# Orange-OpenSource/Cool-Chic

Measured on AMD Instinct MI355X. Metric: decoded Mpixel/s, higher is better.
Workload: dtype int64+f64 entropy / f32 synthesis; 1 GPU; kodak24; frames_on_rank0=24, frame=512x768 RGB 8-bit, HOP decoder

## Files before the change

cool_chic_amd/csrc/ccd_dec_parts4.inc:

```
                ".p2align 6\n\t"
                "440:\n\t"
                "s_lshr_b64 s[40:41], s[52:53], 24\n\t"
                "ds_read2st64_b64 v[58:61], v50 offset0:2 offset1:3\n\t"
                "s_waitcnt lgkmcnt(1)\n\t"
                "v_mad_u64_u32 v[44:45], s[42:43], s40, v40, 0\n\t"
                "v_mad_u32_u24 v45, v40, s41, v45\n\t"
                "v_cmpx_ge_u64 vcc, s[50:51], v[44:45]\n\t"
                "v_mad_u64_u32 v[48:49], s[42:43], s40, v41, 0\n\t"
                "v_mad_u32_u24 v49, v41, s41, v49\n\t"
                "s_ff1_i32_b64 s44, vcc\n\t"
                "v_writelane_b32 %[raw], s44, 0\n\t"
                "v_readfirstlane_b32 s48, v48\n\t"
                "v_readfirstlane_b32 s49, v49\n\t"
                "v_readfirstlane_b32 s46, v44\n\t"
                "v_readfirstlane_b32 s47, v45\n\t"
                "s_mov_b64 exec, -1\n\t"
                "s_sub_u32 s76, s50, s46\n\t"
                "s_subb_u32 s77, s51, s47\n\t"
                "441:\n\t"
                "s_lshr_b64 s[40:41], s[48:49], 24\n\t"
                "v_mad_u64_u32 v[44:45], s[42:43], s40, v42, 0\n\t"
                "v_mad_u32_u24 v45, v42, s41, v45\n\t"
                "v_cmpx_ge_u64 vcc, s[76:77], v[44:45]\n\t"
                "v_mad_u64_u32 v[48:49], s[42:43], s40, v43, 0\n\t"
                "v_mad_u32_u24 v49, v43, s41, v49\n\t"
                "s_ff1_i32_b64 s80, vcc\n\t"
                "v_writelane_b32 %[raw], s80, 1\n\t"
                "v_readfirstlane_b32 s74, v48\n\t"
                "v_readfirstlane_b32 s75, v49\n\t"
                "v_readfirstlane_b32 s78, v44\n\t"
                "v_readfirstlane_b32 s79, v45\n\t"
                "s_mov_b64 exec, -1\n\t"
                "s_min_u32 s58, s49, s75\n\t"
                "s_cmp_eq_u32 s58, 0\n\t"
                "s_cbranch_scc1 1801f\n\t"
                "s_sub_u32 s50, s76, s78\n\t"
                "s_subb_u32 s51, s77, s79\n\t"
                "442:\n\t"
                "ds_read_b32 v54, v51\n\t"
                "s_lshr_b64 s[40:41], s[74:75], 24\n\t"
                "ds_read2st64_b64 v[40:43], v50 offset0:4 offset1:5\n\t"
                "s_waitcnt lgkmcnt(2)\n\t"
                "v_mad_u64_u32 v[44:45], s[42:43], s40, v58, 0\n\t"
                "v_mad_u32_u24 v45, v58, s41, v45\n\t"
                "v_cmpx_ge_u64 vcc, s[50:51], v[44:45]\n\t"
                "v_mad_u64_u32 v[48:49], s[42:43], s40, v59, 0\n\t"
                "v_mad_u32_u24 v49, v59, s41, v49\n\t"
                "s_ff1_i32_b64 s44, vcc\n\t"
                "v_writelane_b32 %[raw], s44, 2\n\t"
                "v_readfirstlane_b32 s52, v48\n\t"
                "v_readfirstlane_b32 s53, v49\n\t"
                "v_readfirstlane_b32 s46, v44\n\t"
                "v_readfirstlane_b32 s47, v45\n\t"
                "s_mov_b64 exec, -1\n\t"
                "s_sub_u32 s76, s50, s46\n\t"
                "s_subb_u32 s77, s51, s47\n\t"
                "443:\n\t"
                "s_lshr_b64 s[40:41], s[52:53], 24\n\t"
                "v_mad_u64_u32 v[44:45], s[42:43], s40, v60, 0\n\t"
                "v_mad_u32_u24 v45, v60, s41, v45\n\t"
                "v_cmpx_ge_u64 vcc, s[76:77], v[44:45]\n\t"
                "v_mad_u64_u32 v[48:49], s[42:43], s40, v61, 0\n\t"
                "v_mad_u32_u24 v49, v61, s41, v49\n\t"
                "s_ff1_i32_b64 s80, vcc\n\t"
                "v_writelane_b32 %[raw], s80, 3\n\t"
                "v_readfirstlane_b32 s48, v48\n\t"
                "v_readfirstlane_b32 s49, v49\n\t"
                "v_readfirstlane_b32 s78, v44\n\t"
                "v_readfirstlane_b32 s79, v45\n\t"
                "s_mov_b64 exec, -1\n\t"
                "s_min_u32 s58, s53, s49\n\t"
                "s_cmp_eq_u32 s58, 0\n\t"
                "s_cbranch_scc1 1802f\n\t"
                "s_sub_u32 s50, s76, s78\n\t"
                "s_subb_u32 s51, s77, s79\n\t"
                "444:\n\t"
                "s_mov_b64 exec, 0xf\n\t"
                "v_sub_u32 v52, %[top], %[raw]\n\t"
                "v_add_u32 v52, 1, v52\n\t"
                "ds_write_b8 %[ring], v52\n\t"
                "global_store_byte %[goff], v52, %[lat]\n\t"
                "s_mov_b64 exec, -1\n\t"
                "s_add_u32 s58, %[pix0], %[i]\n\t"
                "s_add_u32 s58, s58, 4\n\t"
                "v_mov_b32 v56, s58\n\t"
                "ds_write_b32 %[rdy], v56 offset:68\n\t"
                "s_add_u32 s59, %[i], 8\n\t"
                "s_waitcnt lgkmcnt(3)\n\t"
                "v_readfirstlane_b32 s58, v54\n\t"
                "s_cmp_le_u32 s59, s66\n\t"
                "s_cbranch_scc0 445f\n\t"
                "s_bitcmp1_b32 s58, 1\n\t"
                "s_cbranch_scc0 445f\n\t"
                "s_mov_b64 s[52:53], s[48:49]\n\t"
                "v_add_u32 v50, 0x800, v50\n\t"
                "ds_read_b32 %[top], v53\n\t"
                "ds_read_b32 %[ring], v53 offset:520\n\t"
                "ds_read_b32 %[goff], v53 offset:1040\n\t"
                "s_add_u32 %[i], %[i], 4\n\t"
                "s_mov_b32 s67, %[i]\n\t"
                "s_add_u32 s54, %[i], 4\n\t"
                "s_branch 450f\n\t"
                "445:\n\t"
                "s_mov_b64 s[52:53], s[48:49]\n\t"
                "s_add_u32 %[i], %[i], 4\n\t"
                "s_mov_b32 s67, %[i]\n\t"
                "s_branch 126b\n\t"
                "1801:\n\t"
                "s_cmp_eq_u32 s49, 0\n\t"
                "s_cbranch_scc0 1851f\n\t"
                "s_cmp_eq_u32 s48, 0\n\t"
                "s_cbranch_scc1 2001f\n\t"
                "s_sub_u32 s58, %[wpos], %[wbase]\n\t"
                "s_and_b32 s58, s58, 63\n\t"
                "v_readlane_b32 s57, %[wbuf], s58\n\t"
                "s_mov_b32 s77, s76\n\t"
                "s_mov_b32 s76, s57\n\t"
                "s_mov_b32 s49, s48\n\t"
                "s_mov_b32 s48, 0\n\t"
                "s_add_u32 %[wpos], %[wpos], 1\n\t"
                "s_cmp_eq_u32 s58, 63\n\t"
                "s_cbranch_scc0 441b\n\t"
                "s_mov_b64 s[50:51], s[76:77]\n\t"
                "s_mov_b64 s[52:53], s[48:49]\n\t"
                "s_add_u32 %[i], %[i], 1\n\t"
                "s_branch 15f\n\t"
                "2001:\n\t"
                "ds_read_b64 v[42:43], v50 offset:512\n\t"
                "ds_read_b64 v[46:47], v50 offset:1024\n\t"
                "s_branch 40b\n\t"
                "1851:\n\t"
                "s_cmp_eq_u32 s74, 0\n\t"
                "s_cbranch_scc1 2051f\n\t"
                "s_sub_u32 s50, s76, s78\n\t"
                "s_subb_u32 s51, s77, s79\n\t"
                "s_sub_u32 s58, %[wpos], %[wbase]\n\t"
                "s_and_b32 s58, s58, 63\n\t"
                "v_readlane_b32 s57, %[wbuf], s58\n\t"
                "s_mov_b32 s51, s50\n\t"
                "s_mov_b32 s50, s57\n\t"
                "s_mov_b32 s75, s74\n\t"
                "s_mov_b32 s74, 0\n\t"
                "s_add_u32 %[wpos], %[wpos], 1\n\t"
                "s_cmp_eq_u32 s58, 63\n\t"
                "s_cbranch_scc0 442b\n\t"
                "s_mov_b64 s[52:53], s[74:75]\n\t"
                "s_add_u32 %[i], %[i], 2\n\t"
                "s_branch 15f\n\t"
                "2051:\n\t"
                "s_mov_b64 s[50:51], s[76:77]\n\t"
                "s_mov_b32 s46, s78\n\t"
                "s_mov_b32 s47, s79\n\t"
                "s_mov_b32 s44, s80\n\t"
                "s_mov_b64 s[52:53], s[48:49]\n\t"
                "s_mov_b64 s[48:49], s[74:75]\n\t"
                "s_add_u32 %[i], %[i], 1\n\t"
                "ds_read_b64 v[46:47], v50 offset:1024\n\t"
                "ds_read_b64 v[40:41], v50 offset:1536\n\t"
                "s_branch 41b\n\t"
                "1802:\n\t"
                "s_cmp_eq_u32 s53, 0\n\t"
                "s_cbranch_scc0 1852f\n\t"
                "s_cmp_eq_u32 s52, 0\n\t"
                "s_cbranch_scc1 2002f\n\t"
                "s_sub_u32 s58, %[wpos], %[wbase]\n\t"
                "s_and_b32 s58, s58, 63\n\t"
                "v_readlane_b32 s57, %[wbuf], s58\n\t"
                "s_mov_b32 s77, s76\n\t"
                "s_mov_b32 s76, s57\n\t"
                "s_mov_b32 s53, s52\n\t"
                "s_mov_b32 s52, 0\n\t"
                "s_add_u32 %[wpos], %[wpos], 1\n\t"
                "s_cmp_eq_u32 s58, 63\n\t"
                "s_cbranch_scc0 443b\n\t"
                "s_mov_b64 s[50:51], s[76:77]\n\t"
                "s_add_u32 %[i], %[i], 3\n\t"
                "s_branch 15f\n\t"
                "2002:\n\t"
                "s_mov_b64 s[48:49], s[52:53]\n\t"
                "s_mov_b64 s[52:53], s[74:75]\n\t"
                "s_add_u32 %[i], %[i], 2\n\t"
                "ds_read_b64 v[40:41], v50 offset:1536\n\t"
                "ds_read_b64 v[42:43], v50 offset:2048\n\t"
                "s_branch 42b\n\t"
                "1852:\n\t"
                "s_cmp_eq_u32 s48, 0\n\t"
                "s_cbranch_scc1 2052f\n\t"
                "s_sub_u32 s50, s76, s78\n\t"
                "s_subb_u32 s51, s77, s79\n\t"
                "s_sub_u32 s58, %[wpos], %[wbase]\n\t"
                "s_and_b32 s58, s58, 63\n\t"
                "v_readlane_b32 s57, %[wbuf], s58\n\t"
                "s_mov_b32 s51, s50\n\t"
                "s_mov_b32 s50, s57\n\t"
                "s_mov_b32 s49, s48\n\t"
                "s_mov_b32 s48, 0\n\t"
                "s_add_u32 %[wpos], %[wpos], 1\n\t"
                "s_cmp_eq_u32 s58, 63\n\t"
                "s_cbranch_scc0 444b\n\t"
                "s_mov_b64 s[52:53], s[48:49]\n\t"
                "s_add_u32 %[i], %[i], 4\n\t"
                "s_branch 15f\n\t"
                "2052:\n\t"
                "s_mov_b64 s[50:51], s[76:77]\n\t"
                "s_mov_b32 s46, s78\n\t"
                "s_mov_b32 s47, s79\n\t"
                "s_mov_b32 s44, s80\n\t"
                "s_add_u32 %[i], %[i], 3\n\t"
                "v_add_u32 v50, 0x600, v50\n\t"
                "ds_read_b64 v[42:43], v50 offset:512\n\t"
                "ds_read_b64 v[46:47], v50 offset:1024\n\t"
                "s_branch 40b\n\t"
                ".p2align 6\n\t"
                "450:\n\t"
                "s_lshr_b64 s[40:41], s[52:53], 24\n\t"
                "ds_read2st64_b64 v[58:61], v50 offset0:2 offset1:3\n\t"
                "s_waitcnt lgkmcnt(1)\n\t"
                "v_mad_u64_u32 v[44:45], s[42:43], s40, v40, 0\n\t"
                "v_mad_u32_u24 v45, v40, s41, v45\n\t"
                "v_cmpx_ge_u64 vcc, s[50:51], v[44:45]\n\t"
                "v_mad_u64_u32 v[48:49], s[42:43], s40, v41, 0\n\t"
                "v_mad_u32_u24 v49, v41, s41, v49\n\t"
                "s_ff1_i32_b64 s44, vcc\n\t"
                "v_writelane_b32 %[raw], s44, 4\n\t"
                "v_readfirstlane_b32 s48, v48\n\t"
                "v_readfirstlane_b32 s49, v49\n\t"
                "v_readfirstlane_b32 s46, v44\n\t"
                "v_readfirstlane_b32 s47, v45\n\t"
                "s_mov_b64 exec, -1\n\t"
                "s_sub_u32 s76, s50, s46\n\t"
                "s_subb_u32 s77, s51, s47\n\t"
                "451:\n\t"
                "s_lshr_b64 s[40:41], s[48:49], 24\n\t"
                "v_mad_u64_u32 v[44:45], s[42:43], s40, v42, 0\n\t"
                "v_mad_u32_u24 v45, v42, s41, v45\n\t"
                "v_cmpx_ge_u64 vcc, s[76:77], v[44:45]\n\t"
                "v_mad_u64_u32 v[48:49], s[42:43], s40, v43, 0\n\t"
                "v_mad_u32_u24 v49, v43, s41, v49\n\t"
                "s_ff1_i32_b64 s80, vcc\n\t"
                "v_writelane_b32 %[raw], s80, 5\n\t"
                "v_readfirstlane_b32 s74, v48\n\t"
                "v_readfirstlane_b32 s75, v49\n\t"
                "v_readfirstlane_b32 s78, v44\n\t"
                "v_readfirstlane_b32 s79, v45\n\t"
                "s_mov_b64 exec, -1\n\t"
                "s_min_u32 s58, s49, s75\n\t"
                "s_cmp_eq_u32 s58, 0\n\t"
                "s_cbranch_scc1 2201f\n\t"
                "s_sub_u32 s50, s76, s78\n\t"
                "s_subb_u32 s51, s77, s79\n\t"
                "452:\n\t"
                "ds_read_b32 v54, v51\n\t"
                "s_lshr_b64 s[40:41], s[74:75], 24\n\t"
                "ds_read2st64_b64 v[40:43], v50 offset0:4 offset1:5\n\t"
                "s_waitcnt lgkmcnt(2)\n\t"
                "v_mad_u64_u32 v[44:45], s[42:43], s40, v58, 0\n\t"
                "v_mad_u32_u24 v45, v58, s41, v45\n\t"
                "v_cmpx_ge_u64 vcc, s[50:51], v[44:45]\n\t"
                "v_mad_u64_u32 v[48:49], s[42:43], s40, v59, 0\n\t"
                "v_mad_u32_u24 v49, v59, s41, v49\n\t"
                "s_ff1_i32_b64 s44, vcc\n\t"
                "v_writelane_b32 %[raw], s44, 6\n\t"
                "v_readfirstlane_b32 s52, v48\n\t"
                "v_readfirstlane_b32 s53, v49\n\t"
                "v_readfirstlane_b32 s46, v44\n\t"
                "v_readfirstlane_b32 s47, v45\n\t"
                "s_mov_b64 exec, -1\n\t"
                "s_sub_u32 s76, s50, s46\n\t"
                "s_subb_u32 s77, s51, s47\n\t"
                "453:\n\t"
                "s_lshr_b64 s[40:41], s[52:53], 24\n\t"
                "v_mad_u64_u32 v[44:45], s[42:43], s40, v60, 0\n\t"
                "v_mad_u32_u24 v45, v60, s41, v45\n\t"
                "v_cmpx_ge_u64 vcc, s[76:77], v[44:45]\n\t"
                "v_mad_u64_u32 v[48:49], s[42:43], s40, v61, 0\n\t"
                "v_mad_u32_u24 v49, v61, s41, v49\n\t"
                "s_ff1_i32_b64 s80, vcc\n\t"
                "v_writelane_b32 %[raw], s80, 7\n\t"
                "v_readfirstlane_b32 s48, v48\n\t"
                "v_readfirstlane_b32 s49, v49\n\t"
                "v_readfirstlane_b32 s78, v44\n\t"
                "v_readfirstlane_b32 s79, v45\n\t"
                "s_mov_b64 exec, -1\n\t"
                "s_min_u32 s58, s53, s49\n\t"
                "s_cmp_eq_u32 s58, 0\n\t"
                "s_cbranch_scc1 2202f\n\t"
                "s_sub_u32 s50, s76, s78\n\t"
                "s_subb_u32 s51, s77, s79\n\t"
                "454:\n\t"
                "s_mov_b64 exec, 0xf0\n\t"
                "v_sub_u32 v52, %[top], %[raw]\n\t"
                "v_add_u32 v52, 1, v52\n\t"
                "ds_write_b8 %[ring], v52\n\t"
                "global_store_byte %[goff], v52, %[lat]\n\t"
                "s_mov_b64 exec, -1\n\t"
                "s_add_u32 s58, %[pix0], %[i]\n\t"
                "s_add_u32 s58, s58, 4\n\t"
                "v_mov_b32 v56, s58\n\t"
                "ds_write_b32 %[rdy], v56 offset:68\n\t"
                "s_add_u32 s59, %[i], 8\n\t"
                "s_waitcnt lgkmcnt(3)\n\t"
                "v_readfirstlane_b32 s58, v54\n\t"
                "s_cmp_le_u32 s59, s66\n\t"
                "s_cbranch_scc0 455f\n\t"
                "s_bitcmp1_b32 s58, 2\n\t"
                "s_cbranch_scc0 455f\n\t"
                "s_mov_b64 s[52:53], s[48:49]\n\t"
                "v_add_u32 v50, 0x800, v50\n\t"
                "ds_read_b32 %[top], v53\n\t"
                "ds_read_b32 %[ring], v53 offset:520\n\t"
                "ds_read_b32 %[goff], v53 offset:1040\n\t"
                "s_add_u32 %[i], %[i], 4\n\t"
                "s_mov_b32 s67, %[i]\n\t"
                "s_add_u32 s54, %[i], 4\n\t"
                "s_branch 460f\n\t"
                "455:\n\t"
                "s_mov_b64 s[52:53], s[48:49]\n\t"
                "s_add_u32 %[i], %[i], 4\n\t"
                "s_mov_b32 s67, %[i]\n\t"
                "s_branch 126b\n\t"
                "2201:\n\t"
                "s_cmp_eq_u32 s49, 0\n\t"
                "s_cbranch_scc0 2251f\n\t"
                "s_cmp_eq_u32 s48, 0\n\t"
                "s_cbranch_scc1 2401f\n\t"
                "s_sub_u32 s58, %[wpos], %[wbase]\n\t"
                "s_and_b32 s58, s58, 63\n\t"
                "v_readlane_b32 s57, %[wbuf], s58\n\t"
                "s_mov_b32 s77, s76\n\t"
                "s_mov_b32 s76, s57\n\t"
                "s_mov_b32 s49, s48\n\t"
                "s_mov_b32 s48, 0\n\t"
                "s_add_u32 %[wpos], %[wpos], 1\n\t"
                "s_cmp_eq_u32 s58, 63\n\t"
                "s_cbranch_scc0 451b\n\t"
                "s_mov_b64 s[50:51], s[76:77]\n\t"
                "s_mov_b64 s[52:53], s[48:49]\n\t"
                "s_add_u32 %[i], %[i], 1\n\t"
                "s_branch 15f\n\t"
                "2401:\n\t"
                "ds_read_b64 v[42:43], v50 offset:512\n\t"
                "ds_read_b64 v[46:47], v50 offset:1024\n\t"
                "s_branch 40b\n\t"
                "2251:\n\t"
                "s_cmp_eq_u32 s74, 0\n\t"
                "s_cbranch_scc1 2451f\n\t"
                "s_sub_u32 s50, s76, s78\n\t"
                "s_subb_u32 s51, s77, s79\n\t"
                "s_sub_u32 s58, %[wpos], %[wbase]\n\t"
                "s_and_b32 s58, s58, 63\n\t"
                "v_readlane_b32 s57, %[wbuf], s58\n\t"
                "s_mov_b32 s51, s50\n\t"
                "s_mov_b32 s50, s57\n\t"
                "s_mov_b32 s75, s74\n\t"
                "s_mov_b32 s74, 0\n\t"
                "s_add_u32 %[wpos], %[wpos], 1\n\t"
                "s_cmp_eq_u32 s58, 63\n\t"
                "s_cbranch_scc0 452b\n\t"
                "s_mov_b64 s[52:53], s[74:75]\n\t"
                "s_add_u32 %[i], %[i], 2\n\t"
                "s_branch 15f\n\t"
                "2451:\n\t"
                "s_mov_b64 s[50:51], s[76:77]\n\t"
                "s_mov_b32 s46, s78\n\t"
                "s_mov_b32 s47, s79\n\t"
                "s_mov_b32 s44, s80\n\t"
                "s_mov_b64 s[52:53], s[48:49]\n\t"
                "s_mov_b64 s[48:49], s[74:75]\n\t"
                "s_add_u32 %[i], %[i], 1\n\t"
                "ds_read_b64 v[46:47], v50 offset:1024\n\t"
                "ds_read_b64 v[40:41], v50 offset:1536\n\t"
                "s_branch 41b\n\t"
                "2202:\n\t"
                "s_cmp_eq_u32 s53, 0\n\t"
                "s_cbranch_scc0 2252f\n\t"
                "s_cmp_eq_u32 s52, 0\n\t"
                "s_cbranch_scc1 2402f\n\t"
                "s_sub_u32 s58, %[wpos], %[wbase]\n\t"
                "s_and_b32 s58, s58, 63\n\t"
                "v_readlane_b32 s57, %[wbuf], s58\n\t"
                "s_mov_b32 s77, s76\n\t"
                "s_mov_b32 s76, s57\n\t"
                "s_mov_b32 s53, s52\n\t"
                "s_mov_b32 s52, 0\n\t"
                "s_add_u32 %[wpos], %[wpos], 1\n\t"
                "s_cmp_eq_u32 s58, 63\n\t"
                "s_cbranch_scc0 453b\n\t"
                "s_mov_b64 s[50:51], s[76:77]\n\t"
                "s_add_u32 %[i], %[i], 3\n\t"
                "s_branch 15f\n\t"
                "2402:\n\t"
                "s_mov_b64 s[48:49], s[52:53]\n\t"
                "s_mov_b64 s[52:53], s[74:75]\n\t"
                "s_add_u32 %[i], %[i], 2\n\t"
                "ds_read_b64 v[40:41], v50 offset:1536\n\t"
                "ds_read_b64 v[42:43], v50 offset:2048\n\t"
                "s_branch 42b\n\t"
                "2252:\n\t"
                "s_cmp_eq_u32 s48, 0\n\t"
                "s_cbranch_scc1 2452f\n\t"
                "s_sub_u32 s50, s76, s78\n\t"
                "s_subb_u32 s51, s77, s79\n\t"
                "s_sub_u32 s58, %[wpos], %[wbase]\n\t"
                "s_and_b32 s58, s58, 63\n\t"
                "v_readlane_b32 s57, %[wbuf], s58\n\t"
                "s_mov_b32 s51, s50\n\t"
                "s_mov_b32 s50, s57\n\t"
                "s_mov_b32 s49, s48\n\t"
                "s_mov_b32 s48, 0\n\t"
                "s_add_u32 %[wpos], %[wpos], 1\n\t"
                "s_cmp_eq_u32 s58, 63\n\t"
                "s_cbranch_scc0 454b\n\t"
                "s_mov_b64 s[52:53], s[48:49]\n\t"
                "s_add_u32 %[i], %[i], 4\n\t"
                "s_branch 15f\n\t"
                "2452:\n\t"
                "s_mov_b64 s[50:51], s[76:77]\n\t"
                "s_mov_b32 s46, s78\n\t"
                "s_mov_b32 s47, s79\n\t"
                "s_mov_b32 s44, s80\n\t"
                "s_add_u32 %[i], %[i], 3\n\t"
                "v_add_u32 v50, 0x600, v50\n\t"
                "ds_read_b64 v[42:43], v50 offset:512\n\t"
                "ds_read_b64 v[46:47], v50 offset:1024\n\t"
                "s_branch 40b\n\t"
                ".p2align 6\n\t"
                "460:\n\t"
                "s_lshr_b64 s[40:41], s[52:53], 24\n\t"
                "ds_read2st64_b64 v[58:61], v50 offset0:2 offset1:3\n\t"
                "s_waitcnt lgkmcnt(1)\n\t"
                "v_mad_u64_u32 v[44:45], s[42:43], s40, v40, 0\n\t"
                "v_mad_u32_u24 v45, v40, s41, v45\n\t"
                "v_cmpx_ge_u64 vcc, s[50:51], v[44:45]\n\t"
                "v_mad_u64_u32 v[48:49], s[42:43], s40, v41, 0\n\t"
                "v_mad_u32_u24 v49, v41, s41, v49\n\t"
                "s_ff1_i32_b64 s44, vcc\n\t"
                "v_writelane_b32 %[raw], s44, 8\n\t"
                "v_readfirstlane_b32 s48, v48\n\t"
                "v_readfirstlane_b32 s49, v49\n\t"
                "v_readfirstlane_b32 s46, v44\n\t"
                "v_readfirstlane_b32 s47, v45\n\t"
                "s_mov_b64 exec, -1\n\t"
                "s_sub_u32 s76, s50, s46\n\t"
                "s_subb_u32 s77, s51, s47\n\t"
                "461:\n\t"
                "s_lshr_b64 s[40:41], s[48:49], 24\n\t"
                "v_mad_u64_u32 v[44:45], s[42:43], s40, v42, 0\n\t"
                "v_mad_u32_u24 v45, v42, s41, v45\n\t"
                "v_cmpx_ge_u64 vcc, s[76:77], v[44:45]\n\t"
                "v_mad_u64_u32 v[48:49], s[42:43], s40, v43, 0\n\t"
                "v_mad_u32_u24 v49, v43, s41, v49\n\t"
                "s_ff1_i32_b64 s80, vcc\n\t"
                "v_writelane_b32 %[raw], s80, 9\n\t"
                "v_readfirstlane_b32 s74, v48\n\t"
                "v_readfirstlane_b32 s75, v49\n\t"
                "v_readfirstlane_b32 s78, v44\n\t"
                "v_readfirstlane_b32 s79, v45\n\t"
                "s_mov_b64 exec, -1\n\t"
                "s_min_u32 s58, s49, s75\n\t"
                "s_cmp_eq_u32 s58, 0\n\t"
                "s_cbranch_scc1 2601f\n\t"
                "s_sub_u32 s50, s76, s78\n\t"
                "s_subb_u32 s51, s77, s79\n\t"
                "462:\n\t"
                "ds_read_b32 v54, v51\n\t"
                "s_lshr_b64 s[40:41], s[74:75], 24\n\t"
                "ds_read2st64_b64 v[40:43], v50 offset0:4 offset1:5\n\t"
                "s_waitcnt lgkmcnt(2)\n\t"
                "v_mad_u64_u32 v[44:45], s[42:43], s40, v58, 0\n\t"
                "v_mad_u32_u24 v45, v58, s41, v45\n\t"
                "v_cmpx_ge_u64 vcc, s[50:51], v[44:45]\n\t"
                "v_mad_u64_u32 v[48:49], s[42:43], s40, v59, 0\n\t"
                "v_mad_u32_u24 v49, v59, s41, v49\n\t"
                "s_ff1_i32_b64 s44, vcc\n\t"
                "v_writelane_b32 %[raw], s44, 10\n\t"
                "v_readfirstlane_b32 s52, v48\n\t"
                "v_readfirstlane_b32 s53, v49\n\t"
                "v_readfirstlane_b32 s46, v44\n\t"
                "v_readfirstlane_b32 s47, v45\n\t"
                "s_mov_b64 exec, -1\n\t"
                "s_sub_u32 s76, s50, s46\n\t"
                "s_subb_u32 s77, s51, s47\n\t"
                "463:\n\t"
                "s_lshr_b64 s[40:41], s[52:53], 24\n\t"
                "v_mad_u64_u32 v[44:45], s[42:43], s40, v60, 0\n\t"
                "v_mad_u32_u24 v45, v60, s41, v45\n\t"
                "v_cmpx_ge_u64 vcc, s[76:77], v[44:45]\n\t"
                "v_mad_u64_u32 v[48:49], s[42:43], s40, v61, 0\n\t"
                "v_mad_u32_u24 v49, v61, s41, v49\n\t"
                "s_ff1_i32_b64 s80, vcc\n\t"
                "v_writelane_b32 %[raw], s80, 11\n\t"
                "v_readfirstlane_b32 s48, v48\n\t"
                "v_readfirstlane_b32 s49, v49\n\t"
                "v_readfirstlane_b32 s78, v44\n\t"
                "v_readfirstlane_b32 s79, v45\n\t"
                "s_mov_b64 exec, -1\n\t"
                "s_min_u32 s58, s53, s49\n\t"
                "s_cmp_eq_u32 s58, 0\n\t"
                "s_cbranch_scc1 2602f\n\t"
                "s_sub_u32 s50, s76, s78\n\t"
                "s_subb_u32 s51, s77, s79\n\t"
                "464:\n\t"
                "s_mov_b64 exec, 0xf00\n\t"
                "v_sub_u32 v52, %[top], %[raw]\n\t"
                "v_add_u32 v52, 1, v52\n\t"
                "ds_write_b8 %[ring], v52\n\t"
                "global_store_byte %[goff], v52, %[lat]\n\t"
                "s_mov_b64 exec, -1\n\t"
                "s_add_u32 s58, %[pix0], %[i]\n\t"
                "s_add_u32 s58, s58, 4\n\t"
                "v_mov_b32 v56, s58\n\t"
                "ds_write_b32 %[rdy], v56 offset:68\n\t"
                "s_add_u32 s59, %[i], 8\n\t"
                "s_waitcnt lgkmcnt(3)\n\t"
                "v_readfirstlane_b32 s58, v54\n\t"
                "s_cmp_le_u32 s59, s66\n\t"
                "s_cbranch_scc0 465f\n\t"
                "s_bitcmp1_b32 s58, 3\n\t"
                "s_cbranch_scc0 465f\n\t"
                "s_mov_b64 s[52:53], s[48:49]\n\t"
                "v_add_u32 v50, 0x800, v50\n\t"
                "ds_read_b32 %[top], v53\n\t"
                "ds_read_b32 %[ring], v53 offset:520\n\t"
                "ds_read_b32 %[goff], v53 offset:1040\n\t"
                "s_add_u32 %[i], %[i], 4\n\t"
                "s_mov_b32 s67, %[i]\n\t"
                "s_add_u32 s54, %[i], 4\n\t"
                "s_branch 470f\n\t"
                "465:\n\t"
                "s_mov_b64 s[52:53], s[48:49]\n\t"
                "s_add_u32 %[i], %[i], 4\n\t"
                "s_mov_b32 s67, %[i]\n\t"
                "s_branch 126b\n\t"
                "2601:\n\t"
                "s_cmp_eq_u32 s49, 0\n\t"
                "s_cbranch_scc0 2651f\n\t"
                "s_cmp_eq_u32 s48, 0\n\t"
                "s_cbranch_scc1 2801f\n\t"
                "s_sub_u32 s58, %[wpos], %[wbase]\n\t"
                "s_and_b32 s58, s58, 63\n\t"
                "v_readlane_b32 s57, %[wbuf], s58\n\t"
                "s_mov_b32 s77, s76\n\t"
                "s_mov_b32 s76, s57\n\t"
                "s_mov_b32 s49, s48\n\t"
                "s_mov_b32 s48, 0\n\t"
                "s_add_u32 %[wpos], %[wpos], 1\n\t"
                "s_cmp_eq_u32 s58, 63\n\t"
                "s_cbranch_scc0 461b\n\t"
                "s_mov_b64 s[50:51], s[76:77]\n\t"
                "s_mov_b64 s[52:53], s[48:49]\n\t"
                "s_add_u32 %[i], %[i], 1\n\t"
                "s_branch 15f\n\t"
                "2801:\n\t"
                "ds_read_b64 v[42:43], v50 offset:512\n\t"
                "ds_read_b64 v[46:47], v50 offset:1024\n\t"
                "s_branch 40b\n\t"
                "2651:\n\t"
                "s_cmp_eq_u32 s74, 0\n\t"
                "s_cbranch_scc1 2851f\n\t"
                "s_sub_u32 s50, s76, s78\n\t"
                "s_subb_u32 s51, s77, s79\n\t"
                "s_sub_u32 s58, %[wpos], %[wbase]\n\t"
                "s_and_b32 s58, s58, 63\n\t"
                "v_readlane_b32 s57, %[wbuf], s58\n\t"
                "s_mov_b32 s51, s50\n\t"
                "s_mov_b32 s50, s57\n\t"
                "s_mov_b32 s75, s74\n\t"
                "s_mov_b32 s74, 0\n\t"
                "s_add_u32 %[wpos], %[wpos], 1\n\t"
                "s_cmp_eq_u32 s58, 63\n\t"
                "s_cbranch_scc0 462b\n\t"
                "s_mov_b64 s[52:53], s[74:75]\n\t"
                "s_add_u32 %[i], %[i], 2\n\t"
                "s_branch 15f\n\t"
                "2851:\n\t"
                "s_mov_b64 s[50:51], s[76:77]\n\t"
                "s_mov_b32 s46, s78\n\t"
                "s_mov_b32 s47, s79\n\t"
                "s_mov_b32 s44, s80\n\t"
                "s_mov_b64 s[52:53], s[48:49]\n\t"
                "s_mov_b64 s[48:49], s[74:75]\n\t"
                "s_add_u32 %[i], %[i], 1\n\t"
                "ds_read_b64 v[46:47], v50 offset:1024\n\t"
                "ds_read_b64 v[40:41], v50 offset:1536\n\t"
                "s_branch 41b\n\t"
                "2602:\n\t"
                "s_cmp_eq_u32 s53, 0\n\t"
                "s_cbranch_scc0 2652f\n\t"
                "s_cmp_eq_u32 s52, 0\n\t"
                "s_cbranch_scc1 2802f\n\t"
                "s_sub_u32 s58, %[wpos], %[wbase]\n\t"
                "s_and_b32 s58, s58, 63\n\t"
                "v_readlane_b32 s57, %[wbuf], s58\n\t"
                "s_mov_b32 s77, s76\n\t"
                "s_mov_b32 s76, s57\n\t"
                "s_mov_b32 s53, s52\n\t"
                "s_mov_b32 s52, 0\n\t"
                "s_add_u32 %[wpos], %[wpos], 1\n\t"
                "s_cmp_eq_u32 s58, 63\n\t"
                "s_cbranch_scc0 463b\n\t"
                "s_mov_b64 s[50:51], s[76:77]\n\t"
                "s_add_u32 %[i], %[i], 3\n\t"
                "s_branch 15f\n\t"
                "2802:\n\t"
                "s_mov_b64 s[48:49], s[52:53]\n\t"
                "s_mov_b64 s[52:53], s[74:75]\n\t"
                "s_add_u32 %[i], %[i], 2\n\t"
                "ds_read_b64 v[40:41], v50 offset:1536\n\t"
                "ds_read_b64 v[42:43], v50 offset:2048\n\t"
                "s_branch 42b\n\t"
                "2652:\n\t"
                "s_cmp_eq_u32 s48, 0\n\t"
                "s_cbranch_scc1 2852f\n\t"
                "s_sub_u32 s50, s76, s78\n\t"
                "s_subb_u32 s51, s77, s79\n\t"
                "s_sub_u32 s58, %[wpos], %[wbase]\n\t"
                "s_and_b32 s58, s58, 63\n\t"
                "v_readlane_b32 s57, %[wbuf], s58\n\t"
                "s_mov_b32 s51, s50\n\t"
                "s_mov_b32 s50, s57\n\t"
                "s_mov_b32 s49, s48\n\t"
                "s_mov_b32 s48, 0\n\t"
                "s_add_u32 %[wpos], %[wpos], 1\n\t"
                "s_cmp_eq_u32 s58, 63\n\t"
                "s_cbranch_scc0 464b\n\t"
                "s_mov_b64 s[52:53], s[48:49]\n\t"
                "s_add_u32 %[i], %[i], 4\n\t"
                "s_branch 15f\n\t"
                "2852:\n\t"
                "s_mov_b64 s[50:51], s[76:77]\n\t"
                "s_mov_b32 s46, s78\n\t"
                "s_mov_b32 s47, s79\n\t"
                "s_mov_b32 s44, s80\n\t"
                "s_add_u32 %[i], %[i], 3\n\t"
                "v_add_u32 v50, 0x600, v50\n\t"
                "ds_read_b64 v[42:43], v50 offset:512\n\t"
                "ds_read_b64 v[46:47], v50 offset:1024\n\t"
                "s_branch 40b\n\t"
                ".p2align 6\n\t"
                "470:\n\t"
                "s_lshr_b64 s[40:41], s[52:53], 24\n\t"
                "ds_read2st64_b64 v[58:61], v50 offset0:2 offset1:3\n\t"
                "s_waitcnt lgkmcnt(1)\n\t"
                "v_mad_u64_u32 v[44:45], s[42:43], s40, v40, 0\n\t"
                "v_mad_u32_u24 v45, v40, s41, v45\n\t"
                "v_cmpx_ge_u64 vcc, s[50:51], v[44:45]\n\t"
                "v_mad_u64_u32 v[48:49], s[42:43], s40, v41, 0\n\t"
                "v_mad_u32_u24 v49, v41, s41, v49\n\t"
                "s_ff1_i32_b64 s44, vcc\n\t"
                "v_writelane_b32 %[raw], s44, 12\n\t"
                "v_readfirstlane_b32 s48, v48\n\t"
                "v_readfirstlane_b32 s49, v49\n\t"
                "v_readfirstlane_b32 s46, v44\n\t"
                "v_readfirstlane_b32 s47, v45\n\t"
                "s_mov_b64 exec, -1\n\t"
                "s_sub_u32 s76, s50, s46\n\t"
                "s_subb_u32 s77, s51, s47\n\t"
                "471:\n\t"
                "s_lshr_b64 s[40:41], s[48:49], 24\n\t"
                "v_mad_u64_u32 v[44:45], s[42:43], s40, v42, 0\n\t"
                "v_mad_u32_u24 v45, v42, s41, v45\n\t"
                "v_cmpx_ge_u64 vcc, s[76:77], v[44:45]\n\t"
                "v_mad_u64_u32 v[48:49], s[42:43], s40, v43, 0\n\t"
                "v_mad_u32_u24 v49, v43, s41, v49\n\t"
                "s_ff1_i32_b64 s80, vcc\n\t"
                "v_writelane_b32 %[raw], s80, 13\n\t"
                "v_readfirstlane_b32 s74, v48\n\t"
                "v_readfirstlane_b32 s75, v49\n\t"
                "v_readfirstlane_b32 s78, v44\n\t"
                "v_readfirstlane_b32 s79, v45\n\t"
                "s_mov_b64 exec, -1\n\t"
                "s_min_u32 s58, s49, s75\n\t"
                "s_cmp_eq_u32 s58, 0\n\t"
                "s_cbranch_scc1 3001f\n\t"
                "s_sub_u32 s50, s76, s78\n\t"
                "s_subb_u32 s51, s77, s79\n\t"
                "472:\n\t"
                "s_lshr_b64 s[40:41], s[74:75], 24\n\t"
                "s_waitcnt lgkmcnt(0)\n\t"
                "v_mad_u64_u32 v[44:45], s[42:43], s40, v58, 0\n\t"
                "v_mad_u32_u24 v45, v58, s41, v45\n\t"
                "v_cmpx_ge_u64 vcc, s[50:51], v[44:45]\n\t"
                "v_mad_u64_u32 v[48:49], s[42:43], s40, v59, 0\n\t"
                "v_mad_u32_u24 v49, v59, s41, v49\n\t"
                "s_ff1_i32_b64 s44, vcc\n\t"
                "v_writelane_b32 %[raw], s44, 14\n\t"
                "v_readfirstlane_b32 s52, v48\n\t"
                "v_readfirstlane_b32 s53, v49\n\t"
                "v_readfirstlane_b32 s46, v44\n\t"
                "v_readfirstlane_b32 s47, v45\n\t"
                "s_mov_b64 exec, -1\n\t"
                "s_sub_u32 s76, s50, s46\n\t"
                "s_subb_u32 s77, s51, s47\n\t"
                "473:\n\t"
                "s_lshr_b64 s[40:41], s[52:53], 24\n\t"
                "v_mad_u64_u32 v[44:45], s[42:43], s40, v60, 0\n\t"
                "v_mad_u32_u24 v45, v60, s41, v45\n\t"
                "v_cmpx_ge_u64 vcc, s[76:77], v[44:45]\n\t"
                "v_mad_u64_u32 v[48:49], s[42:43], s40, v61, 0\n\t"
                "v_mad_u32_u24 v49, v61, s41, v49\n\t"
                "s_ff1_i32_b64 s80, vcc\n\t"
                "v_writelane_b32 %[raw], s80, 15\n\t"
                "v_readfirstlane_b32 s48, v48\n\t"
                "v_readfirstlane_b32 s49, v49\n\t"
                "v_readfirstlane_b32 s78, v44\n\t"
                "v_readfirstlane_b32 s79, v45\n\t"
                "s_mov_b64 exec, -1\n\t"
                "s_min_u32 s58, s53, s49\n\t"
                "s_cmp_eq_u32 s58, 0\n\t"
                "s_cbranch_scc1 3002f\n\t"
                "s_sub_u32 s50, s76, s78\n\t"
                "s_subb_u32 s51, s77, s79\n\t"
                "474:\n\t"
                "s_mov_b64 s[52:53], s[48:49]\n\t"
                "s_add_u32 %[i], %[i], 4\n\t"
                "s_branch 2b\n\t"
                "3001:\n\t"
                "s_cmp_eq_u32 s49, 0\n\t"
                "s_cbranch_scc0 3051f\n\t"
                "s_cmp_eq_u32 s48, 0\n\t"
                "s_cbranch_scc1 3201f\n\t"
                "s_sub_u32 s58, %[wpos], %[wbase]\n\t"
                "s_and_b32 s58, s58, 63\n\t"
                "v_readlane_b32 s57, %[wbuf], s58\n\t"
                "s_mov_b32 s77, s76\n\t"
                "s_mov_b32 s76, s57\n\t"
                "s_mov_b32 s49, s48\n\t"
                "s_mov_b32 s48, 0\n\t"
                "s_add_u32 %[wpos], %[wpos], 1\n\t"
                "s_cmp_eq_u32 s58, 63\n\t"
                "s_cbranch_scc0 471b\n\t"
                "s_mov_b64 s[50:51], s[76:77]\n\t"
                "s_mov_b64 s[52:53], s[48:49]\n\t"
                "s_add_u32 %[i], %[i], 1\n\t"
                "s_branch 15f\n\t"
                "3201:\n\t"
                "ds_read_b64 v[42:43], v50 offset:512\n\t"
                "ds_read_b64 v[46:47], v50 offset:1024\n\t"
                "s_branch 40b\n\t"
                "3051:\n\t"
                "s_cmp_eq_u32 s74, 0\n\t"
                "s_cbranch_scc1 3251f\n\t"
                "s_sub_u32 s50, s76, s78\n\t"
                "s_subb_u32 s51, s77, s79\n\t"
                "s_sub_u32 s58, %[wpos], %[wbase]\n\t"
                "s_and_b32 s58, s58, 63\n\t"
                "v_readlane_b32 s57, %[wbuf], s58\n\t"
                "s_mov_b32 s51, s50\n\t"
                "s_mov_b32 s50, s57\n\t"
                "s_mov_b32 s75, s74\n\t"
                "s_mov_b32 s74, 0\n\t"
                "s_add_u32 %[wpos], %[wpos], 1\n\t"
                "s_cmp_eq_u32 s58, 63\n\t"
                "s_cbranch_scc0 472b\n\t"
                "s_mov_b64 s[52:53], s[74:75]\n\t"
                "s_add_u32 %[i], %[i], 2\n\t"
                "s_branch 15f\n\t"
                "3251:\n\t"
                "s_mov_b64 s[50:51], s[76:77]\n\t"
                "s_mov_b32 s46, s78\n\t"
                "s_mov_b32 s47, s79\n\t"
                "s_mov_b32 s44, s80\n\t"
                "s_mov_b64 s[52:53], s[48:49]\n\t"
                "s_mov_b64 s[48:49], s[74:75]\n\t"
                "s_add_u32 %[i], %[i], 1\n\t"
                "ds_read_b64 v[46:47], v50 offset:1024\n\t"
                "ds_read_b64 v[40:41], v50 offset:1536\n\t"
                "s_branch 41b\n\t"
                "3002:\n\t"
                "s_cmp_eq_u32 s53, 0\n\t"
                "s_cbranch_scc0 3052f\n\t"
                "s_cmp_eq_u32 s52, 0\n\t"
                "s_cbranch_scc1 3202f\n\t"
                "s_sub_u32 s58, %[wpos], %[wbase]\n\t"
                "s_and_b32 s58, s58, 63\n\t"
                "v_readlane_b32 s57, %[wbuf], s58\n\t"
                "s_mov_b32 s77, s76\n\t"
                "s_mov_b32 s76, s57\n\t"
                "s_mov_b32 s53, s52\n\t"
                "s_mov_b32 s52, 0\n\t"
                "s_add_u32 %[wpos], %[wpos], 1\n\t"
                "s_cmp_eq_u32 s58, 63\n\t"
                "s_cbranch_scc0 473b\n\t"
                "s_mov_b64 s[50:51], s[76:77]\n\t"
                "s_add_u32 %[i], %[i], 3\n\t"
                "s_branch 15f\n\t"
                "3202:\n\t"
                "s_mov_b64 s[48:49], s[52:53]\n\t"
                "s_mov_b64 s[52:53], s[74:75]\n\t"
                "s_add_u32 %[i], %[i], 2\n\t"
                "ds_read_b64 v[40:41], v50 offset:1536\n\t"
                "ds_read_b64 v[42:43], v50 offset:2048\n\t"
                "s_branch 42b\n\t"
                "3052:\n\t"
                "s_cmp_eq_u32 s48, 0\n\t"
                "s_cbranch_scc1 3252f\n\t"
                "s_sub_u32 s50, s76, s78\n\t"
                "s_subb_u32 s51, s77, s79\n\t"
                "s_sub_u32 s58, %[wpos], %[wbase]\n\t"
                "s_and_b32 s58, s58, 63\n\t"
                "v_readlane_b32 s57, %[wbuf], s58\n\t"
                "s_mov_b32 s51, s50\n\t"
                "s_mov_b32 s50, s57\n\t"
                "s_mov_b32 s49, s48\n\t"
                "s_mov_b32 s48, 0\n\t"
                "s_add_u32 %[wpos], %[wpos], 1\n\t"
                "s_cmp_eq_u32 s58, 63\n\t"
                "s_cbranch_scc0 474b\n\t"
                "s_mov_b64 s[52:53], s[48:49]\n\t"
                "s_add_u32 %[i], %[i], 4\n\t"
                "s_branch 15f\n\t"
                "3252:\n\t"
                "s_mov_b64 s[50:51], s[76:77]\n\t"
                "s_mov_b32 s46, s78\n\t"
                "s_mov_b32 s47, s79\n\t"
                "s_mov_b32 s44, s80\n\t"
                "s_add_u32 %[i], %[i], 3\n\t"
                "v_add_u32 v50, 0x600, v50\n\t"
                "ds_read_b64 v[42:43], v50 offset:512\n\t"
                "ds_read_b64 v[46:47], v50 offset:1024\n\t"
                "s_branch 40b\n\t"
```

cool_chic_amd/csrc/ccd_dec_parts8.inc:

```
                ".p2align 6\n\t"
                "400:\n\t"
                "s_lshr_b64 s[40:41], s[52:53], 24\n\t"
                "ds_read2st64_b64 v[58:61], v50 offset0:2 offset1:3\n\t"
                "s_waitcnt lgkmcnt(1)\n\t"
                "v_mad_u64_u32 v[44:45], s[42:43], s40, v40, 0\n\t"
                "v_mad_u32_u24 v45, v40, s41, v45\n\t"
                "v_cmpx_ge_u64 vcc, s[50:51], v[44:45]\n\t"
                "v_mad_u64_u32 v[48:49], s[42:43], s40, v41, 0\n\t"
                "v_mad_u32_u24 v49, v41, s41, v49\n\t"
                "s_ff1_i32_b64 s44, vcc\n\t"
                "v_writelane_b32 %[raw], s44, 0\n\t"
                "v_readfirstlane_b32 s48, v48\n\t"
                "v_readfirstlane_b32 s49, v49\n\t"
                "v_readfirstlane_b32 s46, v44\n\t"
                "v_readfirstlane_b32 s47, v45\n\t"
                "s_mov_b64 exec, -1\n\t"
                "s_sub_u32 s76, s50, s46\n\t"
                "s_subb_u32 s77, s51, s47\n\t"
                "401:\n\t"
                "s_lshr_b64 s[40:41], s[48:49], 24\n\t"
                "v_mad_u64_u32 v[44:45], s[42:43], s40, v42, 0\n\t"
                "v_mad_u32_u24 v45, v42, s41, v45\n\t"
                "v_cmpx_ge_u64 vcc, s[76:77], v[44:45]\n\t"
                "v_mad_u64_u32 v[48:49], s[42:43], s40, v43, 0\n\t"
                "v_mad_u32_u24 v49, v43, s41, v49\n\t"
                "s_ff1_i32_b64 s80, vcc\n\t"
                "v_writelane_b32 %[raw], s80, 1\n\t"
                "v_readfirstlane_b32 s74, v48\n\t"
                "v_readfirstlane_b32 s75, v49\n\t"
                "v_readfirstlane_b32 s78, v44\n\t"
                "v_readfirstlane_b32 s79, v45\n\t"
                "s_mov_b64 exec, -1\n\t"
                "s_min_u32 s58, s49, s75\n\t"
                "s_cmp_eq_u32 s58, 0\n\t"
                "s_cbranch_scc1 1001f\n\t"
                "s_sub_u32 s50, s76, s78\n\t"
                "s_subb_u32 s51, s77, s79\n\t"
                "402:\n\t"
                "s_lshr_b64 s[40:41], s[74:75], 24\n\t"
                "ds_read2st64_b64 v[40:43], v50 offset0:4 offset1:5\n\t"
                "s_waitcnt lgkmcnt(1)\n\t"
                "v_mad_u64_u32 v[44:45], s[42:43], s40, v58, 0\n\t"
                "v_mad_u32_u24 v45, v58, s41, v45\n\t"
                "v_cmpx_ge_u64 vcc, s[50:51], v[44:45]\n\t"
                "v_mad_u64_u32 v[48:49], s[42:43], s40, v59, 0\n\t"
                "v_mad_u32_u24 v49, v59, s41, v49\n\t"
                "s_ff1_i32_b64 s44, vcc\n\t"
                "v_writelane_b32 %[raw], s44, 2\n\t"
                "v_readfirstlane_b32 s52, v48\n\t"
                "v_readfirstlane_b32 s53, v49\n\t"
                "v_readfirstlane_b32 s46, v44\n\t"
                "v_readfirstlane_b32 s47, v45\n\t"
                "s_mov_b64 exec, -1\n\t"
                "s_sub_u32 s76, s50, s46\n\t"
                "s_subb_u32 s77, s51, s47\n\t"
                "403:\n\t"
                "s_lshr_b64 s[40:41], s[52:53], 24\n\t"
                "v_mad_u64_u32 v[44:45], s[42:43], s40, v60, 0\n\t"
                "v_mad_u32_u24 v45, v60, s41, v45\n\t"
                "v_cmpx_ge_u64 vcc, s[76:77], v[44:45]\n\t"
                "v_mad_u64_u32 v[48:49], s[42:43], s40, v61, 0\n\t"
                "v_mad_u32_u24 v49, v61, s41, v49\n\t"
                "s_ff1_i32_b64 s80, vcc\n\t"
                "v_writelane_b32 %[raw], s80, 3\n\t"
                "v_readfirstlane_b32 s48, v48\n\t"
                "v_readfirstlane_b32 s49, v49\n\t"
                "v_readfirstlane_b32 s78, v44\n\t"
                "v_readfirstlane_b32 s79, v45\n\t"
                "s_mov_b64 exec, -1\n\t"
                "s_min_u32 s58, s53, s49\n\t"
                "s_cmp_eq_u32 s58, 0\n\t"
                "s_cbranch_scc1 1002f\n\t"
                "s_sub_u32 s50, s76, s78\n\t"
                "s_subb_u32 s51, s77, s79\n\t"
                "404:\n\t"
                "s_lshr_b64 s[40:41], s[48:49], 24\n\t"
                "ds_read2st64_b64 v[58:61], v50 offset0:6 offset1:7\n\t"
                "s_waitcnt lgkmcnt(1)\n\t"
                "v_mad_u64_u32 v[44:45], s[42:43], s40, v40, 0\n\t"
                "v_mad_u32_u24 v45, v40, s41, v45\n\t"
                "v_cmpx_ge_u64 vcc, s[50:51], v[44:45]\n\t"
                "v_mad_u64_u32 v[48:49], s[42:43], s40, v41, 0\n\t"
                "v_mad_u32_u24 v49, v41, s41, v49\n\t"
                "s_ff1_i32_b64 s44, vcc\n\t"
                "v_writelane_b32 %[raw], s44, 4\n\t"
                "v_readfirstlane_b32 s74, v48\n\t"
                "v_readfirstlane_b32 s75, v49\n\t"
                "v_readfirstlane_b32 s46, v44\n\t"
                "v_readfirstlane_b32 s47, v45\n\t"
                "s_mov_b64 exec, -1\n\t"
                "s_sub_u32 s76, s50, s46\n\t"
                "s_subb_u32 s77, s51, s47\n\t"
                "405:\n\t"
                "s_lshr_b64 s[40:41], s[74:75], 24\n\t"
                "v_mad_u64_u32 v[44:45], s[42:43], s40, v42, 0\n\t"
                "v_mad_u32_u24 v45, v42, s41, v45\n\t"
                "v_cmpx_ge_u64 vcc, s[76:77], v[44:45]\n\t"
                "v_mad_u64_u32 v[48:49], s[42:43], s40, v43, 0\n\t"
                "v_mad_u32_u24 v49, v43, s41, v49\n\t"
                "s_ff1_i32_b64 s80, vcc\n\t"
                "v_writelane_b32 %[raw], s80, 5\n\t"
                "v_readfirstlane_b32 s52, v48\n\t"
                "v_readfirstlane_b32 s53, v49\n\t"
                "v_readfirstlane_b32 s78, v44\n\t"
                "v_readfirstlane_b32 s79, v45\n\t"
                "s_mov_b64 exec, -1\n\t"
                "s_min_u32 s58, s75, s53\n\t"
                "s_cmp_eq_u32 s58, 0\n\t"
                "s_cbranch_scc1 1003f\n\t"
                "s_sub_u32 s50, s76, s78\n\t"
                "s_subb_u32 s51, s77, s79\n\t"
                "406:\n\t"
                "ds_read_b32 v54, v51\n\t"
                "s_lshr_b64 s[40:41], s[52:53], 24\n\t"
                "ds_read2st64_b64 v[40:43], v50 offset0:8 offset1:9\n\t"
                "s_waitcnt lgkmcnt(2)\n\t"
                "v_mad_u64_u32 v[44:45], s[42:43], s40, v58, 0\n\t"
                "v_mad_u32_u24 v45, v58, s41, v45\n\t"
                "v_cmpx_ge_u64 vcc, s[50:51], v[44:45]\n\t"
                "v_mad_u64_u32 v[48:49], s[42:43], s40, v59, 0\n\t"
                "v_mad_u32_u24 v49, v59, s41, v49\n\t"
                "s_ff1_i32_b64 s44, vcc\n\t"
                "v_writelane_b32 %[raw], s44, 6\n\t"
                "v_readfirstlane_b32 s48, v48\n\t"
                "v_readfirstlane_b32 s49, v49\n\t"
                "v_readfirstlane_b32 s46, v44\n\t"
                "v_readfirstlane_b32 s47, v45\n\t"
                "s_mov_b64 exec, -1\n\t"
                "s_sub_u32 s76, s50, s46\n\t"
                "s_subb_u32 s77, s51, s47\n\t"
                "407:\n\t"
                "s_lshr_b64 s[40:41], s[48:49], 24\n\t"
                "v_mad_u64_u32 v[44:45], s[42:43], s40, v60, 0\n\t"
                "v_mad_u32_u24 v45, v60, s41, v45\n\t"
                "v_cmpx_ge_u64 vcc, s[76:77], v[44:45]\n\t"
                "v_mad_u64_u32 v[48:49], s[42:43], s40, v61, 0\n\t"
                "v_mad_u32_u24 v49, v61, s41, v49\n\t"
                "s_ff1_i32_b64 s80, vcc\n\t"
                "v_writelane_b32 %[raw], s80, 7\n\t"
                "v_readfirstlane_b32 s74, v48\n\t"
                "v_readfirstlane_b32 s75, v49\n\t"
                "v_readfirstlane_b32 s78, v44\n\t"
                "v_readfirstlane_b32 s79, v45\n\t"
                "s_mov_b64 exec, -1\n\t"
                "s_min_u32 s58, s49, s75\n\t"
                "s_cmp_eq_u32 s58, 0\n\t"
                "s_cbranch_scc1 1004f\n\t"
                "s_sub_u32 s50, s76, s78\n\t"
                "s_subb_u32 s51, s77, s79\n\t"
                "408:\n\t"
                "s_mov_b64 exec, 0xff\n\t"
                "v_sub_u32 v52, %[top], %[raw]\n\t"
                "v_add_u32 v52, 1, v52\n\t"
                "ds_write_b8 %[ring], v52\n\t"
                "global_store_byte %[goff], v52, %[lat]\n\t"
                "s_mov_b64 exec, -1\n\t"
                "s_add_u32 s58, %[pix0], %[i]\n\t"
                "s_add_u32 s58, s58, 8\n\t"
                "v_mov_b32 v56, s58\n\t"
                "ds_write_b32 %[rdy], v56 offset:68\n\t"
                "s_sub_u32 s59, s66, %[i]\n\t"
                "s_waitcnt lgkmcnt(3)\n\t"
                "v_readfirstlane_b32 s58, v54\n\t"
                "s_cmp_eq_u32 s59, 16\n\t"
                "s_cbranch_scc0 409f\n\t"
                "s_bitcmp1_b32 s58, 1\n\t"
                "s_cbranch_scc0 409f\n\t"
                "ds_read_b32 %[top], v53\n\t"
                "ds_read_b32 %[ring], v53 offset:520\n\t"
                "ds_read_b32 %[goff], v53 offset:1040\n\t"
                "s_mov_b32 s65, 0\n\t"
                "s_mov_b32 s54, s66\n\t"
                "s_branch 308b\n\t"
                "409:\n\t"
                "s_mov_b64 s[52:53], s[74:75]\n\t"
                "s_add_u32 %[i], %[i], 8\n\t"
                "s_mov_b32 s67, %[i]\n\t"
                "s_branch 126b\n\t"
                "1001:\n\t"
                "s_cmp_eq_u32 s49, 0\n\t"
                "s_cbranch_scc0 1051f\n\t"
                "s_cmp_eq_u32 s48, 0\n\t"
                "s_cbranch_scc1 1201f\n\t"
                "s_sub_u32 s58, %[wpos], %[wbase]\n\t"
                "s_and_b32 s58, s58, 63\n\t"
                "v_readlane_b32 s57, %[wbuf], s58\n\t"
                "s_mov_b32 s77, s76\n\t"
                "s_mov_b32 s76, s57\n\t"
                "s_mov_b32 s49, s48\n\t"
                "s_mov_b32 s48, 0\n\t"
                "s_add_u32 %[wpos], %[wpos], 1\n\t"
                "s_cmp_eq_u32 s58, 63\n\t"
                "s_cbranch_scc0 401b\n\t"
                "s_mov_b64 s[50:51], s[76:77]\n\t"
                "s_mov_b64 s[52:53], s[48:49]\n\t"
                "s_add_u32 %[i], %[i], 1\n\t"
                "s_branch 15f\n\t"
                "1201:\n\t"
                "ds_read_b64 v[42:43], v50 offset:512\n\t"
                "ds_read_b64 v[46:47], v50 offset:1024\n\t"
                "s_branch 40b\n\t"
                "1051:\n\t"
                "s_cmp_eq_u32 s74, 0\n\t"
                "s_cbranch_scc1 1251f\n\t"
                "s_sub_u32 s50, s76, s78\n\t"
                "s_subb_u32 s51, s77, s79\n\t"
                "s_sub_u32 s58, %[wpos], %[wbase]\n\t"
                "s_and_b32 s58, s58, 63\n\t"
                "v_readlane_b32 s57, %[wbuf], s58\n\t"
                "s_mov_b32 s51, s50\n\t"
                "s_mov_b32 s50, s57\n\t"
                "s_mov_b32 s75, s74\n\t"
                "s_mov_b32 s74, 0\n\t"
                "s_add_u32 %[wpos], %[wpos], 1\n\t"
                "s_cmp_eq_u32 s58, 63\n\t"
                "s_cbranch_scc0 402b\n\t"
                "s_mov_b64 s[52:53], s[74:75]\n\t"
                "s_add_u32 %[i], %[i], 2\n\t"
                "s_branch 15f\n\t"
                "1251:\n\t"
                "s_mov_b64 s[50:51], s[76:77]\n\t"
                "s_mov_b32 s46, s78\n\t"
                "s_mov_b32 s47, s79\n\t"
                "s_mov_b32 s44, s80\n\t"
                "s_mov_b64 s[52:53], s[48:49]\n\t"
                "s_mov_b64 s[48:49], s[74:75]\n\t"
                "s_add_u32 %[i], %[i], 1\n\t"
                "ds_read_b64 v[46:47], v50 offset:1024\n\t"
                "ds_read_b64 v[40:41], v50 offset:1536\n\t"
                "s_branch 41b\n\t"
                "1002:\n\t"
                "s_cmp_eq_u32 s53, 0\n\t"
                "s_cbranch_scc0 1052f\n\t"
                "s_cmp_eq_u32 s52, 0\n\t"
                "s_cbranch_scc1 1202f\n\t"
                "s_sub_u32 s58, %[wpos], %[wbase]\n\t"
                "s_and_b32 s58, s58, 63\n\t"
                "v_readlane_b32 s57, %[wbuf], s58\n\t"
                "s_mov_b32 s77, s76\n\t"
                "s_mov_b32 s76, s57\n\t"
                "s_mov_b32 s53, s52\n\t"
                "s_mov_b32 s52, 0\n\t"
                "s_add_u32 %[wpos], %[wpos], 1\n\t"
                "s_cmp_eq_u32 s58, 63\n\t"
                "s_cbranch_scc0 403b\n\t"
                "s_mov_b64 s[50:51], s[76:77]\n\t"
                "s_add_u32 %[i], %[i], 3\n\t"
                "s_branch 15f\n\t"
                "1202:\n\t"
                "s_mov_b64 s[48:49], s[52:53]\n\t"
                "s_mov_b64 s[52:53], s[74:75]\n\t"
                "s_add_u32 %[i], %[i], 2\n\t"
                "ds_read_b64 v[40:41], v50 offset:1536\n\t"
                "ds_read_b64 v[42:43], v50 offset:2048\n\t"
                "s_branch 42b\n\t"
                "1052:\n\t"
                "s_cmp_eq_u32 s48, 0\n\t"
                "s_cbranch_scc1 1252f\n\t"
                "s_sub_u32 s50, s76, s78\n\t"
                "s_subb_u32 s51, s77, s79\n\t"
                "s_sub_u32 s58, %[wpos], %[wbase]\n\t"
                "s_and_b32 s58, s58, 63\n\t"
                "v_readlane_b32 s57, %[wbuf], s58\n\t"
                "s_mov_b32 s51, s50\n\t"
                "s_mov_b32 s50, s57\n\t"
                "s_mov_b32 s49, s48\n\t"
                "s_mov_b32 s48, 0\n\t"
                "s_add_u32 %[wpos], %[wpos], 1\n\t"
                "s_cmp_eq_u32 s58, 63\n\t"
                "s_cbranch_scc0 404b\n\t"
                "s_mov_b64 s[52:53], s[48:49]\n\t"
                "s_add_u32 %[i], %[i], 4\n\t"
                "s_branch 15f\n\t"
                "1252:\n\t"
                "s_mov_b64 s[50:51], s[76:77]\n\t"
                "s_mov_b32 s46, s78\n\t"
                "s_mov_b32 s47, s79\n\t"
                "s_mov_b32 s44, s80\n\t"
                "s_add_u32 %[i], %[i], 3\n\t"
                "v_add_u32 v50, 0x600, v50\n\t"
                "ds_read_b64 v[42:43], v50 offset:512\n\t"
                "ds_read_b64 v[46:47], v50 offset:1024\n\t"
                "s_branch 40b\n\t"
                "1003:\n\t"
                "s_cmp_eq_u32 s75, 0\n\t"
                "s_cbranch_scc0 1053f\n\t"
                "s_cmp_eq_u32 s74, 0\n\t"
                "s_cbranch_scc1 1203f\n\t"
                "s_sub_u32 s58, %[wpos], %[wbase]\n\t"
                "s_and_b32 s58, s58, 63\n\t"
                "v_readlane_b32 s57, %[wbuf], s58\n\t"
                "s_mov_b32 s77, s76\n\t"
                "s_mov_b32 s76, s57\n\t"
                "s_mov_b32 s75, s74\n\t"
                "s_mov_b32 s74, 0\n\t"
                "s_add_u32 %[wpos], %[wpos], 1\n\t"
                "s_cmp_eq_u32 s58, 63\n\t"
                "s_cbranch_scc0 405b\n\t"
                "s_mov_b64 s[50:51], s[76:77]\n\t"
                "s_mov_b64 s[52:53], s[74:75]\n\t"
                "s_add_u32 %[i], %[i], 5\n\t"
                "s_branch 15f\n\t"
                "1203:\n\t"
                "s_mov_b64 s[52:53], s[48:49]\n\t"
                "s_mov_b64 s[48:49], s[74:75]\n\t"
                "s_add_u32 %[i], %[i], 4\n\t"
                "v_add_u32 v50, 0x600, v50\n\t"
                "ds_read_b64 v[46:47], v50 offset:1024\n\t"
                "ds_read_b64 v[40:41], v50 offset:1536\n\t"
                "s_branch 41b\n\t"
                "1053:\n\t"
                "s_cmp_eq_u32 s52, 0\n\t"
                "s_cbranch_scc1 1253f\n\t"
                "s_sub_u32 s50, s76, s78\n\t"
                "s_subb_u32 s51, s77, s79\n\t"
                "s_sub_u32 s58, %[wpos], %[wbase]\n\t"
                "s_and_b32 s58, s58, 63\n\t"
                "v_readlane_b32 s57, %[wbuf], s58\n\t"
                "s_mov_b32 s51, s50\n\t"
                "s_mov_b32 s50, s57\n\t"
                "s_mov_b32 s53, s52\n\t"
                "s_mov_b32 s52, 0\n\t"
                "s_add_u32 %[wpos], %[wpos], 1\n\t"
                "s_cmp_eq_u32 s58, 63\n\t"
                "s_cbranch_scc0 406b\n\t"
                "s_add_u32 %[i], %[i], 6\n\t"
                "s_branch 15f\n\t"
                "1253:\n\t"
                "s_mov_b64 s[50:51], s[76:77]\n\t"
                "s_mov_b32 s46, s78\n\t"
                "s_mov_b32 s47, s79\n\t"
                "s_mov_b32 s44, s80\n\t"
                "s_mov_b64 s[48:49], s[52:53]\n\t"
                "s_mov_b64 s[52:53], s[74:75]\n\t"
                "s_add_u32 %[i], %[i], 5\n\t"
                "v_add_u32 v50, 0x600, v50\n\t"
                "ds_read_b64 v[40:41], v50 offset:1536\n\t"
                "ds_read_b64 v[42:43], v50 offset:2048\n\t"
                "s_branch 42b\n\t"
                "1004:\n\t"
                "s_cmp_eq_u32 s49, 0\n\t"
                "s_cbranch_scc0 1054f\n\t"
                "s_cmp_eq_u32 s48, 0\n\t"
                "s_cbranch_scc1 1204f\n\t"
                "s_sub_u32 s58, %[wpos], %[wbase]\n\t"
                "s_and_b32 s58, s58, 63\n\t"
                "v_readlane_b32 s57, %[wbuf], s58\n\t"
                "s_mov_b32 s77, s76\n\t"
                "s_mov_b32 s76, s57\n\t"
                "s_mov_b32 s49, s48\n\t"
                "s_mov_b32 s48, 0\n\t"
                "s_add_u32 %[wpos], %[wpos], 1\n\t"
                "s_cmp_eq_u32 s58, 63\n\t"
                "s_cbranch_scc0 407b\n\t"
                "s_mov_b64 s[50:51], s[76:77]\n\t"
                "s_mov_b64 s[52:53], s[48:49]\n\t"
                "s_add_u32 %[i], %[i], 7\n\t"
                "s_branch 15f\n\t"
                "1204:\n\t"
                "s_add_u32 %[i], %[i], 6\n\t"
                "v_add_u32 v50, 0xc00, v50\n\t"
                "ds_read_b64 v[42:43], v50 offset:512\n\t"
                "ds_read_b64 v[46:47], v50 offset:1024\n\t"
                "s_branch 40b\n\t"
                "1054:\n\t"
                "s_cmp_eq_u32 s74, 0\n\t"
                "s_cbranch_scc1 1254f\n\t"
                "s_sub_u32 s50, s76, s78\n\t"
                "s_subb_u32 s51, s77, s79\n\t"
                "s_sub_u32 s58, %[wpos], %[wbase]\n\t"
                "s_and_b32 s58, s58, 63\n\t"
                "v_readlane_b32 s57, %[wbuf], s58\n\t"
                "s_mov_b32 s51, s50\n\t"
                "s_mov_b32 s50, s57\n\t"
                "s_mov_b32 s75, s74\n\t"
                "s_mov_b32 s74, 0\n\t"
                "s_add_u32 %[wpos], %[wpos], 1\n\t"
                "s_cmp_eq_u32 s58, 63\n\t"
                "s_cbranch_scc0 408b\n\t"
                "s_mov_b64 s[52:53], s[74:75]\n\t"
                "s_add_u32 %[i], %[i], 8\n\t"
                "s_branch 15f\n\t"
                "1254:\n\t"
                "s_mov_b64 s[50:51], s[76:77]\n\t"
                "s_mov_b32 s46, s78\n\t"
                "s_mov_b32 s47, s79\n\t"
                "s_mov_b32 s44, s80\n\t"
                "s_mov_b64 s[52:53], s[48:49]\n\t"
                "s_mov_b64 s[48:49], s[74:75]\n\t"
                "s_add_u32 %[i], %[i], 7\n\t"
                "v_add_u32 v50, 0xc00, v50\n\t"
                "ds_read_b64 v[46:47], v50 offset:1024\n\t"
                "ds_read_b64 v[40:41], v50 offset:1536\n\t"
                "s_branch 41b\n\t"
                ".p2align 6\n\t"
                "420:\n\t"
                "s_lshr_b64 s[40:41], s[52:53], 24\n\t"
                "ds_read2st64_b64 v[58:61], v50 offset0:2 offset1:3\n\t"
                "s_waitcnt lgkmcnt(1)\n\t"
                "v_mad_u64_u32 v[44:45], s[42:43], s40, v40, 0\n\t"
                "v_mad_u32_u24 v45, v40, s41, v45\n\t"
                "v_cmpx_ge_u64 vcc, s[50:51], v[44:45]\n\t"
                "v_mad_u64_u32 v[48:49], s[42:43], s40, v41, 0\n\t"
                "v_mad_u32_u24 v49, v41, s41, v49\n\t"
                "s_ff1_i32_b64 s44, vcc\n\t"
                "v_writelane_b32 %[raw], s44, 8\n\t"
                "v_readfirstlane_b32 s48, v48\n\t"
                "v_readfirstlane_b32 s49, v49\n\t"
                "v_readfirstlane_b32 s46, v44\n\t"
                "v_readfirstlane_b32 s47, v45\n\t"
                "s_mov_b64 exec, -1\n\t"
                "s_sub_u32 s76, s50, s46\n\t"
                "s_subb_u32 s77, s51, s47\n\t"
                "421:\n\t"
                "s_lshr_b64 s[40:41], s[48:49], 24\n\t"
                "v_mad_u64_u32 v[44:45], s[42:43], s40, v42, 0\n\t"
                "v_mad_u32_u24 v45, v42, s41, v45\n\t"
                "v_cmpx_ge_u64 vcc, s[76:77], v[44:45]\n\t"
                "v_mad_u64_u32 v[48:49], s[42:43], s40, v43, 0\n\t"
                "v_mad_u32_u24 v49, v43, s41, v49\n\t"
                "s_ff1_i32_b64 s80, vcc\n\t"
                "v_writelane_b32 %[raw], s80, 9\n\t"
                "v_readfirstlane_b32 s74, v48\n\t"
                "v_readfirstlane_b32 s75, v49\n\t"
                "v_readfirstlane_b32 s78, v44\n\t"
                "v_readfirstlane_b32 s79, v45\n\t"
                "s_mov_b64 exec, -1\n\t"
                "s_min_u32 s58, s49, s75\n\t"
                "s_cmp_eq_u32 s58, 0\n\t"
                "s_cbranch_scc1 1401f\n\t"
                "s_sub_u32 s50, s76, s78\n\t"
                "s_subb_u32 s51, s77, s79\n\t"
                "422:\n\t"
                "s_lshr_b64 s[40:41], s[74:75], 24\n\t"
                "ds_read2st64_b64 v[40:43], v50 offset0:4 offset1:5\n\t"
                "s_waitcnt lgkmcnt(1)\n\t"
                "v_mad_u64_u32 v[44:45], s[42:43], s40, v58, 0\n\t"
                "v_mad_u32_u24 v45, v58, s41, v45\n\t"
                "v_cmpx_ge_u64 vcc, s[50:51], v[44:45]\n\t"
                "v_mad_u64_u32 v[48:49], s[42:43], s40, v59, 0\n\t"
                "v_mad_u32_u24 v49, v59, s41, v49\n\t"
                "s_ff1_i32_b64 s44, vcc\n\t"
                "v_writelane_b32 %[raw], s44, 10\n\t"
                "v_readfirstlane_b32 s52, v48\n\t"
                "v_readfirstlane_b32 s53, v49\n\t"
                "v_readfirstlane_b32 s46, v44\n\t"
                "v_readfirstlane_b32 s47, v45\n\t"
                "s_mov_b64 exec, -1\n\t"
                "s_sub_u32 s76, s50, s46\n\t"
                "s_subb_u32 s77, s51, s47\n\t"
                "423:\n\t"
                "s_lshr_b64 s[40:41], s[52:53], 24\n\t"
                "v_mad_u64_u32 v[44:45], s[42:43], s40, v60, 0\n\t"
                "v_mad_u32_u24 v45, v60, s41, v45\n\t"
                "v_cmpx_ge_u64 vcc, s[76:77], v[44:45]\n\t"
                "v_mad_u64_u32 v[48:49], s[42:43], s40, v61, 0\n\t"
                "v_mad_u32_u24 v49, v61, s41, v49\n\t"
                "s_ff1_i32_b64 s80, vcc\n\t"
                "v_writelane_b32 %[raw], s80, 11\n\t"
                "v_readfirstlane_b32 s48, v48\n\t"
                "v_readfirstlane_b32 s49, v49\n\t"
                "v_readfirstlane_b32 s78, v44\n\t"
                "v_readfirstlane_b32 s79, v45\n\t"
                "s_mov_b64 exec, -1\n\t"
                "s_min_u32 s58, s53, s49\n\t"
                "s_cmp_eq_u32 s58, 0\n\t"
                "s_cbranch_scc1 1402f\n\t"
                "s_sub_u32 s50, s76, s78\n\t"
                "s_subb_u32 s51, s77, s79\n\t"
                "424:\n\t"
                "s_lshr_b64 s[40:41], s[48:49], 24\n\t"
                "ds_read2st64_b64 v[58:61], v50 offset0:6 offset1:7\n\t"
                "s_waitcnt lgkmcnt(1)\n\t"
                "v_mad_u64_u32 v[44:45], s[42:43], s40, v40, 0\n\t"
                "v_mad_u32_u24 v45, v40, s41, v45\n\t"
                "v_cmpx_ge_u64 vcc, s[50:51], v[44:45]\n\t"
                "v_mad_u64_u32 v[48:49], s[42:43], s40, v41, 0\n\t"
// ... 286 lines not shown
```

cool_chic_amd/csrc/ccd_entropy_pipe.hip:

```cpp
#include <hip/hip_runtime.h>
#include <type_traits>

#include "ccd_device.hpp"
#include "ccd_kernels.hpp"
#include "ccd_laplace.hpp"
#include "ccd_wavefront.hpp"

namespace ccd {

#if defined(CCD_PIPE_PROFILE) && CCD_PIPE_PROFILE >= 3
#define PROF_T() __builtin_amdgcn_s_memtime()
#define PROF_ADD(var, t0) var += __builtin_amdgcn_s_memtime() - (t0)
#define PROF_SUB(var, t0) var -= __builtin_amdgcn_s_memtime() - (t0)
#else
#define PROF_T() 0ull
#define PROF_ADD(var, t0) (void)(t0)
#define PROF_SUB(var, t0) (void)(t0)
#endif
#if defined(CCD_PIPE_PROFILE) && CCD_PIPE_PROFILE == 2 && defined(CCD_PIPE_TRACE)
#define LPROF_T(cond) __builtin_amdgcn_s_memtime()
#elif defined(CCD_PIPE_PROFILE) && CCD_PIPE_PROFILE == 2
#define LPROF_T(cond) ((cond) ? __builtin_amdgcn_s_memtime() : 0ull)
#else
#define LPROF_T(cond) 0ull
#endif
#if defined(CCD_PIPE_TRACE)
constexpr int kTraceTasks = 512;
constexpr uint32_t kTraceLdsBytes = kTraceTasks * 32u;
__device__ unsigned int g_trace[kTraceTasks * 8];
__device__ unsigned int g_trace_cfg[2];
constexpr bool kProfTrace = true;
#else
constexpr bool kProfTrace = false;
#endif

#ifndef CCD_T8
#define CCD_T8 25
#endif
#ifndef CCD_T4
#define CCD_T4 9
#endif
#ifndef CCD_PIPE_THREADS
#define CCD_PIPE_THREADS 512
#endif
constexpr int kPipeThreads = CCD_PIPE_THREADS;
constexpr int kPipeWaves = kPipeThreads / 64;
constexpr int kProducers = kPipeWaves - 1;
constexpr int kRows = 128;
constexpr int kSlots = 16;
constexpr int kMaxNV = 8;
constexpr int kRingRows = 512;
constexpr int kNarrowMaxScale = kScaleOffset;
constexpr int kIfceFastIn = 12;
constexpr unsigned kSpinLimit = 1u << 27;

struct alignas(16) RowMeta {
    double rcp[kRows + 2];
    int32_t mu_idx[kRows + 2];
    int32_t top[kRows + 2];
    uint32_t cell[kRows + 2];
    uint32_t goff[kRows + 2];
};
static_assert(offsetof(RowMeta, cell) - offsetof(RowMeta, top) == 520 && offsetof(RowMeta, goff) - offsetof(RowMeta, top) == 1040,
              "the decoder's asm region reads cell / goff at these immediate offsets from a top symbol's address");

extern __shared__ __attribute__((aligned(16))) unsigned char ccd_pipe_smem[];
template <typename T>
__device__ __forceinline__ T* smem_at(uint32_t off) { return reinterpret_cast<T*>(ccd_pipe_smem + off); }
__device__ __forceinline__ uint32_t lds_addr(const void* p) {
    return static_cast<uint32_t>(reinterpret_cast<uintptr_t>((__attribute__((address_space(3))) const char*)p));
}
template <typename T>
__device__ __forceinline__ __attribute__((address_space(3))) T* lds_at(uint32_t addr) {
    return reinterpret_cast<__attribute__((address_space(3))) T*>(static_cast<uintptr_t>(addr));
}
template <typename T>
struct LdsRef {
    uint32_t off;
    __device__ __forceinline__ operator T*() const { return reinterpret_cast<T*>(ccd_pipe_smem + off); }
    __device__ __forceinline__ LdsRef& operator=(T* p) {
        off = static_cast<uint32_t>(reinterpret_cast<unsigned char*>(const_cast<typename std::remove_const<T>::type*>(p)) - ccd_pipe_smem);
        return *this;
    }
};

struct PipeLayout { uint32_t ring, w, b, act, a, tab, meta, rcp, exp, ready, consumed, abort, end; int n_w_hidden; };
__host__ __device__ constexpr PipeLayout pipe_layout(int dim, int n_layers, int in_pad, int ring_rows, int mf_tabs) {
    PipeLayout L{};
    L.ring = 0;
    L.w = static_cast<uint32_t>(ring_rows) * 64u;
    L.n_w_hidden = (n_layers - 1) * dim * in_pad;
    const int n_w_total = L.n_w_hidden + 4 * in_pad;
    L.b = L.w + static_cast<uint32_t>((n_w_total + 3) & ~3) * 4u;
    const int n_b_total = (n_layers - 1) * dim + 4;
    L.act = L.b + static_cast<uint32_t>((n_b_total + 1) & ~1) * 8u;
    L.a = L.act + static_cast<uint32_t>(kProducers * ((mf_tabs ? 16 : 8) * in_pad + 4)) * 4u;
    L.tab = L.a + static_cast<uint32_t>(mf_tabs) * 1024u;
    L.meta = L.tab + static_cast<uint32_t>(kRows + 1) * 64u * 8u;
    L.rcp = L.meta + static_cast<uint32_t>(sizeof(RowMeta));
    L.exp = L.rcp + static_cast<uint32_t>(kNumScale + 1) * 8u;
    L.ready = L.exp + static_cast<uint32_t>(1 << CCD_EXP_LOG) * 8u;
    L.consumed = L.ready + static_cast<uint32_t>(kSlots) * 4u;
    L.abort = L.consumed + 8u;
    L.end = (L.ready + static_cast<uint32_t>(kSlots + 8) * 4u + 15u) & ~15u;
    return L;
}

struct ShapeDyn { static constexpr bool fixed = false; static constexpr int dim = 0, n_layers = 0, n_sp = 0; };
template <int DIM, int NL, int NSP>
struct ShapeFix { static constexpr bool fixed = true; static constexpr int dim = DIM, n_layers = NL, n_sp = NSP; };
using ShapeHop = ShapeFix<20, 3, 14>;

__host__ __device__ constexpr int feat_stride(int n_if) { return n_if > 0 ? n_if : 1; }

struct PipeCtx {
    const EntropyParams* P;
    LdsRef<uint2> s_tab;
    LdsRef<RowMeta> s_meta;
    LdsRef<const double> s_rcp;
    LdsRef<const double> s_exp;
    LdsRef<int32_t> s_w;
    LdsRef<int64_t> s_b;
    LdsRef<int32_t> s_act;
    LdsRef<uint32_t> s_a;
    LdsRef<int8_t> s_ring;
    LdsRef<uint32_t> s_ready;
    LdsRef<uint32_t> s_consumed;
    LdsRef<uint32_t> s_abort;
    int dim, n_layers, n_sp, n_if, n_w_hidden;
    int ring_mask;
#if defined(CCD_PIPE_TRACE)
    uint32_t trace_off;
#endif
    int H, W, fin, fh, fw;
    int fstride;
    int task_pix;
    int k_left;
    int8_t* lat;
    uint32_t seq_base;
    uint32_t px_base;
};

struct DecState {
    uint64_t dist, range;
    uint32_t word_pos, wbase, wbuf;
    uint64_t n_decoded;
    uint32_t n_part_batches;
    unsigned long long prof_wait, prof_work, stall_ticks, stall_events, n_rare, n_search, n_spins;
    unsigned long long wait_by_j[6];
};

__device__ __forceinline__ void lds_write_release(uint32_t* p, uint32_t v) {
    __hip_atomic_store(p, v, __ATOMIC_RELEASE, __HIP_MEMORY_SCOPE_WORKGROUP);
}
__device__ __forceinline__ uint32_t lds_load_acquire(const uint32_t* p) {
    return __builtin_amdgcn_readfirstlane(__hip_atomic_load(p, __ATOMIC_ACQUIRE, __HIP_MEMORY_SCOPE_WORKGROUP));
}

template <typename T> using glb_ptr = T __attribute__((address_space(1)))*;

__device__ __forceinline__ int uni(int v) { return __builtin_amdgcn_readfirstlane(v); }
__device__ __forceinline__ uint32_t uni(uint32_t v) { return __builtin_amdgcn_readfirstlane(v); }
__device__ __forceinline__ uint64_t uni(uint64_t v) {
    return (static_cast<uint64_t>(uni(static_cast<uint32_t>(v >> 32))) << 32) | uni(static_cast<uint32_t>(v));
}

__device__ __forceinline__ bool wait_ge(const uint32_t* p, uint32_t want_v, uint32_t* s_abort) {
    const uint32_t want = uni(want_v);
    if (__builtin_expect(static_cast<int32_t>(lds_load_acquire(p) - want) >= 0, 1)) return true;
    unsigned spins = 0;
    while (static_cast<int32_t>(lds_load_acquire(p) - want) < 0) {
        if ((++spins & 1023u) == 0) {
            if (lds_load_acquire(s_abort) != 0) return false;
            if (spins > kSpinLimit) { lds_write_release(s_abort, static_cast<uint32_t>(-CCD_ERR_HIP)); return false; }
        }
    }
    return true;
}

__device__ __forceinline__ bool progress_reached(const uint32_t* p, uint32_t want_batches, uint32_t want_pixels) {
    const uint64_t v = uni(__hip_atomic_load(reinterpret_cast<const uint64_t*>(p), __ATOMIC_ACQUIRE, __HIP_MEMORY_SCOPE_WORKGROUP));
    return static_cast<int32_t>((static_cast<uint32_t>(v) - want_batches) | (static_cast<uint32_t>(v >> 32) - want_pixels)) >= 0;
}
__device__ __forceinline__ bool wait_ge2(const uint32_t* p, uint32_t want_batches_v, uint32_t want_pixels_v, uint32_t* s_abort) {
    const uint32_t want_batches = uni(want_batches_v), want_pixels = uni(want_pixels_v);
    if (__builtin_expect(progress_reached(p, want_batches, want_pixels), 1)) return true;
    unsigned spins = 0;
    while (!progress_reached(p, want_batches, want_pixels)) {
        if ((++spins & 1023u) == 0) {
            if (lds_load_acquire(s_abort) != 0) return false;
            if (spins > kSpinLimit) { lds_write_release(s_abort, static_cast<uint32_t>(-CCD_ERR_HIP)); return false; }
        }
    }
    return true;
}

template <bool MF>
__device__ __forceinline__ uint32_t decoder_grid(const PipeCtx& C, DecState& S) {
    const int lane = threadIdx.x & 63;
    const EntropyParams& P = *C.P;
    StepIter it;
    it.init(uni(C.H), uni(C.W));
    uint32_t seq = uni(C.seq_base);
    uint64_t rc_dist = uni(S.dist), rc_range = uni(S.range);
    uint32_t word_pos = uni(S.word_pos), wbase = uni(S.wbase), wbuf = S.wbuf;
    const uint32_t n_words = uni(P.n_words);
    const glb_ptr<const uint32_t> words_g = (glb_ptr<const uint32_t>)P.words;
    int task_pix = uni(C.task_pix);
    const int grid_w = uni(C.W);
    const uint32_t bpx_shift = task_pix == 2 ? 3u : 4u;
    const int bpx = task_pix == 2 ? 8 : 16;
    const int slot_mask = kRows / bpx - 1;
    int task_shift = task_pix == 8 ? 3 : (task_pix == 4 ? 2 : 1);
    const uint32_t ready_base = C.s_ready.off;
    const uint32_t top_base = C.s_meta.off + static_cast<uint32_t>(offsetof(RowMeta, top));
    const uint32_t tab_lane = C.s_tab.off + static_cast<uint32_t>(lane) * 8u;
    const uint32_t lane_top_off = top_base + static_cast<uint32_t>(lane & (bpx - 1)) * 4u;
    const uint64_t lat_addr = uni(reinterpret_cast<uint64_t>(C.lat));
    const RowMeta& meta = *C.s_meta;
    bool ok = true;
    int raw = 0, top_l = 0;
    uint32_t n_spins = 0;
    uint32_t pix0 = uni(C.px_base);
    uint32_t n_part = 0;
    GridSeg segs[3];
    const int n_segs = grid_segments(static_cast<uint32_t>(it.H), static_cast<uint32_t>(it.W), uni(C.task_pix), segs);
    int seg_i = 0, seg_c = 0;
    while (ok && seg_c < it.n_steps) {
        while (seg_i + 1 < n_segs && seg_c >= static_cast<int>(segs[seg_i].first + segs[seg_i].steps)) ++seg_i;
        const bool seg_body = segs[seg_i].body;
        const int seg_steps = it.raster ? 1 : static_cast<int>(segs[seg_i].steps);
        const uint32_t seg_n_pix = uni(segs[seg_i].n_pix);
        task_pix = uni(segs[seg_i].task_pix);
        task_shift = task_pix == 8 ? 3 : (task_pix == 4 ? 2 : 1);
        it.seek(seg_c);
        seg_c += seg_steps;
        uint32_t n_step = seg_body ? seg_n_pix : static_cast<uint32_t>(it.n), step_x0 = static_cast<uint32_t>(it.x0), step_hy = static_cast<uint32_t>(it.H - it.y0);
        uint32_t steps_left = (it.raster || seg_body) ? 1u : static_cast<uint32_t>(seg_steps);
        uint32_t i = 0, mode = 0;
        uint32_t v_ring = 0, v_goff = 0;
        while (true) {
            uint32_t status, k_rare;
            i = uni(i); seq = uni(seq); mode = uni(mode); n_spins = uni(n_spins);
            n_step = uni(n_step); step_x0 = uni(step_x0); step_hy = uni(step_hy); steps_left = uni(steps_left); pix0 = uni(pix0);
            n_part = uni(n_part);
#pragma clang diagnostic push
#pragma clang diagnostic ignored "-Winline-asm"
            asm volatile(
                "s_mov_b64 s[50:51], %[dst]\n\t"
                "s_mov_b64 s[52:53], %[rng]\n\t"
                "s_lshl_b32 s69, 1, %[bshift]\n\t"
                "s_sub_u32 s62, s69, 1\n\t"
                "s_lshl_b32 s70, 1, %[tshift]\n\t"
                "s_sub_u32 s70, s70, 1\n\t"
                "s_sub_u32 s64, %[gw], 10\n\t"
                "s_mov_b32 s65, 0\n\t"
                "s_cmp_eq_u32 s69, 16\n\t"
                "s_cselect_b32 s61, 1, 0\n\t"
                "s_mul_i32 s72, %[n], s61\n\t"
                "s_lshr_b32 s73, 16, %[tshift]\n\t"
                "s_bfm_b32 s73, s73, 0\n\t"
                "s_cmp_eq_u32 %[mode], 0\n\t"
                "s_cbranch_scc0 6f\n\t"
                "5:\n\t"
                "s_add_u32 s54, %[i], s69\n\t"
                "s_min_u32 s54, s54, %[n]\n\t"
                "s_and_b32 s55, %[seq], %[smask]\n\t"
                "v_lshl_add_u32 v51, s55, 2, %[rdy]\n\t"
                "s_lshl_b32 s56, s55, %[bshift]\n\t"
                "s_sub_u32 s57, s54, %[i]\n\t"
                "s_add_u32 s57, s57, s70\n\t"
                "s_lshr_b32 s57, s57, %[tshift]\n\t"
                "s_bfm_b32 s57, s57, 0\n\t"
                "v_lshl_add_u32 v50, s56, 9, %[tabl]\n\t"
                "v_lshl_add_u32 v53, s56, 2, %[l4]\n\t"
                "s_mov_b32 s68, 0\n\t"
                "s_branch 18f\n\t"
                "11:\n\t"
                "s_add_u32 s68, s68, 1\n\t"
                "s_cmp_lt_u32 s68, 1024\n\t"
                "s_cbranch_scc0 7f\n\t"
                "18:\n\t"
                "ds_read_b32 v52, v51\n\t"
                "ds_read_b32 %[top], v53\n\t"
                "ds_read_b32 %[ring], v53 offset:520\n\t"
                "ds_read_b32 %[goff], v53 offset:1040\n\t"
                "ds_read2st64_b64 v[40:43], v50 offset1:1\n\t"
                "s_waitcnt lgkmcnt(4)\n\t"
                "v_readfirstlane_b32 s58, v52\n\t"
                "s_cmp_eq_u32 s58, s57\n\t"
                "s_cbranch_scc1 13f\n\t"
                "s_bitcmp1_b32 s58, 0\n\t"
                "s_cbranch_scc0 11b\n\t"
                "s_add_u32 %[spins], %[spins], s68\n\t"
                "s_add_u32 %[npart], %[npart], 1\n\t"
                "s_mov_b32 s65, 1\n\t"
                "s_mov_b32 s66, s54\n\t"
                "s_mov_b32 s67, %[i]\n\t"
                "s_add_u32 s54, %[i], s70\n\t"
                "s_add_u32 s54, s54, 1\n\t"
                "s_min_u32 s54, s54, s66\n\t"
                "s_sub_u32 s58, s54, %[i]\n\t"
                "s_cmp_eq_u32 s58, 8\n\t"
                "s_cbranch_scc1 400f\n\t"
                "s_cmp_eq_u32 s58, 4\n\t"
                "s_cbranch_scc1 440f\n\t"
                "s_branch 31f\n\t"
                "8:\n\t"
                "ds_read2st64_b64 v[40:43], v50 offset1:1\n\t"
                "s_branch 19f\n\t"
                "13:\n\t"
                "s_add_u32 %[spins], %[spins], s68\n\t"
                "19:\n\t"
                "s_sub_u32 s58, s54, %[i]\n\t"
                "s_cmp_eq_u32 s58, 16\n\t"
                "s_cbranch_scc1 80f\n\t"
                "31:\n\t"
                "s_waitcnt lgkmcnt(0)\n\t"
                ".p2align 6\n\t"
                "1:\n\t"
                "s_lshr_b64 s[40:41], s[52:53], 24\n\t"
                "ds_read_b64 v[46:47], v50 offset:1024\n\t"
                "s_waitcnt lgkmcnt(2)\n\t"
                "v_mad_u64_u32 v[44:45], s[42:43], s40, v40, 0\n\t"
                "v_mad_u32_u24 v45, v40, s41, v45\n\t"
                "v_cmpx_ge_u64 vcc, s[50:51], v[44:45]\n\t"
                "v_mad_u64_u32 v[48:49], s[42:43], s40, v41, 0\n\t"
                "v_mad_u32_u24 v49, v41, s41, v49\n\t"
                "s_and_b32 m0, %[i], s62\n\t"
                "s_ff1_i32_b64 s44, vcc\n\t"
                "v_readfirstlane_b32 s48, v48\n\t"
                "v_readfirstlane_b32 s49, v49\n\t"
                "v_readfirstlane_b32 s46, v44\n\t"
                "v_readfirstlane_b32 s47, v45\n\t"
                "s_mov_b64 exec, -1\n\t"
                "s_cmp_eq_u32 s49, 0\n\t"
                "s_cbranch_scc1 40f\n\t"
                "s_mov_b64 s[52:53], s[48:49]\n\t"
                "s_sub_u32 s50, s50, s46\n\t"
                "s_subb_u32 s51, s51, s47\n\t"
                "v_writelane_b32 %[raw], s44, m0\n\t"
                "s_add_u32 %[i], %[i], 1\n\t"
                "s_cmp_lt_u32 %[i], s54\n\t"
                "s_cbranch_scc0 2f\n\t"
                "16:\n\t"
                "s_lshr_b64 s[40:41], s[52:53], 24\n\t"
                "ds_read_b64 v[40:41], v50 offset:1536\n\t"
                "s_waitcnt lgkmcnt(2)\n\t"
                "v_mad_u64_u32 v[44:45], s[42:43], s40, v42, 0\n\t"
                "v_mad_u32_u24 v45, v42, s41, v45\n\t"
                "v_cmpx_ge_u64 vcc, s[50:51], v[44:45]\n\t"
                "v_mad_u64_u32 v[48:49], s[42:43], s40, v43, 0\n\t"
                "v_mad_u32_u24 v49, v43, s41, v49\n\t"
                "s_and_b32 m0, %[i], s62\n\t"
                "s_ff1_i32_b64 s44, vcc\n\t"
                "v_readfirstlane_b32 s48, v48\n\t"
                "v_readfirstlane_b32 s49, v49\n\t"
                "v_readfirstlane_b32 s46, v44\n\t"
                "v_readfirstlane_b32 s47, v45\n\t"
                "s_mov_b64 exec, -1\n\t"
                "s_cmp_eq_u32 s49, 0\n\t"
                "s_cbranch_scc1 41f\n\t"
                "s_mov_b64 s[52:53], s[48:49]\n\t"
                "s_sub_u32 s50, s50, s46\n\t"
                "s_subb_u32 s51, s51, s47\n\t"
                "v_writelane_b32 %[raw], s44, m0\n\t"
                "s_add_u32 %[i], %[i], 1\n\t"
                "s_cmp_lt_u32 %[i], s54\n\t"
                "s_cbranch_scc0 2f\n\t"
                "17:\n\t"
                "s_lshr_b64 s[40:41], s[52:53], 24\n\t"
                "ds_read_b64 v[42:43], v50 offset:2048\n\t"
                "s_waitcnt lgkmcnt(2)\n\t"
                "v_mad_u64_u32 v[44:45], s[42:43], s40, v46, 0\n\t"
                "v_mad_u32_u24 v45, v46, s41, v45\n\t"
                "v_cmpx_ge_u64 vcc, s[50:51], v[44:45]\n\t"
                "v_mad_u64_u32 v[48:49], s[42:43], s40, v47, 0\n\t"
                "v_mad_u32_u24 v49, v47, s41, v49\n\t"
                "s_and_b32 m0, %[i], s62\n\t"
                "s_ff1_i32_b64 s44, vcc\n\t"
                "v_readfirstlane_b32 s48, v48\n\t"
                "v_readfirstlane_b32 s49, v49\n\t"
                "v_readfirstlane_b32 s46, v44\n\t"
                "v_readfirstlane_b32 s47, v45\n\t"
                "s_mov_b64 exec, -1\n\t"
                "s_cmp_eq_u32 s49, 0\n\t"
                "s_cbranch_scc1 42f\n\t"
                "s_mov_b64 s[52:53], s[48:49]\n\t"
                "s_sub_u32 s50, s50, s46\n\t"
                "s_subb_u32 s51, s51, s47\n\t"
                "v_writelane_b32 %[raw], s44, m0\n\t"
                "s_add_u32 %[i], %[i], 1\n\t"
                "v_add_u32 v50, 0x600, v50\n\t"
                "s_cmp_lt_u32 %[i], s54\n\t"
                "s_cbranch_scc1 1b\n\t"
                "2:\n\t"
                "s_cmp_eq_u32 s65, 0\n\t"
                "s_cbranch_scc0 26f\n\t"
                "s_sub_u32 s58, s54, 1\n\t"
                "s_and_b32 s58, s58, s62\n\t"
                "s_add_u32 s58, s58, 1\n\t"
                "s_bfm_b64 exec, s58, 0\n\t"
                "v_sub_u32 v52, %[top], %[raw]\n\t"
                "v_add_u32 v52, 1, v52\n\t"
                "ds_write_b8 %[ring], v52\n\t"
                "global_store_byte %[goff], v52, %[lat]\n\t"
                "s_mov_b64 exec, -1\n\t"
                "ds_write_b32 v51, %[zero]\n\t"
                "s_add_u32 %[seq], %[seq], 1\n\t"
                "s_add_u32 s58, %[pix0], %[i]\n\t"
                "v_mov_b32 v56, %[seq]\n\t"
                "v_mov_b32 v57, s58\n\t"
                "ds_write_b64 %[rdy], v[56:57] offset:64\n\t"
                "s_branch 22f\n\t"
                "26:\n\t"
                "s_and_b32 s58, s67, s62\n\t"
                "s_sub_u32 s59, %[i], s67\n\t"
                "s_bfm_b64 exec, s59, s58\n\t"
                "v_sub_u32 v52, %[top], %[raw]\n\t"
                "v_add_u32 v52, 1, v52\n\t"
                "ds_write_b8 %[ring], v52\n\t"
                "global_store_byte %[goff], v52, %[lat]\n\t"
                "s_mov_b64 exec, -1\n\t"
                "s_add_u32 s58, %[pix0], %[i]\n\t"
                "v_mov_b32 v52, s58\n\t"
                "ds_write_b32 %[rdy], v52 offset:68\n\t"
                "126:\n\t"
                "s_cmp_lt_u32 %[i], s66\n\t"
                "s_cbranch_scc0 29f\n\t"
                "s_and_b32 s59, %[i], s62\n\t"
                "s_add_u32 s58, s59, s56\n\t"
                "v_lshl_add_u32 v50, s58, 9, %[tabl]\n\t"
                "s_lshr_b32 s59, s59, %[tshift]\n\t"
                "s_mov_b32 s67, %[i]\n\t"
                "s_add_u32 s54, %[i], s70\n\t"
                "s_add_u32 s54, s54, 1\n\t"
                "s_min_u32 s54, s54, s66\n\t"
                "s_mov_b32 s68, 0\n\t"
                "28:\n\t"
                "ds_read_b32 v52, v51\n\t"
                "ds_read_b32 %[top], v53\n\t"
                "ds_read_b32 %[ring], v53 offset:520\n\t"
                "ds_read_b32 %[goff], v53 offset:1040\n\t"
                "ds_read2st64_b64 v[40:43], v50 offset1:1\n\t"
                "s_waitcnt lgkmcnt(4)\n\t"
                "v_readfirstlane_b32 s58, v52\n\t"
                "s_bitcmp1_b32 s58, s59\n\t"
                "s_cbranch_scc1 27f\n\t"
                "s_add_u32 s68, s68, 1\n\t"
                "s_cmp_lt_u32 s68, 1024\n\t"
                "s_cbranch_scc1 28b\n\t"
                "s_branch 7f\n\t"
                "27:\n\t"
                "s_add_u32 %[spins], %[spins], s68\n\t"
                "s_sub_u32 s58, s54, %[i]\n\t"
                "s_cmp_eq_u32 s58, 8\n\t"
                "s_cbranch_scc1 420f\n\t"
                "s_cmp_eq_u32 s58, 4\n\t"
                "s_cbranch_scc0 31b\n\t"
                "s_and_b32 s58, %[i], s62\n\t"
                "s_cmp_eq_u32 s58, 4\n\t"
                "s_cbranch_scc1 450f\n\t"
                "s_cmp_eq_u32 s58, 8\n\t"
                "s_cbranch_scc1 460f\n\t"
                "s_cmp_eq_u32 s58, 12\n\t"
                "s_cbranch_scc1 470f\n\t"
                "s_branch 31b\n\t"
                "29:\n\t"
                "s_mov_b32 s65, 0\n\t"
                "ds_write_b32 v51, %[zero]\n\t"
                "s_add_u32 %[seq], %[seq], 1\n\t"
                "v_mov_b32 v52, %[seq]\n\t"
                "ds_write_b32 %[rdy], v52 offset:64\n\t"
                "s_branch 22f\n\t"
                "6:\n\t"
                "s_sub_u32 s58, %[i], 1\n\t"
                "s_sub_u32 s57, s69, 1\n\t"
                "s_andn2_b32 s58, s58, s57\n\t"
                "s_add_u32 s54, s58, s69\n\t"
                "s_min_u32 s54, s54, %[n]\n\t"
                "s_and_b32 s55, %[seq], %[smask]\n\t"
                "v_lshl_add_u32 v51, s55, 2, %[rdy]\n\t"
                "s_lshl_b32 s56, s55, %[bshift]\n\t"
                "s_sub_u32 s57, %[i], s58\n\t"
                "s_add_u32 s57, s57, s56\n\t"
                "s_lshl_b32 s57, s57, 9\n\t"
                "v_add_u32 v50, s57, %[tabl]\n\t"
                "v_lshl_add_u32 v53, s56, 2, %[l4]\n\t"
                "s_mov_b32 s65, 1\n\t"
                "s_mov_b32 s66, s54\n\t"
                "s_mov_b32 s67, s58\n\t"
                "s_sub_u32 s57, %[i], 1\n\t"
                "s_or_b32 s57, s57, s70\n\t"
                "s_add_u32 s57, s57, 1\n\t"
                "s_min_u32 s54, s57, s66\n\t"
                "s_mov_b32 s68, 0\n\t"
                "s_cmp_lt_u32 %[i], s54\n\t"
                "s_cbranch_scc1 8b\n\t"
                "s_branch 2b\n\t"
                "7:\n\t"
                "s_mov_b32 %[st], 2\n\t"
                "s_branch 4f\n\t"
                "40:\n\t"
                "s_cmp_eq_u32 s48, 0\n\t"
                "s_cbranch_scc1 14f\n\t"
                "s_sub_u32 s50, s50, s46\n\t"
                "s_subb_u32 s51, s51, s47\n\t"
                "s_and_b32 m0, %[i], s62\n\t"
                "v_writelane_b32 %[raw], s44, m0\n\t"
                "s_add_u32 %[i], %[i], 1\n\t"
                "s_sub_u32 s58, %[wpos], %[wbase]\n\t"
                "s_and_b32 s58, s58, 63\n\t"
                "v_readlane_b32 s57, %[wbuf], s58\n\t"
                "s_mov_b32 s51, s50\n\t"
                "s_mov_b32 s50, s57\n\t"
                "s_mov_b32 s53, s48\n\t"
                "s_mov_b32 s52, 0\n\t"
                "s_add_u32 %[wpos], %[wpos], 1\n\t"
                "s_cmp_eq_u32 s58, 63\n\t"
                "s_cbranch_scc1 15f\n\t"
                "s_cmp_lt_u32 %[i], s54\n\t"
                "s_cbranch_scc0 2b\n\t"
                "s_branch 16b\n\t"
                "41:\n\t"
                "s_cmp_eq_u32 s48, 0\n\t"
                "s_cbranch_scc1 14f\n\t"
                "s_sub_u32 s50, s50, s46\n\t"
                "s_subb_u32 s51, s51, s47\n\t"
                "s_and_b32 m0, %[i], s62\n\t"
                "v_writelane_b32 %[raw], s44, m0\n\t"
                "s_add_u32 %[i], %[i], 1\n\t"
                "s_sub_u32 s58, %[wpos], %[wbase]\n\t"
                "s_and_b32 s58, s58, 63\n\t"
                "v_readlane_b32 s57, %[wbuf], s58\n\t"
                "s_mov_b32 s51, s50\n\t"
                "s_mov_b32 s50, s57\n\t"
                "s_mov_b32 s53, s48\n\t"
                "s_mov_b32 s52, 0\n\t"
                "s_add_u32 %[wpos], %[wpos], 1\n\t"
                "s_cmp_eq_u32 s58, 63\n\t"
                "s_cbranch_scc1 15f\n\t"
                "s_cmp_lt_u32 %[i], s54\n\t"
                "s_cbranch_scc0 2b\n\t"
                "s_branch 17b\n\t"
                "42:\n\t"
                "s_cmp_eq_u32 s48, 0\n\t"
                "s_cbranch_scc1 14f\n\t"
                "s_sub_u32 s50, s50, s46\n\t"
                "s_subb_u32 s51, s51, s47\n\t"
                "s_and_b32 m0, %[i], s62\n\t"
                "v_writelane_b32 %[raw], s44, m0\n\t"
                "s_add_u32 %[i], %[i], 1\n\t"
                "s_sub_u32 s58, %[wpos], %[wbase]\n\t"
                "s_and_b32 s58, s58, 63\n\t"
                "v_readlane_b32 s57, %[wbuf], s58\n\t"
                "s_mov_b32 s51, s50\n\t"
                "s_mov_b32 s50, s57\n\t"
                "s_mov_b32 s53, s48\n\t"
                "s_mov_b32 s52, 0\n\t"
                "s_add_u32 %[wpos], %[wpos], 1\n\t"
                "s_cmp_eq_u32 s58, 63\n\t"
                "s_cbranch_scc1 15f\n\t"
                "v_add_u32 v50, 0x600, v50\n\t"
                "s_cmp_lt_u32 %[i], s54\n\t"
                "s_cbranch_scc0 2b\n\t"
                "s_branch 1b\n\t"
                ".p2align 6\n\t"
                "80:\n\t"
#include "ccd_dec_block16p.inc"
                "s_mov_b64 exec, 0xffff\n\t"
                "v_sub_u32 v52, %[top], %[raw]\n\t"
                "v_add_u32 v52, 1, v52\n\t"
                "ds_write_b8 %[ring], v52\n\t"
                "global_store_byte %[goff], v52, %[lat]\n\t"
                "s_mov_b64 exec, -1\n\t"
                "ds_write_b32 v51, %[zero]\n\t"
                "s_add_u32 %[seq], %[seq], 1\n\t"
                "s_add_u32 s58, %[pix0], %[i]\n\t"
                "v_mov_b32 v56, %[seq]\n\t"
                "v_mov_b32 v57, s58\n\t"
                "ds_write_b64 %[rdy], v[56:57] offset:64\n\t"
                "22:\n\t"
                "s_and_b32 s55, %[seq], %[smask]\n\t"
                "v_lshl_add_u32 v51, s55, 2, %[rdy]\n\t"
                "ds_read_b32 v54, v51\n\t"
                "s_lshl_b32 s56, s55, %[bshift]\n\t"
                "v_lshl_add_u32 v53, s56, 2, %[l4]\n\t"
                "ds_read_b32 %[top], v53\n\t"
                "ds_read_b32 %[ring], v53 offset:520\n\t"
                "ds_read_b32 %[goff], v53 offset:1040\n\t"
                "v_lshl_add_u32 v50, s56, 9, %[tabl]\n\t"
                "ds_read2st64_b64 v[40:43], v50 offset1:1\n\t"
                "s_add_u32 s54, %[i], s69\n\t"
                "s_cmp_le_u32 s54, s72\n\t"
                "s_cbranch_scc0 25f\n\t"
                "s_waitcnt lgkmcnt(4)\n\t"
                "v_readfirstlane_b32 s59, v54\n\t"
                "s_cmp_eq_u32 s59, s73\n\t"
                "s_cbranch_scc1 80b\n\t"
                "s_mov_b32 s57, s73\n\t"
                "s_branch 23f\n\t"
                "25:\n\t"
                "s_cmp_lt_u32 %[i], %[n]\n\t"
                "s_cbranch_scc0 30f\n\t"
                "s_add_u32 s54, %[i], s69\n\t"
                "s_min_u32 s54, s54, %[n]\n\t"
                "24:\n\t"
                "s_sub_u32 s58, s54, %[i]\n\t"
                "s_add_u32 s57, s58, s70\n\t"
                "s_lshr_b32 s57, s57, %[tshift]\n\t"
                "s_bfm_b32 s57, s57, 0\n\t"
                "s_waitcnt lgkmcnt(4)\n\t"
                "v_readfirstlane_b32 s59, v54\n\t"
                "s_cmp_eq_u32 s59, s57\n\t"
                "s_cbranch_scc0 23f\n\t"
                "s_cmp_eq_u32 s58, 16\n\t"
                "s_cbranch_scc1 80b\n\t"
                "s_branch 31b\n\t"
                "23:\n\t"
                "s_mov_b32 s68, 0\n\t"
                "s_branch 11b\n\t"
                "30:\n\t"
                "s_add_u32 %[pix0], %[pix0], %[n]\n\t"
                "s_sub_u32 %[cleft], %[cleft], 1\n\t"
                "s_cmp_eq_u32 %[cleft], 0\n\t"
                "s_cbranch_scc1 10f\n\t"
                "s_add_u32 %[x0], %[x0], 1\n\t"
                "s_cmp_eq_u32 %[x0], %[gw]\n\t"
                "s_cselect_b32 %[x0], s64, %[x0]\n\t"
                "s_cselect_b32 s60, 1, 0\n\t"
                "s_sub_u32 %[hy], %[hy], s60\n\t"
                "s_mul_i32 s60, %[x0], 0xcccd\n\t"
                "s_lshr_b32 s60, s60, 19\n\t"
                "s_add_u32 s60, s60, 1\n\t"
                "s_min_u32 %[n], s60, %[hy]\n\t"
                "s_mul_i32 s72, %[n], s61\n\t"
                "s_mov_b32 %[i], 0\n\t"
                "s_min_u32 s54, s69, %[n]\n\t"
                "s_branch 24b\n\t"
                "10:\n\t"
                "s_mov_b32 %[st], 0\n\t"
                "s_branch 4f\n\t"
#include "ccd_dec_tramp16p.inc"
#include "ccd_dec_parts8.inc"
#include "ccd_dec_parts4.inc"
                "15:\n\t"
                "s_mov_b32 %[st], 3\n\t"
                "s_branch 4f\n\t"
                "14:\n\t"
                "s_mov_b32 %[st], 1\n\t"
                "4:\n\t"
                "s_mov_b32 %[kr], s44\n\t"
                "s_mov_b64 %[dst], s[50:51]\n\t"
                "s_mov_b64 %[rng], s[52:53]\n\t"
                "s_waitcnt lgkmcnt(0)\n\t"
                : [dst] "+s"(rc_dist), [rng] "+s"(rc_range), [i] "+s"(i), [seq] "+s"(seq), [raw] "+v"(raw), [top] "+v"(top_l),
                  [ring] "+v"(v_ring), [goff] "+v"(v_goff), [spins] "+s"(n_spins), [wpos] "+s"(word_pos), [st] "=s"(status), [kr] "=s"(k_rare),
                  [n] "+s"(n_step), [x0] "+s"(step_x0), [hy] "+s"(step_hy), [cleft] "+s"(steps_left),
                  [pix0] "+s"(pix0), [npart] "+s"(n_part)
                : [mode] "s"(mode), [gw] "s"(static_cast<uint32_t>(grid_w)), [smask] "s"(static_cast<uint32_t>(slot_mask)),
                  [bshift] "s"(bpx_shift), [tshift] "s"(static_cast<uint32_t>(task_shift)),
                  [rdy] "v"(ready_base), [zero] "v"(0u),
                  [wbuf] "v"(wbuf), [wbase] "s"(wbase), [tabl] "v"(tab_lane), [lane] "v"(static_cast<uint32_t>(lane)),
                  [l4] "v"(lane_top_off), [lat] "s"(lat_addr)
                : "memory", "vcc", "scc", "m0", "s40", "s41", "s42", "s43", "s44", "s46", "s47", "s48", "s49", "s50", "s51", "s52", "s53", "s54", "s55",
                  "s56", "s57", "s58", "s59", "s60", "s61", "s62", "s63", "s64", "s65", "s66", "s67", "s68", "s69", "s70", "s71", "s72", "s73", "s74", "s75", "s76", "s77", "s78", "s79", "s80", "v40", "v41", "v42", "v43", "v44", "v45", "v46", "v47", "v48", "v49", "v50", "v51", "v52", "v53", "v54", "v55", "v56", "v57", "v58", "v59", "v60", "v61");
#pragma clang diagnostic pop
            if (status == 0) break;
            if (status == 3) {
                wbase = word_pos;
                wbuf = (wbase + lane < n_words) ? words_g[wbase + lane] : 0u;
                mode = 1;
                continue;
            }
            const int i0 = static_cast<int>(i & ~static_cast<uint32_t>(bpx - 1));
            const int slot = uni(static_cast<int>(seq) & slot_mask);
            const int row0 = slot * bpx;
            if (status == 2) {
                const int cnt = min(bpx, static_cast<int>(n_step) - i0);
                const uint32_t n_parts = static_cast<uint32_t>((cnt + task_pix - 1) >> task_shift);
#ifdef CCD_PIPE_PROFILE
                const unsigned long long ts = __builtin_amdgcn_s_memtime();
#endif
                if (!wait_ge(&C.s_ready[slot], (1u << n_parts) - 1u, C.s_abort)) { ok = false; break; }
#ifdef CCD_PIPE_PROFILE
                const unsigned long long dts = __builtin_amdgcn_s_memtime() - ts;
                S.stall_ticks += dts;
                S.stall_events += 1;
                if (n_step >= 48) S.wait_by_j[min(i0 / bpx, 5)] += dts;
#endif
                __builtin_amdgcn_fence(__ATOMIC_ACQUIRE, "workgroup");
                mode = (i & static_cast<uint32_t>(bpx - 1)) ? 1u : 0u;
                continue;
            }
            S.n_rare += 1;
            const int pi = static_cast<int>(i) - i0;
            const uint2* tab = C.s_tab + static_cast<size_t>(row0) * 64 + lane;
            const uint2 cur = tab[pi * 64];
            const uint32_t sc_lo = static_cast<uint32_t>(rc_range >> 24);
            const uint32_t sc_hi = static_cast<uint32_t>(rc_range >> 56);
            const uint64_t p0 = static_cast<uint64_t>(sc_lo) * cur.x;
            const uint32_t p_lo = static_cast<uint32_t>(p0);
            const uint32_t p_hi = static_cast<uint32_t>(p0 >> 32) + __umul24(sc_hi, cur.x);
            int k = static_cast<int>(k_rare);
            const uint32_t l_lo = static_cast<uint32_t>(__builtin_amdgcn_readlane(p_lo, k));
            const uint32_t l_hi = static_cast<uint32_t>(__builtin_amdgcn_readlane(p_hi, k));
            const uint32_t psel = static_cast<uint32_t>(__builtin_amdgcn_readlane(cur.y, k));
            uint64_t nd = rc_dist - ((static_cast<uint64_t>(l_hi) << 32) | l_lo);
            uint64_t nr = static_cast<uint64_t>(sc_lo) * psel + (static_cast<uint64_t>(sc_hi * psel) << 32);
            if (nr == 0) {
                S.n_search += 1;
                const uint64_t scale = rc_range >> kRcPrecision;
                if ((rc_dist >> kRcPrecision) >= scale) {
                    lds_write_release(C.s_abort, static_cast<uint32_t>(-CCD_ERR_INVALID_DATA));
                    ok = false;
                    break;
                }
                const double mu = -64.0 + static_cast<double>(meta.mu_idx[row0 + pi]) * (1.0 / 256.0);
                const double rcp = meta.rcp[row0 + pi];
                const uint32_t f0 = window_left(mu, rcp, kAcLo + lane, C.s_exp);
                const uint32_t f1 = window_left(mu, rcp, kAcLo + 64 + lane, C.s_exp);
                const unsigned long long m0 = __ballot(scale * f0 <= rc_dist), m1 = __ballot(scale * f1 <= rc_dist);
                const int sidx = __popcll(m0) + __popcll(m1) - 1;
                const uint32_t left = uni(static_cast<uint32_t>(__shfl(sidx < 64 ? f0 : f1, sidx & 63)));
                uint32_t right = uni(static_cast<uint32_t>(__shfl(sidx + 1 < 64 ? f0 : f1, (sidx + 1) & 63)));
                if (sidx == kAlphabet - 1) right = 1u << kRcPrecision;
                nd = rc_dist - scale * left;
                nr = scale * static_cast<uint64_t>(right - left);
                k = uni(1 - ((sidx + kAcLo) - meta.top[row0 + pi]));
            }
            if (static_cast<uint32_t>(nr >> 32) == 0) {
                nr <<= 32;
                nd = (nd << 32) | static_cast<uint32_t>(__builtin_amdgcn_readlane(wbuf, (word_pos - wbase) & 63));
                ++word_pos;
                if (word_pos - wbase == 64) { wbase = word_pos; wbuf = (wbase + lane < n_words) ? words_g[wbase + lane] : 0u; }
            }
            rc_dist = uni(nd); rc_range = uni(nr);
            asm volatile("s_mov_b32 m0, %2\n\tv_writelane_b32 %0, %1, m0" : "+v"(raw) : "s"(k), "s"(pi));
            ++i;
            mode = 1;
        }
    }
    S.dist = rc_dist; S.range = rc_range; S.word_pos = word_pos; S.wbase = wbase; S.wbuf = wbuf;
    S.n_spins += n_spins;
    S.n_part_batches += n_part;
    return seq;
}

__device__ __forceinline__ void mad64(int64_t& acc, int32_t x, int32_t w) {
    acc += static_cast<int64_t>(x) * static_cast<int64_t>(w);
    asm("" : "+v"(acc));
}
__device__ __forceinline__ int32_t relu_q16(int64_t a) {
    return static_cast<int32_t>(a >> 16) & ~static_cast<int32_t>(a >> 63);
}
#define CCD_MAD4(ACC, X, Wv, NCH)                                                   \
    _Pragma("unroll") for (int g_ = 0; g_ < (NCH); ++g_) mad64(ACC[g_], (X).x, Wv[g_].x); \
    _Pragma("unroll") for (int g_ = 0; g_ < (NCH); ++g_) mad64(ACC[g_], (X).y, Wv[g_].y); \
    _Pragma("unroll") for (int g_ = 0; g_ < (NCH); ++g_) mad64(ACC[g_], (X).z, Wv[g_].z); \
    _Pragma("unroll") for (int g_ = 0; g_ < (NCH); ++g_) mad64(ACC[g_], (X).w, Wv[g_].w);
#define CCD_MAD4_PAIR(ACC, ACC2, X, Wv)                                             \
    mad64(ACC[0], (X).x, Wv[0].x); mad64(ACC2, (X).y, Wv[0].y); mad64(ACC[0], (X).z, Wv[0].z); mad64(ACC2, (X).w, Wv[0].w);
__device__ __forceinline__ void mad64_seq(int64_t& acc, int32_t x, int32_t w) {
    mad64(acc, x, w);
    __builtin_amdgcn_sched_barrier(0);
}
#define CCD_MAD4_SEQ(ACC, X, Wv, NCH)                                               \
    _Pragma("unroll") for (int g_ = 0; g_ < (NCH); ++g_) mad64_seq(ACC[g_], (X).x, Wv[g_].x); \
    _Pragma("unroll") for (int g_ = 0; g_ < (NCH); ++g_) mad64_seq(ACC[g_], (X).y, Wv[g_].y); \
    _Pragma("unroll") for (int g_ = 0; g_ < (NCH); ++g_) mad64_seq(ACC[g_], (X).z, Wv[g_].z); \
    _Pragma("unroll") for (int g_ = 0; g_ < (NCH); ++g_) mad64_seq(ACC[g_], (X).w, Wv[g_].w);
#define CCD_MAD4_PAIR_SEQ(ACC, ACC2, X, Wv)                                         \
    mad64_seq(ACC[0], (X).x, Wv[0].x); mad64_seq(ACC2, (X).y, Wv[0].y); mad64_seq(ACC[0], (X).z, Wv[0].z); mad64_seq(ACC2, (X).w, Wv[0].w);

typedef int i32x4 __attribute__((ext_vector_type(4)));
constexpr long long kMfMaxDigits3 = 0x7F7F7F;
constexpr long long kMfMaxDigits2 = 0x7F7F;
constexpr int kMfLayer1 = 8;
constexpr int kMfHidden = 10;
constexpr int kMfOut = 5;
__host__ __device__ constexpr int mf_tables(int n_layers) { return kMfLayer1 + (n_layers - 2) * kMfHidden + kMfOut; }

__device__ __forceinline__ uint32_t mf_byte(int32_t w, int j) {
    const uint32_t d = (static_cast<uint32_t>(w) + 0x00808080u) ^ 0x00808080u;
    return (j < 0 || j > 2) ? 0u : ((d >> (8 * j)) & 0xffu);
}
__device__ __forceinline__ int mf_slot_input(bool first, int g, int beta, int n_sp, int n_if, int dim, int* limb) {
    if (first) {
        if (beta < 8) { *limb = 0; const int k = g + 4 * beta; return k < n_sp ? k : -1; }
        if (beta < 12) { *limb = (beta - 8) & 1; const int f = g + 4 * ((beta - 8) >> 1); return f < n_if ? n_sp + f : -1; }
        return -1;
    }
    if (beta >= 15) return -1;
    const int a = beta / 3;
    *limb = beta - 3 * a;
    const int k = a < 4 ? 4 * g + a : 16 + g;
    return k < dim ? k : -1;
}
__device__ __forceinline__ i32x4 mf_pack15(const int32_t (&a)[5]) {
    uint32_t d[5];
#pragma unroll
    for (int i = 0; i < 5; ++i) d[i] = ((static_cast<uint32_t>(a[i]) + 0x00808080u) ^ 0x00808080u) & 0x00ffffffu;
    i32x4 r;
    r[0] = static_cast<int>(d[0] | (d[1] << 24));
    r[1] = static_cast<int>((d[1] >> 8) | (d[2] << 16));
    r[2] = static_cast<int>((d[2] >> 16) | (d[3] << 8));
    r[3] = static_cast<int>(d[4]);
    return r;
}
__device__ __forceinline__ int64_t mf_comb4(const i32x4 (&c)[4], int r, int64_t bias) {
    const int32_t lo = c[0][r] + (c[1][r] << 8), hi = c[2][r] + (c[3][r] << 8);
    return bias + (static_cast<int64_t>(lo) << 16) + (static_cast<int64_t>(hi) << 32);
}
__device__ __forceinline__ int64_t mf_comb5(const i32x4 (&c)[5], int r, int64_t bias) {
    const int32_t lo = c[0][r] + (c[1][r] << 8), mid = c[2][r] + (c[3][r] << 8);
    return bias + lo + (static_cast<int64_t>(mid) << 16) + (static_cast<int64_t>(c[4][r]) << 32);
}

__device__ void mf_build_tables(const PipeCtx& C, int in_pad, uint32_t* s_a_words, int tid) {
    const int dim = C.dim, n_layers = C.n_layers, n_sp = C.n_sp, n_if = C.n_if;
    const int n_tab = mf_tables(n_layers);
    for (int e = tid; e < n_tab * 256; e += kPipeThreads) {
        const int idx = e >> 8, ln = (e >> 2) & 63, dw = e & 3, m = ln & 15, g = ln >> 4;
        int layer, tile, s;
        if (idx < kMfLayer1) { layer = 0; tile = idx >> 2; s = idx & 3; }
        else {
            const int j = idx - kMfLayer1, hl = j / kMfHidden;
            if (hl < n_layers - 2) { layer = 1 + hl; tile = (j - hl * kMfHidden) / 5; s = (j - hl * kMfHidden) % 5; }
            else { layer = n_layers - 1; tile = 0; s = j - (n_layers - 2) * kMfHidden; }
        }
        const int32_t* row = nullptr;
        if (layer == n_layers - 1) { if (m < 2) row = C.s_w + C.n_w_hidden + m * in_pad; }
        else {
            int o = -1;
            if (tile == 0) o = m;
            else if ((m & 3) == 0) o = 16 + (m >> 2);
            if (o >= 0 && o < dim) row = C.s_w + layer * dim * in_pad + o * in_pad;
            if (layer == 0 && tile == 1 && (m == 1 || m == 2)) row = C.s_w + C.n_w_hidden + 2 * in_pad + (m - 1) * in_pad;
        }
        uint32_t word = 0;
        if (row)
            for (int bb = 0; bb < 4; ++bb) {
                int limb = 0;
                const int k = mf_slot_input(layer == 0, g, dw * 4 + bb, n_sp, n_if, dim, &limb);
                if (k >= 0) word |= mf_byte(row[k], s - limb) << (8 * bb);
            }
        s_a_words[e] = word;
    }
}

template <int NV>
__device__ __forceinline__ void mf_exact_task(const PipeCtx& C, int32_t* tile, int n, int y, int x, int W, int fin, int fw, int feat_plane,
                                              int ring_mask, int64_t& out_mu, int64_t& out_ls) {
    constexpr int in_pad = 4 * NV;
    const EntropyParams& P = *C.P;
    const int dim = C.dim, n_layers = C.n_layers, n_sp = C.n_sp;
    int32_t* ain = tile + n * in_pad;
    int32_t* aout = tile + (8 + n) * in_pad;
#pragma unroll 1
    for (int k = 0; k < dim; ++k) {
        int32_t v = 0;
        if (k < n_sp) {
            const int yy = y - P.ctx_dy[k], xx = x + P.ctx_dx[k];
            if (yy >= 0 && xx >= 0 && xx < W) v = C.s_ring[ring_cell(yy, xx, ring_mask)];
        } else if (fin > 0) {
            v = reinterpret_cast<const int16_t*>(P.ifce_feat)[((y >> 1) * fw + (x >> 1)) * C.fstride + (k - n_sp)];
        }
        ain[k] = v << 16;
    }
    int64_t stab[2];
#pragma unroll
    for (int o = 0; o < 2; ++o) {
        int64_t acc = C.s_b[(n_layers - 1) * dim + 2 + o];
        const int32_t* w = C.s_w + C.n_w_hidden + 2 * in_pad + o * in_pad;
#pragma unroll 1
        for (int k = 0; k < dim; ++k) acc += static_cast<int64_t>(ain[k]) * w[k];
        stab[o] = acc;
    }
#pragma unroll 1
    for (int l = 0; l < n_layers - 1; ++l) {
#pragma unroll 1
        for (int o = 0; o < dim; ++o) {
            int64_t acc = C.s_b[l * dim + o];
            const int32_t* w = C.s_w + l * dim * in_pad + o * in_pad;
#pragma unroll 1
            for (int k = 0; k < dim; ++k) acc += static_cast<int64_t>(ain[k]) * w[k];
            aout[o] = static_cast<int32_t>((acc < 0 ? 0 : acc) >> 16);
        }
        int32_t* t = ain; ain = aout; aout = t;
    }
#pragma unroll
    for (int o = 0; o < 2; ++o) {
        int64_t acc = C.s_b[(n_layers - 1) * dim + o] + stab[o];
        const int32_t* w = C.s_w + C.n_w_hidden + o * in_pad;
#pragma unroll 1
        for (int k = 0; k < dim; ++k) acc += static_cast<int64_t>(ain[k]) * w[k];
        if (o == 0) out_mu = acc; else out_ls = acc;
    }
}

constexpr int16_t kFeatSentinel = -32768;

struct ExactArgs {
    const EntropyParams* P;
    uint32_t s_w, s_b, s_ring;
    int n_w_hidden, dim, n_layers, n_sp, in_pad;
    int W, fin, fw, feat_plane, ring_mask, fstride;
};
struct ExactOut { int64_t mu, ls; };
__device__ __forceinline__ ExactOut exact_pixel(const ExactArgs& A, int y, int x) {
    const EntropyParams& P = *A.P;
    const int lane = threadIdx.x & 63;
    const int dim = A.dim, n_layers = A.n_layers, n_sp = A.n_sp, in_pad = A.in_pad;
    const int32_t* s_w = reinterpret_cast<const int32_t*>(ccd_pipe_smem + A.s_w);
    const int64_t* s_b = reinterpret_cast<const int64_t*>(ccd_pipe_smem + A.s_b);
    const int8_t* s_ring = reinterpret_cast<const int8_t*>(ccd_pipe_smem + A.s_ring);
    uint64_t xin = 0;
    if (lane < dim) {
        int64_t v = 0;
        if (lane < n_sp) {
            const int yy = y - P.ctx_dy[lane], xx = x + P.ctx_dx[lane];
            if (yy >= 0 && xx >= 0 && xx < A.W) v = s_ring[ring_cell(yy, xx, A.ring_mask)];
        } else if (A.fin > 0) {
            const int pos = (y >> 1) * A.fw + (x >> 1);
            v = reinterpret_cast<const int16_t*>(P.ifce_feat)[pos * A.fstride + (lane - n_sp)];
            if (v == kFeatSentinel) v = static_cast<int64_t>(static_cast<float>(P.ifce_wide[(lane - n_sp) * A.feat_plane + pos]));
        }
        xin = static_cast<uint64_t>(v) << 16;
    }
    auto bcast = [&](uint64_t v, int k) {
        const uint32_t lo = static_cast<uint32_t>(__shfl(static_cast<int>(static_cast<uint32_t>(v)), k));
        const uint32_t hi = static_cast<uint32_t>(__shfl(static_cast<int>(static_cast<uint32_t>(v >> 32)), k));
        return (static_cast<uint64_t>(hi) << 32) | lo;
    };
    auto layer = [&](const int32_t* wt, const int64_t* bias, int n_out, uint64_t xv) {
        const int o = min(lane, n_out - 1);
        uint64_t acc = static_cast<uint64_t>(bias[o]);
#pragma unroll 1
        for (int k = 0; k < dim; ++k) acc += bcast(xv, k) * static_cast<uint64_t>(static_cast<int64_t>(wt[o * in_pad + k]));
        return acc;
    };
    const uint64_t stab = layer(s_w + A.n_w_hidden + 2 * in_pad, s_b + (n_layers - 1) * dim + 2, 2, xin);
    uint64_t xv = xin;
#pragma unroll 1
    for (int l = 0; l < n_layers - 1; ++l) {
        const int64_t a = static_cast<int64_t>(layer(s_w + l * dim * in_pad, s_b + l * dim, dim, xv));
        xv = static_cast<uint64_t>((a < 0 ? 0 : a) >> 16);
    }
    const uint64_t out = layer(s_w + A.n_w_hidden, s_b + (n_layers - 1) * dim, 2, xv) + stab;
    ExactOut r;
    r.mu = static_cast<int64_t>(bcast(out, 0));
    r.ls = static_cast<int64_t>(bcast(out, 1));
    return r;
}

template <int CTRL>
__device__ __forceinline__ int64_t dpp_add64(int64_t v) {
    const uint32_t lo = static_cast<uint32_t>(__builtin_amdgcn_mov_dpp(static_cast<int>(v), CTRL, 0xf, 0xf, true));
    const uint32_t hi = static_cast<uint32_t>(__builtin_amdgcn_mov_dpp(static_cast<int>(v >> 32), CTRL, 0xf, 0xf, true));
    typedef unsigned int u32x2 __attribute__((ext_vector_type(2)));
    const u32x2 other = {lo, hi};
    return v + __builtin_bit_cast(int64_t, other);
}
__device__ __forceinline__ int64_t dpp_add64_row_below(int64_t v) {
    const uint32_t lo = static_cast<uint32_t>(__builtin_amdgcn_update_dpp(0, static_cast<int>(v), 0x142, 0xa, 0xf, false));
    const uint32_t hi = static_cast<uint32_t>(__builtin_amdgcn_update_dpp(0, static_cast<int>(v >> 32), 0x142, 0xa, 0xf, false));
    typedef unsigned int u32x2 __attribute__((ext_vector_type(2)));
    const u32x2 other = {lo, hi};
    return v + __builtin_bit_cast(int64_t, other);
}
template <int LANES>
__device__ __forceinline__ void group_sum2(int64_t& a, int64_t& b) {
    static_assert(LANES == 8 || LANES == 16 || LANES == 32, "a pixel's lane group: part of a DPP row, a row, or two rows");
    a = dpp_add64<0xB1>(a); b = dpp_add64<0xB1>(b);
    a = dpp_add64<0x4E>(a); b = dpp_add64<0x4E>(b);
    a = dpp_add64<0x141>(a); b = dpp_add64<0x141>(b);
    if constexpr (LANES >= 16) { a = dpp_add64<0x140>(a); b = dpp_add64<0x140>(b); }
    if constexpr (LANES == 32) { a = dpp_add64_row_below(a); b = dpp_add64_row_below(b); }
}
__device__ __forceinline__ int32_t table_index(int64_t sum, int32_t off, int32_t hi) {
    const int32_t h = min(max(static_cast<int32_t>(sum >> 32), -(1 << 22)), 1 << 22);
    const int32_t x = static_cast<int32_t>((static_cast<uint32_t>(h) << 8) | (static_cast<uint32_t>(sum) >> 24));
    return min(max(x + off, 0), hi);
}
static_assert(kMuOffset < (1 << 29) && kScaleOffset < (1 << 29) && kMuOffset >= 0 && kScaleOffset >= 0, "table_index: offsets");
static_assert(offsetof(RowMeta, top) - offsetof(RowMeta, mu_idx) == (kRows + 2) * 4, "a pixel's top symbol is stored (kRows + 2) words behind its mu index");

#if defined(CCD_PIPE_PROFILE)
constexpr int kProfLevel = CCD_PIPE_PROFILE;
#else
constexpr int kProfLevel = 0;
#endif
struct TaskClock {
    enum Phase { kWait, kGather, kMlp, kStab, kHidden, kOut, kTables, kPhases };
    unsigned long long* prof;
    bool p0;
    unsigned long long a = 0, b = 0, c = 0, d = 0, prev_end = 0, t[kPhases];
    __device__ __forceinline__ TaskClock(unsigned long long* prof_, int pw) : prof(prof_), p0(pw == 0) {}
    __device__ __forceinline__ unsigned long long stamp() const { return (kProfTrace || p0) ? __builtin_amdgcn_s_memtime() : 0ull; }
    __device__ __forceinline__ void task_begin() { if constexpr (kProfLevel == 2) { a = stamp(); if (p0 && prev_end) prof[4] += a - prev_end; } }
    __device__ __forceinline__ void early_wait_end() { if constexpr (kProfLevel == 2) b = stamp(); }
    __device__ __forceinline__ void late_wait_begin() { if constexpr (kProfLevel == 2) c = stamp(); }
    __device__ __forceinline__ void late_wait_end() { if constexpr (kProfLevel == 2) d = stamp(); }
    __device__ __forceinline__ void task_end(const PipeCtx& C, uint32_t W, uint32_t steps_left, uint32_t gidx, uint32_t word0, uint32_t px_ahead) {
        if constexpr (kProfLevel == 2) {
            const unsigned long long e = __builtin_amdgcn_s_memtime();
#if defined(CCD_PIPE_TRACE)
            if ((threadIdx.x & 63) == 0 && W == uni(g_trace_cfg[0]) && uni(g_trace_cfg[1]) - steps_left < 64u) {
                typedef unsigned int u32x4 __attribute__((ext_vector_type(4)));
                u32x4* r = reinterpret_cast<u32x4*>(ccd_pipe_smem + C.trace_off + (gidx % kTraceTasks) * 32u);
                r[0] = u32x4{word0, static_cast<uint32_t>(a), static_cast<uint32_t>(b), static_cast<uint32_t>(c)};
                r[1] = u32x4{static_cast<uint32_t>(d), static_cast<uint32_t>(e), px_ahead, static_cast<uint32_t>(a >> 32)};
            }
#endif
            if (p0) { prof[0] += b - a; prof[1] += c - b; prof[2] += d - c; prof[3] += e - d; prof[8] += 1; prev_end = e; }
        }
    }
    __device__ __forceinline__ void begin(Phase p) { if constexpr (kProfLevel >= 3) t[p] = __builtin_amdgcn_s_memtime(); }
    __device__ __forceinline__ void add(int k, Phase p) { if constexpr (kProfLevel >= 3) prof[k] += __builtin_amdgcn_s_memtime() - t[p]; }
    __device__ __forceinline__ void sub(int k, Phase p) { if constexpr (kProfLevel >= 3) prof[k] -= __builtin_amdgcn_s_memtime() - t[p]; }
    __device__ __forceinline__ void count_task() { if constexpr (kProfLevel >= 3) prof[8] += 1; }
};
__device__ __forceinline__ void store_row_position(RowMeta& meta, int row, int y, int x, int W, int ring_mask) {
    meta.cell[row] = static_cast<uint32_t>(ring_cell(y, x, ring_mask));
    meta.goff[row] = static_cast<uint32_t>(y * W + x);
}
__device__ __forceinline__ void publish_ready(uint32_t rdy_addr, uint32_t rdy_val) {
    asm volatile("" ::: "memory");
    unsigned long long exec_all;
    asm volatile("s_mov_b64 %0, exec\n\ts_mov_b64 exec, 1\n\tds_or_b32 %1, %2\n\ts_mov_b64 exec, %0"
                 : "=&s"(exec_all) : "v"(rdy_addr), "v"(rdy_val) : "memory");
}
template <int NV, int kLpp, bool MF, bool DYN_RING, bool DYN, class SH>
__device__ __forceinline__ uint32_t producer_grid(const PipeCtx& C_run, unsigned long long* prof, const GridSeg& seg) {
    constexpr int in_pad = 4 * NV;
    static_assert(!SH::fixed || (!MF && SH::dim <= in_pad && SH::dim > in_pad - 4 && SH::n_sp >= 1 && SH::n_layers >= 2), "ShapeFix: vector-ALU path, matching width");
    PipeCtx C_fix = C_run;
    if constexpr (SH::fixed) {
        constexpr PipeLayout L = pipe_layout(SH::dim, SH::n_layers, in_pad, kRingRows, 0);
        C_fix.s_ring.off = L.ring; C_fix.s_w.off = L.w; C_fix.s_b.off = L.b; C_fix.s_act.off = L.act; C_fix.s_a.off = L.a; C_fix.s_tab.off = L.tab;
        C_fix.s_meta.off = L.meta; C_fix.s_rcp.off = L.rcp; C_fix.s_exp.off = L.exp; C_fix.s_ready.off = L.ready; C_fix.s_consumed.off = L.consumed;
        C_fix.s_abort.off = L.abort; C_fix.n_w_hidden = L.n_w_hidden; C_fix.ring_mask = kRingRows - 1;
#if defined(CCD_PIPE_TRACE)
        C_fix.trace_off = L.end;
#endif
        C_fix.dim = SH::dim; C_fix.n_layers = SH::n_layers; C_fix.n_sp = SH::n_sp; C_fix.k_left = 0;
    }
    const PipeCtx& C = C_fix;
    constexpr int kTaskPix = 64 / kLpp;
    constexpr int kBpx = kTaskPix == 2 ? 8 : 16;
    constexpr int kHalves = kBpx / kTaskPix;
    constexpr int kNSlots = kRows / kBpx;
    constexpr int NOUT = (in_pad + kLpp - 1) / kLpp;
    const int lane = threadIdx.x & 63;
    const int pw = uni(static_cast<int>(threadIdx.x >> 6) - 1);
    const EntropyParams& P = *C.P;
    const int dim = SH::fixed ? SH::dim : uni(C.dim), n_layers = SH::fixed ? SH::n_layers : uni(C.n_layers), n_sp = SH::fixed ? SH::n_sp : uni(C.n_sp);
    const int W = uni(C.W);
    const int k_left = SH::fixed ? 0 : uni(C.k_left), fin = uni(C.fin), fw = uni(C.fw);
    const uint32_t seq_base = uni(C.seq_base);
    int32_t* act = C.s_act + pw * ((DYN_RING ? 16 : 8) * in_pad + 4);
    [[maybe_unused]] int32_t* const act_dummy = act + (DYN_RING ? 16 : 8) * in_pad;
    const int px = MF ? (lane & 15) : lane / kLpp;
    const int q = MF ? (lane >> 4) : lane % kLpp;
    const int ring_mask = DYN_RING ? uni(C.ring_mask) : kRingRows - 1;
    [[maybe_unused]] const int n_if = uni(C.n_if), mf_bits = uni(P.mfma);
    const int4* act_row = reinterpret_cast<const int4*>(act + px * in_pad);
    int ctx_dy_l[NOUT], ctx_dx_l[NOUT];
#pragma unroll
    for (int t = 0; t < NOUT; ++t) {
        const int k = q + kLpp * t;
        ctx_dy_l[t] = k < n_sp ? P.ctx_dy[k] : 0;
        ctx_dx_l[t] = k < n_sp ? P.ctx_dx[k] : 0;
    }
    const glb_ptr<const int16_t> ifce_feat = (glb_ptr<const int16_t>)reinterpret_cast<const int16_t*>(P.ifce_feat);
    const int feat_plane = uni(C.fh) * fw;
    const int fstride = SH::fixed ? feat_stride(SH::dim - SH::n_sp) : uni(C.fstride);
    [[maybe_unused]] int32_t mf_dxy[8], mf_wl[7];
    if constexpr (MF) {
#pragma unroll
        for (int t = 0; t < 8; ++t) {
            const int k = q + 4 * t;
            mf_dxy[t] = k < n_sp ? static_cast<int32_t>((static_cast<uint32_t>(P.ctx_dy[k]) << 16) | (static_cast<uint32_t>(P.ctx_dx[k]) & 0xffffu)) : 0;
        }
#pragma unroll
        for (int r = 0; r < 7; ++r) {
            const int o = r < 4 ? 4 * q + r : 16 + q;
            int32_t w = 0;
            if (k_left >= 0) {
                if (r < 5) w = o < dim ? C.s_w[o * in_pad + k_left] : 0;
                else w = C.s_w[C.n_w_hidden + 2 * in_pad + (r - 5) * in_pad + k_left];
            }
            mf_wl[r] = w;
        }
    }
    TaskClock clk(prof, pw);
    constexpr uint32_t kTaskShift = kTaskPix == 8 ? 3 : (kTaskPix == 4 ? 2 : 1), kBpxShift = kBpx == 32 ? 5 : (kBpx == 16 ? 4 : 3), kHalvesShift = kBpxShift - kTaskShift;
    StepWalk it;
    it.init(static_cast<uint32_t>(uni(C.H)), static_cast<uint32_t>(W));
    uint32_t seq = seq_base;
    uint32_t pix0 = uni(C.px_base), prev_pix0 = pix0, prev2_pix0 = pix0, prev_moved = 0;
    const uint32_t seg_first = uni(seg.first), seg_steps = uni(seg.steps);
    const bool seg_body = uni(seg.body ? 1 : 0) != 0;
    if (seg_first > 0u) {
        it.seek_before(seg_first);
        pix0 += uni(seg.pix_before);
        prev_pix0 = pix0 - it.n;
        prev2_pix0 = prev_pix0 - (seg_first > 1u ? it.len_of(seg_first - 2u) : 0u);
        prev_moved = it.moved;
    }
    uint32_t phase = static_cast<uint32_t>((static_cast<unsigned long long>(seq_base) * kHalves) % kProducers);
    const bool split = k_left >= 0 && W > 9 && n_layers >= 2;
    const uint32_t n_steps_total = wf_n_steps(it.H, it.W);
    const uint32_t seg_end = seg_first + seg_steps;
    const auto walk_on = [&]() {
        prev2_pix0 = prev_pix0; prev_pix0 = pix0; pix0 += it.n; prev_moved = it.moved;
        const uint32_t nx = it.x0 + 1u, mv = nx == it.W ? 1u : 0u;
        it.x0 = mv ? it.W - kWfSlope : nx; it.y0 += mv; it.moved = mv; --it.left;
        it.n = min(it.H - it.y0, wf_div10(it.x0) + 1u);
    };
    while (n_steps_total - it.left < seg_end && it.next()) {
        const uint32_t seg_n = seg_body ? uni(seg.n_pix) : it.n;
        const uint32_t seg_pix0 = pix0;
        const uint32_t nb = (seg_n + kBpx - 1) >> kBpxShift;
        const uint32_t n_tasks = (seg_n + kTaskPix - 1) >> kTaskShift;
        const uint32_t seq0 = seq;
        uint32_t t_first = static_cast<uint32_t>(pw) - phase;
        t_first += static_cast<int32_t>(t_first) < 0 ? kProducers : 0;
        {
            for (uint32_t task = t_first; task < n_tasks; task += kProducers) {
                const uint32_t j = task >> kHalvesShift;
                const int half = static_cast<int>(task & (kHalves - 1));
                seq = seq0 + j;
                const int slot = static_cast<int>(seq & (kNSlots - 1));
                const int i0 = static_cast<int>(task << kTaskShift);
                const int cnt = min(kTaskPix, static_cast<int>(seg_n) - i0);
                while (seg_pix0 + static_cast<uint32_t>(i0) >= pix0 + it.n) walk_on();
                const uint32_t ia = seg_pix0 + static_cast<uint32_t>(i0) - pix0;
                const uint32_t n_a = min(static_cast<uint32_t>(cnt), it.n - ia);
                const uint32_t bx1 = it.x0 + 1u, b_moved = bx1 == static_cast<uint32_t>(W) ? 1u : 0u;
                const uint32_t bx0 = b_moved ? static_cast<uint32_t>(W) - kWfSlope : bx1, by0 = it.y0 + b_moved;
                const bool in_b = static_cast<uint32_t>(px) >= n_a;
                const int ii = in_b ? px - static_cast<int>(n_a) : static_cast<int>(ia) + px;
                const int y = static_cast<int>(in_b ? by0 : it.y0) + ii, x = static_cast<int>(in_b ? bx0 : it.x0) - kWfSlope * ii;
                const uint32_t dy1 = it.moved, dy2 = it.moved + prev_moved;
                const uint32_t prev_n = pix0 - prev_pix0, prev2_n = prev_pix0 - prev2_pix0;
                uint32_t f_raw[NOUT];
                bool f_has[NOUT];
                if constexpr (!MF) {
                    const int fo = (y >> 1) * fw + (x >> 1);
#pragma unroll
                    for (int t = 0; t < NOUT; ++t) {
                        const int k = q + kLpp * t;
                        f_has[t] = fin > 0 && px < cnt && k >= n_sp && k < dim;
                        f_raw[t] = reinterpret_cast<glb_ptr<const uint16_t>>(ifce_feat)[f_has[t] ? fo * fstride + (k - n_sp) : 0];
                    }
                } else {
#pragma unroll
                    for (int t = 0; t < NOUT; ++t) { f_raw[t] = 0; f_has[t] = false; }
                }
                unsigned long long bad_lanes = 0ull;
                const uint32_t need_slot = seq >= static_cast<uint32_t>(kNSlots) ? seq - kNSlots + 1 : 0;
                const bool ends_in_b = n_a < static_cast<uint32_t>(cnt);
                const uint32_t last1 = ends_in_b ? static_cast<uint32_t>(cnt) - n_a : ia + static_cast<uint32_t>(cnt);
                const uint32_t need_px = ends_in_b ? pix0 + min(last1 + b_moved, it.n) : prev_pix0 + min(last1 + dy1, prev_n);
                const uint32_t need_early_px = ends_in_b ? prev_pix0 + min(last1 + b_moved + dy1, prev_n)
                                                         : prev2_pix0 + min(last1 + dy2, prev2_n);
                uint32_t win_left_m = 0, win_keep_m = 0, win_e0 = 0, win_e1 = 0;
                constexpr int kQ0 = kLpp == 32 ? 16 : 0;
                constexpr int kEpl = kLpp == 8 ? 2 : 1;
                const int e0 = kEpl * (q & 15);
                int32_t idx_mu = 0, idx_sc = 0;
                double own_rcp = 0.0;
                uint32_t own_ent = 0;
                uint32_t mu_dst = 0, rcp_dst = 0;
                uint32_t rdy_addr = 0, rdy_val = 0;
                unsigned narrow_mask = 0;
                unsigned long long wide_lanes = 0ull;
                RowMeta& meta = *C.s_meta;
                if constexpr (MF) {
                    const int n = px, g = q;
                    const bool live = n < cnt;
                    int32_t f0 = 0, f1 = 0;
                    if (live && fin > 0) {
                        const int fo = (y >> 1) * fw + (x >> 1);
                        if (g < n_if) f0 = ifce_feat[fo * fstride + g];
                        if (g + 4 < n_if) f1 = ifce_feat[fo * fstride + g + 4];
                    }
                    clk.a = LPROF_T(pw == 0);
#if defined(CCD_PIPE_PROFILE) && CCD_PIPE_PROFILE == 2
                    if (pw == 0 && clk.prev_end) prof[4] += clk.a - clk.prev_end;
#endif
                    {
                        const unsigned long long t0 = PROF_T();
                        if (!wait_ge2(C.s_consumed, need_slot, split ? need_early_px : need_px, C.s_abort)) return seq;
                        PROF_ADD(prof[0], t0);
                    }
                    clk.b = LPROF_T(pw == 0);
                    const unsigned long long t_g = PROF_T();
                    {
                        const int mi = (g == 0 && live) ? slot * kBpx + half * kTaskPix + n : kRows;
                        meta.cell[mi] = static_cast<uint32_t>(ring_cell(y, x, ring_mask));
                        meta.goff[mi] = static_cast<uint32_t>(y * W + x);
                    }
                    uint32_t w0 = 0, w1 = 0;
#pragma unroll
                    for (int t = 0; t < 8; ++t) {
                        if (4 * t < n_sp) {
                            const int k = g + 4 * t;
                            const int yy = y - (mf_dxy[t] >> 16), xx = x + static_cast<int16_t>(mf_dxy[t] & 0xffff);
                            const bool take = live && k < n_sp && yy >= 0 && xx >= 0 && xx < W && !(split && k == k_left);
                            const int cell = take ? ring_cell(yy, xx, ring_mask) : 0;
                            int32_t v = C.s_ring[cell];
                            v = take ? v : 0;
                            if (t < 4) w0 |= static_cast<uint32_t>(v & 0xff) << (8 * t);
                            else w1 |= static_cast<uint32_t>(v & 0xff) << (8 * (t - 4));
                        }
                    }
                    const uint32_t d0 = (static_cast<uint32_t>(f0) + 0x8080u) ^ 0x8080u, d1 = (static_cast<uint32_t>(f1) + 0x8080u) ^ 0x8080u;
                    const i32x4 bop = {static_cast<int>(w0), static_cast<int>(w1), static_cast<int>((d0 & 0xffffu) | (d1 << 16)), 0};
                    PROF_ADD(prof[1], t_g);
                    const unsigned long long t_m = PROF_T();
                    const i32x4* sa = reinterpret_cast<const i32x4*>(static_cast<uint32_t*>(C.s_a)) + lane;
                    const i32x4 zero4 = {0, 0, 0, 0};
                    int64_t pre[5], st0, st1;
                    {
                        i32x4 c1[2][4];
#pragma unroll
                        for (int t = 0; t < 2; ++t)
#pragma unroll
                            for (int s = 0; s < 4; ++s) c1[t][s] = __builtin_amdgcn_mfma_i32_16x16x64_i8(sa[(t * 4 + s) * 64], bop, zero4, 0, 0, 0);
                        const int64_t* bl = C.s_b;
#pragma unroll
                        for (int r = 0; r < 4; ++r) {
                            const int o = 4 * g + r;
                            const int64_t bias = bl[min(o, dim - 1)];
                            pre[r] = mf_comb4(c1[0], r, o < dim ? bias : 0);
                        }
                        {
                            const int64_t bias = bl[min(16 + g, dim - 1)];
                            pre[4] = mf_comb4(c1[1], 0, 16 + g < dim ? bias : 0);
                        }
                        st0 = mf_comb4(c1[1], 1, bl[(n_layers - 1) * dim + 2]);
                        st1 = mf_comb4(c1[1], 2, bl[(n_layers - 1) * dim + 3]);
                    }
                    const i32x4* sl_out = sa + (kMfLayer1 + (n_layers - 2) * kMfHidden) * 64;
                    i32x4 a_h[10], a_o[5];
                    int64_t b_h[5];
                    if (n_layers > 2) {
#pragma unroll
                        for (int s = 0; s < 10; ++s) a_h[s] = sa[(kMfLayer1 + s) * 64];
#pragma unroll
                        for (int r = 0; r < 5; ++r) {
                            const int o = r < 4 ? 4 * g + r : 16 + g;
                            const int64_t bias = C.s_b[dim + min(o, dim - 1)];
                            b_h[r] = o < dim ? bias : 0;
                        }
                    }
#pragma unroll
                    for (int s = 0; s < 5; ++s) a_o[s] = sl_out[s * 64];
                    const int64_t b_mu = C.s_b[(n_layers - 1) * dim], b_ls = C.s_b[(n_layers - 1) * dim + 1];
                    PROF_ADD(prof[4], t_m);
                    int32_t xleft = 0;
                    clk.c = LPROF_T(pw == 0);
                    if (split) {
                        const unsigned long long t0 = PROF_T();
                        if (!wait_ge(C.s_consumed + 1, need_px, C.s_abort)) return seq;
                        PROF_ADD(prof[0], t0);
                        PROF_SUB(prof[2], t0);
                        PROF_ADD(prof[5], t0);
                        if (live && x >= 1) xleft = static_cast<int32_t>(C.s_ring[ring_cell(y, x - 1, ring_mask)]) << 16;
                    }
                    clk.d = LPROF_T(pw == 0);
                    const unsigned long long t_h = PROF_T();
                    int32_t av[5];
                    uint32_t big = 0;
                    uint32_t over = 0;
#pragma unroll
                    for (int r = 0; r < 5; ++r) {
                        mad64(pre[r], xleft, mf_wl[r]);
                        const int64_t a = pre[r] < 0 ? 0 : pre[r];
                        av[r] = static_cast<int32_t>(a >> 16);
                        big |= static_cast<uint32_t>(av[r]); over |= static_cast<uint32_t>(av[r]) + 0x00808080u;
                    }
                    mad64(st0, xleft, mf_wl[5]);
                    mad64(st1, xleft, mf_wl[6]);
                    for (int l = 1; l < n_layers - 1; ++l) {
                        const i32x4 b2 = mf_pack15(av);
                        i32x4 c2[5], c2b[5];
#pragma unroll
                        for (int s = 0; s < 5; ++s) c2[s] = __builtin_amdgcn_mfma_i32_16x16x64_i8(a_h[s], b2, zero4, 0, 0, 0);
                        if (dim > 16) {
#pragma unroll
                            for (int s = 0; s < 5; ++s) c2b[s] = __builtin_amdgcn_mfma_i32_16x16x64_i8(a_h[5 + s], b2, zero4, 0, 0, 0);
                        }
#pragma unroll
                        for (int r = 0; r < 4; ++r) {
                            const int64_t a = mf_comb5(c2, r, b_h[r]);
                            av[r] = static_cast<int32_t>((a < 0 ? 0 : a) >> 16);
                            big |= static_cast<uint32_t>(av[r]); over |= static_cast<uint32_t>(av[r]) + 0x00808080u;
                        }
                        av[4] = 0;
                        if (dim > 16) {
                            const int64_t a = mf_comb5(c2b, 0, b_h[4]);
                            av[4] = static_cast<int32_t>((a < 0 ? 0 : a) >> 16);
                            big |= static_cast<uint32_t>(av[4]); over |= static_cast<uint32_t>(av[4]) + 0x00808080u;
                        }
                        if (l + 1 < n_layers - 1) {
                            const i32x4* sl = sa + (kMfLayer1 + l * kMfHidden) * 64;
#pragma unroll
                            for (int s = 0; s < 10; ++s) a_h[s] = sl[s * 64];
#pragma unroll
                            for (int r = 0; r < 5; ++r) {
                                const int o = r < 4 ? 4 * g + r : 16 + g;
                                const int64_t bias = C.s_b[(l + 1) * dim + min(o, dim - 1)];
                                b_h[r] = o < dim ? bias : 0;
                            }
                        }
                    }
                    PROF_ADD(prof[6], t_h);
                    const unsigned long long t_o = PROF_T();
                    int64_t out_mu, out_ls;
                    {
                        const i32x4 b3 = mf_pack15(av);
                        i32x4 c3[5];
#pragma unroll
                        for (int s = 0; s < 5; ++s) c3[s] = __builtin_amdgcn_mfma_i32_16x16x64_i8(a_o[s], b3, zero4, 0, 0, 0);
                        out_mu = mf_comb5(c3, 0, b_mu) + st0;
                        out_ls = mf_comb5(c3, 1, b_ls) + st1;
                    }
                    if (__ballot(((big >> mf_bits) | (over >> 24)) != 0u) != 0ull) {
                        if (g == 0 && live) mf_exact_task<NV>(C, act, n, y, x, W, fin, fw, feat_plane, ring_mask, out_mu, out_ls);
                        if (lane == 0) atomicAdd(reinterpret_cast<int*>(P.status) + 39, 1);
                    }
                    const int64_t m8 = (out_mu >> 24) + kMuOffset, s8 = (out_ls >> 24) + kScaleOffset;
                    const int32_t idx_mu = static_cast<int32_t>(m8 < 0 ? 0 : (m8 > kNumMu - 1 ? kNumMu - 1 : m8));
                    const int32_t idx_sc = static_cast<int32_t>(s8 < 0 ? 0 : (s8 > kNumScale - 1 ? kNumScale - 1 : s8));
                    const int mpx = slot * kBpx + half * kTaskPix + n;
                    if (g == 0 && live) {
                        meta.mu_idx[mpx] = idx_mu;
                        meta.rcp[mpx] = C.s_rcp[idx_sc];
                    }
                    narrow_mask = static_cast<unsigned>(__ballot(g == 0 && live && idx_sc <= kNarrowMaxScale)) & 0xffffu;
                    PROF_ADD(prof[2], t_m);
                    PROF_ADD(prof[7], t_o);
#if defined(CCD_PIPE_PROFILE) && CCD_PIPE_PROFILE >= 3
                    prof[8] += 1;
#endif
                    clk.begin(TaskClock::kTables);
                } else {
                clk.task_begin();
                int32_t hid[NOUT];
                clk.begin(TaskClock::kWait);
                if (!wait_ge2(C.s_consumed, need_slot, split ? need_early_px : need_px, C.s_abort)) return seq;
                clk.add(0, TaskClock::kWait);
                clk.early_wait_end();
                clk.begin(TaskClock::kGather);
                store_row_position(meta, (q == 0 && px < cnt) ? slot * kBpx + half * kTaskPix + px : kRows, y, x, W, ring_mask);
                {
                    typedef unsigned int u32x4 __attribute__((ext_vector_type(4)));
                    const u32x4 z4 = {0u, 0u, 0u, 0u};
                    uint2* const tab0 = C.s_tab + static_cast<size_t>(slot * kBpx + half * kTaskPix) * 64;
#pragma unroll
                    for (int j = 0; j < (kTaskPix * 24 + 63) / 64; ++j) {
                        const int t = lane + 64 * j, row = t / 24, e2 = t - 24 * row;
                        uint2* const dst = row < cnt ? &tab0[row * 64 + 16 + 2 * e2] : C.s_tab + kRows * 64 + 16 + 2 * (e2 % 24);
                        *reinterpret_cast<u32x4*>(dst) = z4;
                    }
                }
                {
                    int32_t rr[NOUT];
#pragma unroll
                    for (int t = 0; t < NOUT; ++t) {
                        const int yy = y - ctx_dy_l[t], xx = x + ctx_dx_l[t];
                        rr[t] = C.s_ring[ring_cell(yy, xx, ring_mask)];
                    }
                    if constexpr (NOUT == 1) asm volatile("" : "+v"(rr[0]));
                    else if constexpr (NOUT == 2) asm volatile("" : "+v"(rr[0]), "+v"(rr[1]));
                    else if constexpr (NOUT == 3) asm volatile("" : "+v"(rr[0]), "+v"(rr[1]), "+v"(rr[2]));
                    else if constexpr (NOUT == 4) asm volatile("" : "+v"(rr[0]), "+v"(rr[1]), "+v"(rr[2]), "+v"(rr[3]));
                    else {
#pragma unroll
                        for (int t = 0; t < NOUT; ++t) asm volatile("" : "+v"(rr[t]));
                    }
                    int32_t fv[NOUT];
                    bool feat_bad = false;
#pragma unroll
                    for (int t = 0; t < NOUT; ++t) {
                        asm volatile("" : "+v"(f_raw[t]));
                        fv[t] = f_has[t] ? static_cast<int32_t>(static_cast<int16_t>(f_raw[t])) : 0;
                        feat_bad |= DYN && fv[t] == kFeatSentinel;
                    }
                    if constexpr (DYN) bad_lanes = __ballot(feat_bad);
#pragma unroll
                    for (int t = 0; t < NOUT; ++t) {
                        const int k = q + kLpp * t;
                        const int yy = y - ctx_dy_l[t], xx = x + ctx_dx_l[t];
                        const int32_t v = k < n_sp ? ((yy >= 0 && xx >= 0 && xx < W && !(split && k == k_left)) ? rr[t] : 0) : fv[t];
                        int32_t* const dst = k < in_pad ? act + px * in_pad + k : act_dummy;
                        *dst = v << 16;
                        hid[t] = v << 16;
                    }
                }
                clk.add(1, TaskClock::kGather);
                clk.begin(TaskClock::kMlp);
                int4 xv[NV];
#pragma unroll
                for (int v = 0; v < NV; ++v) xv[v] = act_row[v];
                clk.add(4, TaskClock::kMlp);
                clk.begin(TaskClock::kStab);
                int64_t so[2];
                const int qs = q < 2 ? q : 1;
                {
                    const int4* wr = reinterpret_cast<const int4*>(C.s_w + C.n_w_hidden + 2 * in_pad + qs * in_pad);
                    so[0] = C.s_b[(n_layers - 1) * dim + 2 + qs];
                    so[1] = 0;
                    int4 wv[NV];
#pragma unroll
                    for (int v = 0; v < NV; ++v) wv[v] = wr[v];
#pragma unroll
                    for (int v = 0; v < NV; ++v) {
                        const int4 w = wv[v];
                        mad64(so[0], xv[v].x, w.x); mad64(so[1], xv[v].y, w.y); mad64(so[0], xv[v].z, w.z); mad64(so[1], xv[v].w, w.w);
                    }
                }
                clk.add(5, TaskClock::kStab);
                clk.begin(TaskClock::kHidden);
                int64_t acc0[NOUT];
                [[maybe_unused]] int64_t acc0_b = 0;
                int32_t wleft[NOUT], wleft_stab = 0;
                if (n_layers >= 2) {
                    const int32_t* wl = C.s_w;
                    const int64_t* bl = C.s_b;
                    const int4* wr[NOUT];
                    const int kl = split ? k_left : 0;
#pragma unroll
                    for (int t = 0; t < NOUT; ++t) {
                        const int oc = min(q + kLpp * t, dim - 1);
                        wr[t] = reinterpret_cast<const int4*>(wl + oc * in_pad);
                        acc0[t] = bl[oc];
                        wleft[t] = wl[oc * in_pad + kl];
                    }
                    wleft_stab = C.s_w[C.n_w_hidden + 2 * in_pad + qs * in_pad + kl];
                    int4 w[NOUT], wn[NOUT];
#pragma unroll
                    for (int t = 0; t < NOUT; ++t) w[t] = wr[t][0];
#pragma unroll
                    for (int v = 0; v < NV; ++v) {
                        if (v + 1 < NV) {
#pragma unroll
                            for (int t = 0; t < NOUT; ++t) wn[t] = wr[t][v + 1];
                        }
                        if constexpr (NOUT == 1) { CCD_MAD4_PAIR(acc0, acc0_b, xv[v], w) } else { CCD_MAD4(acc0, xv[v], w, NOUT) }
#pragma unroll
                        for (int t = 0; t < NOUT; ++t) w[t] = wn[t];
                    }
                    if constexpr (NOUT == 1) acc0[0] += acc0_b;
                }
                int32_t xleft = 0;
                int qo = q;
                asm volatile("" : "+v"(qo));
                const int mpx = slot * kBpx + half * kTaskPix + px;
                mu_dst = lds_addr(&meta.mu_idx[px < cnt && qo == kQ0 ? mpx : kRows]);
                rcp_dst = lds_addr(&meta.rcp[px < cnt && qo == kQ0 + 1 ? mpx : kRows]);
                int32_t wide_above = px < cnt && qo == kQ0 + 1 ? kNarrowMaxScale : 0x7fffffff;
                asm volatile("" : "+v"(mu_dst), "+v"(rcp_dst), "+v"(wide_above));
                int64_t out_m = 0, out_l = 0;
                int32_t wl_m = 0, wl_l = 0, wo_m[NOUT], wo_l[NOUT];
                {
                    const int64_t s = so[0] + so[1] + C.s_b[(n_layers - 1) * dim + qs];
                    const int64_t keep_m = qo == 0 ? -1 : 0, keep_l = qo == 1 ? -1 : 0;
                    out_m = s & keep_m;
                    out_l = s & keep_l;
                    wl_m = wleft_stab & static_cast<int32_t>(keep_m);
                    wl_l = wleft_stab & static_cast<int32_t>(keep_l);
                    asm volatile("" : "+v"(out_m), "+v"(out_l), "+v"(wl_m), "+v"(wl_l));
                    const int32_t* const w_out = C.s_w + C.n_w_hidden;
#pragma unroll
                    for (int t = 0; t < NOUT; ++t) {
                        const int o = qo + kLpp * t, oc = min(o, in_pad - 1);
                        const int32_t keep = (o - dim) >> 31;
                        wo_m[t] = w_out[oc] & keep;
                        wo_l[t] = w_out[in_pad + oc] & keep;
                        asm volatile("" : "+v"(wo_m[t]), "+v"(wo_l[t]));
                    }
                }
                rdy_addr = lds_addr(&C.s_ready[slot]);
                rdy_val = 1u << half;
                asm volatile("" : "+v"(rdy_addr), "+v"(rdy_val));
                const int e0o = kEpl * (qo & 15);
                own_ent = lds_addr(&C.s_tab[static_cast<size_t>(px < cnt && qo >= kQ0 ? mpx : kRows) * 64 + e0o]);
                win_left_m = e0o + kEpl - 1 == 15 ? 0u : ~0u;
                win_keep_m = (e0o == 0 || e0o == 15) ? 0u : ~0u;
                win_e0 = e0o == 0 ? (1u << kRcPrecision) - 1u : 0u;
                win_e1 = (e0o <= 1 && e0o + kEpl > 1) ? 1u : 0u;
                asm volatile("" : "+v"(own_ent), "+v"(win_left_m), "+v"(win_keep_m), "+v"(win_e0), "+v"(win_e1));
                clk.late_wait_begin();
                if (split) {
                    clk.begin(TaskClock::kWait);
                    const uint32_t want = uni(need_px);
                    const uint32_t cell = static_cast<uint32_t>(ring_cell(y, x - 1, ring_mask));
                    uint32_t seen_v;
                    int32_t r;
                    asm volatile("ds_read_b32 %0, %2 offset:4\n\tds_read_i8 %1, %3\n\ts_waitcnt lgkmcnt(0)"
                                 : "=&v"(seen_v), "=&v"(r) : "v"(C.s_consumed.off), "v"(C.s_ring.off + cell) : "memory");
                    if (__builtin_expect(static_cast<int32_t>(uni(seen_v) - want) < 0, 0)) {
                        unsigned spins = 0;
                        do {
                            if ((++spins & 1023u) == 0) {
                                if (lds_load_acquire(C.s_abort) != 0) return seq;
                                if (spins > kSpinLimit) { lds_write_release(C.s_abort, static_cast<uint32_t>(-CCD_ERR_HIP)); return seq; }
                            }
                            asm volatile("ds_read_b32 %0, %2 offset:4\n\tds_read_i8 %1, %3\n\ts_waitcnt lgkmcnt(0)"
                                         : "=&v"(seen_v), "=&v"(r) : "v"(C.s_consumed.off), "v"(C.s_ring.off + cell) : "memory");
                        } while (static_cast<int32_t>(uni(seen_v) - want) < 0);
                    }
                    clk.add(0, TaskClock::kWait);
                    clk.sub(2, TaskClock::kWait);
                    clk.sub(6, TaskClock::kWait);
                    xleft = (px < cnt && x >= 1) ? r << 16 : 0;
                }
                clk.late_wait_end();
                __builtin_amdgcn_s_setprio(1);
                mad64(out_m, xleft, wl_m);
                mad64(out_l, xleft, wl_l);
                if (n_layers >= 2) {
#pragma unroll
                    for (int t = 0; t < NOUT; ++t) {
                        mad64(acc0[t], xleft, wleft[t]);
                        hid[t] = relu_q16(acc0[t]);
                    }
                    if (n_layers > 2) {
#pragma unroll
                        for (int t = 0; t < NOUT; ++t) {
                            const int o = q + kLpp * t;
                            int32_t* const dst = o < dim ? act + px * in_pad + o : act_dummy;
                            *dst = hid[t];
                        }
#pragma unroll
                        for (int v = 0; v < NV; ++v) xv[v] = act_row[v];
                    }
                }
                for (int l = 1; l < n_layers - 1; ++l) {
                    const int32_t* wl = C.s_w + l * dim * in_pad;
                    const int64_t* bl = C.s_b + l * dim;
                    int64_t acc[NOUT];
                    [[maybe_unused]] int64_t acc_b = 0;
                    const int4* wr[NOUT];
#pragma unroll
                    for (int t = 0; t < NOUT; ++t) {
                        const int oc = min(q + kLpp * t, dim - 1);
                        wr[t] = reinterpret_cast<const int4*>(wl + oc * in_pad);
                        acc[t] = bl[oc];
                    }
                    int4 w[NOUT], wn[NOUT];
#pragma unroll
                    for (int t = 0; t < NOUT; ++t) w[t] = wr[t][0];
#pragma unroll
                    for (int v = 0; v < NV; ++v) {
                        if (v + 1 < NV) {
#pragma unroll
                            for (int t = 0; t < NOUT; ++t) wn[t] = wr[t][v + 1];
                        }
                        if constexpr (NOUT == 1) { CCD_MAD4_PAIR_SEQ(acc, acc_b, xv[v], w) } else { CCD_MAD4_SEQ(acc, xv[v], w, NOUT) }
#pragma unroll
                        for (int t = 0; t < NOUT; ++t) w[t] = wn[t];
                    }
                    if constexpr (NOUT == 1) acc[0] += acc_b;
#pragma unroll
                    for (int t = 0; t < NOUT; ++t) {
                        hid[t] = relu_q16(acc[t]);
                        asm("" : "+v"(hid[t]));
                    }
                    if (l + 2 < n_layers) {
#pragma unroll
                        for (int t = 0; t < NOUT; ++t) {
                            const int o = q + kLpp * t;
                            int32_t* const dst = o < dim ? act + px * in_pad + o : act_dummy;
                            *dst = hid[t];
                        }
#pragma unroll
                        for (int v = 0; v < NV; ++v) xv[v] = act_row[v];
                    }
                }
                clk.add(6, TaskClock::kHidden);
                clk.begin(TaskClock::kOut);
#pragma unroll
                for (int t = 0; t < NOUT; ++t) { mad64_seq(out_m, hid[t], wo_m[t]); mad64_seq(out_l, hid[t], wo_l[t]); }
                group_sum2<kLpp>(out_m, out_l);
                idx_mu = table_index(out_m, kMuOffset, kNumMu - 1);
                idx_sc = table_index(out_l, kScaleOffset, kNumScale - 1);
                own_rcp = C.s_rcp[idx_sc];
                if (DYN && __builtin_expect(bad_lanes != 0ull, 0)) {
                    int n_redo = 0;
                    for (int p = 0; p < cnt; ++p) {
                        if (((bad_lanes >> (p * kLpp)) & ((1ull << kLpp) - 1ull)) == 0ull) continue;
                        ExactArgs A;
                        A.P = C.P; A.s_w = uni(C.s_w.off); A.s_b = uni(C.s_b.off); A.s_ring = uni(C.s_ring.off);
                        A.n_w_hidden = uni(C.n_w_hidden); A.dim = dim; A.n_layers = n_layers; A.n_sp = n_sp; A.in_pad = in_pad;
                        A.W = W; A.fin = fin; A.fw = fw; A.feat_plane = feat_plane; A.ring_mask = ring_mask; A.fstride = fstride;
                        asm volatile("" : "+s"(A.P), "+s"(A.s_w), "+s"(A.s_b), "+s"(A.s_ring), "+s"(A.n_w_hidden), "+s"(A.dim), "+s"(A.n_layers));
                        asm volatile("" : "+s"(A.n_sp), "+s"(A.W), "+s"(A.fin), "+s"(A.fw), "+s"(A.feat_plane), "+s"(A.ring_mask), "+s"(A.fstride));
                        const ExactOut r = exact_pixel(A, __builtin_amdgcn_readlane(y, MF ? p : p * kLpp), __builtin_amdgcn_readlane(x, MF ? p : p * kLpp));
                        if (px == p) {
                            idx_mu = table_index(r.mu, kMuOffset, kNumMu - 1);
                            idx_sc = table_index(r.ls, kScaleOffset, kNumScale - 1);
                            own_rcp = C.s_rcp[idx_sc];
                        }
                        ++n_redo;
                    }
                    if (lane == 0) atomicAdd(reinterpret_cast<int*>(P.status) + 39, n_redo);
                }
                wide_lanes = __ballot(idx_sc > wide_above);
                clk.add(2, TaskClock::kMlp);
                clk.add(7, TaskClock::kOut);
                clk.count_task();
                clk.begin(TaskClock::kTables);
                }
                const int base = slot * kBpx + half * kTaskPix;
                uint2* tab = C.s_tab + static_cast<size_t>(base) * 64;
                if constexpr (!MF) {
                    {
                        int top = ((idx_mu + 128) >> 8) - 64 + 6;
                        top = max(kAcLo + 13, min(kAcLo + kAlphabet - 1, top));
                        lds_at<int32_t>(mu_dst)[0] = idx_mu;
                        lds_at<int32_t>(mu_dst)[kRows + 2] = top;
                        const double rcp256 = window_rcp256(own_rcp);
                        *lds_at<double>(rcp_dst) = own_rcp;
                        const bool at_top = top == kAcLo + kAlphabet - 1;
                        const uint32_t hi_f = at_top ? win_e0 : 0u, to_full = at_top ? win_e1 : 0u;
                        uint32_t left[kEpl];
#pragma unroll
                        for (int j = 0; j < kEpl; ++j) {
                            const int ssym = top - (e0 + j - 1);
                            uint32_t lo_m = static_cast<uint32_t>((kAcLo - ssym) >> 31);
                            if (j == kEpl - 1) lo_m &= win_left_m;
                            uint32_t l = window_cum_d256(window_d256(idx_mu, ssym), rcp256, C.s_exp) + static_cast<uint32_t>(ssym - kAcLo);
                            l = min(l, (1u << kRcPrecision) - 1u);
                            if (j == 0) l |= hi_f;
                            left[j] = l & lo_m;
                            if (j + 1 < kEpl) __builtin_amdgcn_sched_barrier(0);
                        }
                        const uint32_t right = static_cast<uint32_t>(__builtin_amdgcn_update_dpp(0, static_cast<int>(left[kEpl - 1]), 0x111, 0xf, 0xf, false));
                        if constexpr (kEpl == 1) {
                            typedef unsigned int u32x2 __attribute__((ext_vector_type(2)));
                            const u32x2 ent = {left[0], (right - left[0] + to_full) & win_keep_m};
                            *lds_at<u32x2>(own_ent) = ent;
                        } else {
                            typedef unsigned int u32x4 __attribute__((ext_vector_type(4)));
                            const u32x4 ent = {left[0], (right - left[0]) & win_keep_m, left[1], (left[0] - left[1] + to_full) & win_left_m};
                            *lds_at<u32x4>(own_ent) = ent;
                        }
                    }
                }
                unsigned rest = MF ? narrow_mask : 0u;
                while (rest) {
                    int pix[4];
                    int n_here = 0;
#pragma unroll
                    for (int u = 0; u < 4; ++u) {
                        pix[u] = rest ? __builtin_ctz(rest) : -1;
                        if (rest) { rest &= rest - 1; ++n_here; }
                    }
                    const int u = lane >> 4, e = lane & 15;
                    const int mine = u == 0 ? pix[0] : (u == 1 ? pix[1] : (u == 2 ? pix[2] : pix[3]));
                    const int mi = base + (mine < 0 ? pix[0] : mine);
                    const int mu_idx = meta.mu_idx[mi];
                    int top = ((mu_idx + 128) >> 8) - 64 + 6;
                    top = max(kAcLo + 13, min(kAcLo + kAlphabet - 1, top));
                    const double mu = -64.0 + static_cast<double>(mu_idx) * (1.0 / 256.0);
                    const int ssym = top - (e - 1);
                    uint32_t left = min(window_left(mu, meta.rcp[mi], ssym, C.s_exp), (1u << kRcPrecision) - 1u);
                    left = e == 15 ? 0u : left;
                    const uint32_t right = static_cast<uint32_t>(__builtin_amdgcn_update_dpp(0, static_cast<int>(left), 0x111, 0xf, 0xf, false));
                    uint2 ent;
                    ent.x = left;
                    ent.y = (e == 0 || e == 15) ? 0u : ((e == 1 && ssym == kAcLo + kAlphabet - 1) ? (1u << kRcPrecision) - left : right - left);
                    if (mine >= 0) {
                        tab[mine * 64 + e] = ent;
                        if (e == 0) meta.top[mi] = top;
                    }
                    if constexpr (MF) {
                        typedef unsigned int u32x4 __attribute__((ext_vector_type(4)));
                        const u32x4 z4 = {0u, 0u, 0u, 0u};
#pragma unroll
                        for (int j = 0; j < 2; ++j) {
                            const int t = lane + 64 * j;
                            const int ru = t >= 72 ? 3 : (t >= 48 ? 2 : (t >= 24 ? 1 : 0));
                            const int rp = ru == 0 ? pix[0] : (ru == 1 ? pix[1] : (ru == 2 ? pix[2] : pix[3]));
                            if (t < 96 && rp >= 0) *reinterpret_cast<u32x4*>(&tab[rp * 64 + 16 + 2 * (t - 24 * ru)]) = z4;
                        }
                    }
                    (void)n_here;
                }
                unsigned long long wide = MF ? static_cast<unsigned long long>(((1u << cnt) - 1u) & ~narrow_mask) : wide_lanes;
                while (wide) {
                    const int bit = __builtin_ctzll(wide);
                    wide &= wide - 1;
                    const int i = MF ? bit : bit / kLpp;
                    const int mi = base + i;
                    const int mu_idx = meta.mu_idx[mi];
                    int top = ((mu_idx + 128) >> 8) - 64 + 30;
                    top = max(kAcLo + 61, min(kAcLo + kAlphabet - 1, top));
                    const int ssym = top - (lane - 1);
                    uint32_t left = min(window_left_d256(window_d256(mu_idx, ssym), window_rcp256(meta.rcp[mi]), ssym, C.s_exp), (1u << kRcPrecision) - 1u);
                    left = lane == 63 ? 0u : left;
                    const uint32_t right = __shfl_up(left, 1);
                    uint2 ent;
                    ent.x = left;
                    ent.y = (lane == 0 || lane == 63) ? 0u
                            : ((lane == 1 && ssym == kAcLo + kAlphabet - 1) ? (1u << kRcPrecision) - left : right - left);
                    tab[i * 64 + lane] = ent;
                    if (lane == 0) meta.top[mi] = top;
                }
                if constexpr (!MF) publish_ready(rdy_addr, rdy_val);
                else {
                    asm volatile("" ::: "memory");
                    if (lane == 0) __hip_atomic_fetch_or(&C.s_ready[slot], 1u << half, __ATOMIC_RELAXED, __HIP_MEMORY_SCOPE_WORKGROUP);
                }
                __builtin_amdgcn_s_setprio(0);
                asm volatile("" ::: "memory");
                clk.add(3, TaskClock::kTables);
                clk.task_end(C, static_cast<uint32_t>(W), it.left, seq0 * kHalves + task,
                             (it.left << 12) | ((task & 15u) << 8) | (static_cast<uint32_t>(pw) << 4) | static_cast<uint32_t>(cnt), need_px - pix0);
            }
        }
        seq = seq0 + nb;
        phase = (phase + nb * kHalves) % kProducers;
        if (seg_body) {
            while (n_steps_total - it.left < seg_end) walk_on();
        }
        prev2_pix0 = prev_pix0;
        prev_pix0 = pix0;
        pix0 += it.n;
        prev_moved = it.moved;
    }
    return seq;
}

template <int NV, bool MF, bool DYN, class SH>
__global__ __launch_bounds__(kPipeThreads) void entropy_pipe_kernel(const EntropyParams* slots_desc) {
    const EntropyParams& P = slots_desc[blockIdx.x];
    const int tid = threadIdx.x;
    const int lane = tid & 63;
    const int wave = __builtin_amdgcn_readfirstlane(tid >> 6);
    const int dim = P.dim;
    constexpr int in_pad = 4 * NV;
    const int n_layers = P.n_layers;
    const int n_if = P.has_ifce ? P.n_ifce_out : 0;

    PipeCtx C;
    C.P = &P;
    const int ring_rows = MF ? P.ring_rows : kRingRows;
    {
        const PipeLayout L = pipe_layout(dim, n_layers, in_pad, ring_rows, MF ? mf_tables(n_layers) : 0);
        C.s_ring.off = L.ring; C.s_w.off = L.w; C.s_b.off = L.b; C.s_act.off = L.act; C.s_a.off = L.a; C.s_tab.off = L.tab;
        C.s_meta.off = L.meta; C.s_rcp.off = L.rcp; C.s_exp.off = L.exp; C.s_ready.off = L.ready; C.s_consumed.off = L.consumed;
        C.s_abort.off = L.abort; C.n_w_hidden = L.n_w_hidden;
#if defined(CCD_PIPE_TRACE)
        C.trace_off = L.end;
#endif
    }
    C.ring_mask = ring_rows - 1;
    constexpr int kActRows = MF ? 16 : 8;
    double* s_rcp = smem_at<double>(C.s_rcp.off);
    double* s_exp = smem_at<double>(C.s_exp.off);
    for (int i = tid; i < kNumScale; i += kPipeThreads) s_rcp[i] = P.rcp_table[i];
    for (int i = tid; i < kExpN; i += kPipeThreads) s_exp[i] = kExpTab[i];
    C.dim = dim; C.n_layers = n_layers; C.n_sp = P.n_spatial; C.n_if = n_if;
    C.fstride = feat_stride(n_if);
    C.k_left = -1;
    for (int k = 0; k < P.n_spatial; ++k) if (P.ctx_dy[k] == 0 && P.ctx_dx[k] == -1) C.k_left = k;

    {
        const int64_t* src = P.arm;
        for (int l = 0; l < n_layers; ++l) {
            const int n_out = (l == n_layers - 1) ? 2 : dim;
            int32_t* wt = C.s_w + (l < n_layers - 1 ? l * dim * in_pad : C.n_w_hidden);
            for (int i = tid; i < n_out * in_pad; i += kPipeThreads) {
                const int o = i / in_pad, k = i - o * in_pad;
                wt[i] = k < dim ? static_cast<int32_t>(src[k * n_out + o]) : 0;
            }
            int64_t* bb = C.s_b + (l < n_layers - 1 ? l * dim : (n_layers - 1) * dim);
            for (int i = tid; i < n_out; i += kPipeThreads) bb[i] = src[dim * n_out + i];
            src += dim * n_out + n_out;
        }
        int32_t* wst = C.s_w + C.n_w_hidden + 2 * in_pad;
        for (int i = tid; i < 2 * in_pad; i += kPipeThreads) {
            const int o = i / in_pad, k = i - o * in_pad;
            wst[i] = k < dim ? static_cast<int32_t>(src[k * 2 + o]) : 0;
        }
        if (tid < 2) C.s_b[(n_layers - 1) * dim + 2 + tid] = src[dim * 2 + tid];
    }
    for (int i = tid; i < kProducers * (kActRows * in_pad + 4); i += kPipeThreads) C.s_act[i] = 0;
    if constexpr (MF) {
        __syncthreads();
        mf_build_tables(C, in_pad, C.s_a, tid);
    }
    if (tid < kSlots) C.s_ready[tid] = 0;
    if (tid == 0) { C.s_consumed[0] = 0; C.s_consumed[1] = 0; *C.s_abort = 0; P.status[39] = 0; }
#if defined(CCD_PIPE_TRACE)
    for (int i = tid; i < kTraceTasks * 8; i += kPipeThreads) reinterpret_cast<unsigned int*>(ccd_pipe_smem + C.trace_off)[i] = 0u;
#endif

    DecState S;
    S.range = ~uint64_t{0}; S.dist = 0; S.word_pos = 2; S.wbase = 2; S.wbuf = 0; S.n_decoded = 0;
    S.n_part_batches = 0;
    S.prof_wait = 0; S.prof_work = 0; S.stall_ticks = 0; S.stall_events = 0; S.n_rare = 0; S.n_search = 0; S.n_spins = 0;
    for (int i = 0; i < 6; ++i) S.wait_by_j[i] = 0;
    if (wave == 0) {
        const uint32_t w0 = __builtin_amdgcn_readfirstlane(P.n_words > 0 ? P.words[0] : 0u);
        const uint32_t w1 = __builtin_amdgcn_readfirstlane(P.n_words > 1 ? P.words[1] : 0u);
        S.dist = (static_cast<uint64_t>(w0) << 32) | w1;
        S.wbuf = (S.wbase + lane < P.n_words) ? P.words[S.wbase + lane] : 0u;
    }
    unsigned long long prof[9] = {0, 0, 0, 0, 0, 0, 0, 0, 0};
    const unsigned long long prof_total0 = PROF_T();
    C.seq_base = 0;
    C.px_base = 0;
    __syncthreads();

    unsigned long long prof_ifce = 0, prof_bar = 0;
    for (int g = P.n_grids - 1; g >= 0; --g) {
        const unsigned long long t_if = PROF_T();
        C.H = P.grid_h[g]; C.W = P.grid_w[g];
        C.lat = P.latent[g];
        C.fin = P.ifce_in[g];
        C.fh = (g == P.n_grids - 1) ? C.H : P.grid_h[g + 1];
        C.fw = (g == P.n_grids - 1) ? C.W : P.grid_w[g + 1];
        {
            const int n_max = wf_longest_step(C.H, C.W);
            C.task_pix = n_max >= CCD_T8 ? 8 : (n_max >= CCD_T4 ? 4 : 2);
        }
        if (C.fin > 0) {
            const int fin = C.fin, fh = C.fh, fw = C.fw;
            int64_t* s_fw = reinterpret_cast<int64_t*>(static_cast<uint2*>(C.s_tab));
            const int8_t** s_src = reinterpret_cast<const int8_t**>(s_fw + fin * n_if + n_if);
            int32_t* s_gw = reinterpret_cast<int32_t*>(s_src + fin);
            int32_t* s_sh = s_gw + fin;
            {
                const int64_t* src = P.ifce + P.ifce_off[g];
                for (int i = tid; i < fin * n_if + n_if; i += kPipeThreads) s_fw[i] = src[i];
                const int base_level = (g == P.n_grids - 1) ? 0 : P.level[g + 1];
                for (int c = tid; c < fin; c += kPipeThreads) {
                    const int m = (g == P.n_grids - 1) ? g : g + 1 + c;
                    s_src[c] = P.latent[m];
                    s_gw[c] = P.grid_w[m];
                    s_sh[c] = (g == P.n_grids - 1) ? 0 : P.level[m] - base_level;
                }
            }
            __syncthreads();
            const bool zero_input = g == P.n_grids - 1;
            int16_t* feat = reinterpret_cast<int16_t*>(P.ifce_feat);
            const int64_t feat_lim = int64_t{1} << P.feat_bits;
            const int feat_hi_shift = P.feat_bits - 8;
            if (fin <= kIfceFastIn && n_if <= 8 && P.ifce_w32) {
                int32_t* const s_w32 = reinterpret_cast<int32_t*>(static_cast<uint2*>(C.s_tab) + 2048);
                for (int i = tid; i < kIfceFastIn * 8; i += kPipeThreads) {
                    const int c = i >> 3, j = i & 7;
                    s_w32[i] = (c < fin && j < n_if) ? static_cast<int32_t>(s_fw[c * n_if + j]) : 0;
                }
                __syncthreads();
                const auto pass = [&](auto kin_c) {
                    constexpr int KIN = decltype(kin_c)::value;
                    const glb_ptr<int16_t> featg = (glb_ptr<int16_t>)feat;
                    const glb_ptr<int32_t> wideg = (glb_ptr<int32_t>)P.ifce_wide;
                    const int plane = fh * fw;
                    const int fstride_g = C.fstride;
                    glb_ptr<const int8_t> srcp[KIN];
                    int gwr[KIN], shr[KIN];
#pragma unroll
                    for (int c = 0; c < KIN; ++c) {
                        const int cc = min(c, fin - 1);
                        srcp[c] = (glb_ptr<const int8_t>)reinterpret_cast<const int8_t*>(uni(reinterpret_cast<uint64_t>(s_src[cc])));
                        gwr[c] = uni(s_gw[cc]);
                        shr[c] = uni(s_sh[cc]);
                    }
                    auto fetch = [&](int p, int32_t (&v)[KIN]) {
                        const int y = p / fw, x = p - y * fw;
#pragma unroll
                        for (int c = 0; c < KIN; ++c) v[c] = static_cast<int32_t>(srcp[c][(y >> shr[c]) * gwr[c] + (x >> shr[c])]);
                    };
                    int64_t br[8];
#pragma unroll
                    for (int j = 0; j < 8; ++j) br[j] = j < n_if ? s_fw[fin * n_if + j] : 0;
                    int n_if_lane = n_if;
                    asm volatile("" : "+v"(n_if_lane));
                    const int in_scale = zero_input ? 0 : 65536;
                    int32_t v_next[KIN];
                    fetch(min(tid, plane - 1), v_next);
                    for (int p = tid; p < plane; p += kPipeThreads) {
                        int32_t v[KIN];
#pragma unroll
                        for (int c = 0; c < KIN; ++c) v[c] = v_next[c] * in_scale;
                        fetch(min(p + kPipeThreads, plane - 1), v_next);
                        int64_t acc[8];
#pragma unroll
                        for (int j = 0; j < 8; ++j) acc[j] = br[j];
#pragma unroll
                        for (int c = 0; c < KIN; ++c) {
                            const int4 w0 = *reinterpret_cast<const int4*>(s_w32 + c * 8), w1 = *reinterpret_cast<const int4*>(s_w32 + c * 8 + 4);
                            const int64_t x = v[c];
                            acc[0] += x * w0.x; acc[1] += x * w0.y; acc[2] += x * w0.z; acc[3] += x * w0.w;
                            acc[4] += x * w1.x; acc[5] += x * w1.y; acc[6] += x * w1.z; acc[7] += x * w1.w;
                        }
#pragma unroll
                        for (int j = 0; j < 8; ++j) {
                            const int32_t hi = static_cast<int32_t>(acc[j] >> 32), q32 = static_cast<int32_t>(acc[j] >> 24);
                            const bool big = static_cast<uint32_t>((hi >> feat_hi_shift) + 1) > 1u || (q32 & 0xffff) == 0x8000;
                            if (j < n_if_lane) featg[p * fstride_g + min(j, n_if - 1)] = (DYN && big) ? kFeatSentinel : static_cast<int16_t>(q32);
                            if (DYN && j < n_if_lane && big) wideg[min(j, n_if - 1) * plane + p] = q32;
                        }
                    }
                };
                if (fin <= 6) pass(std::integral_constant<int, 6>{});
                else pass(std::integral_constant<int, kIfceFastIn>{});
            } else
            for (int p = tid; p < fh * fw; p += kPipeThreads) {
                const int y = p / fw, x = p - y * fw;
                for (int o0 = 0; o0 < n_if; o0 += 8) {
                    uint64_t acc[8];
#pragma unroll
                    for (int j = 0; j < 8; ++j) acc[j] = o0 + j < n_if ? static_cast<uint64_t>(s_fw[fin * n_if + o0 + j]) : 0;
                    if (!zero_input) {
                        for (int c = 0; c < fin; ++c) {
                            const int sh = s_sh[c];
                            const uint64_t v = static_cast<uint64_t>(static_cast<int64_t>(s_src[c][(y >> sh) * s_gw[c] + (x >> sh)]) << 16);
#pragma unroll
                            for (int j = 0; j < 8; ++j)
                                if (o0 + j < n_if) acc[j] += v * static_cast<uint64_t>(s_fw[c * n_if + o0 + j]);
                        }
                    }
#pragma unroll
                    for (int j = 0; j < 8; ++j) {
                        if (o0 + j < n_if) {
                            const int64_t q8 = static_cast<int64_t>(acc[j]) >> 24;
                            const bool big = static_cast<uint64_t>(q8 + feat_lim - 1) >= static_cast<uint64_t>(2 * feat_lim - 1);
                            feat[p * C.fstride + (o0 + j)] = (DYN && big) ? kFeatSentinel : static_cast<int16_t>(q8);
                            if (DYN && big) P.ifce_wide[(o0 + j) * fh * fw + p] = static_cast<int32_t>(q8);
                        }
                    }
                }
            }
        }
        __syncthreads();
        PROF_ADD(prof_ifce, t_if);
#if defined(CCD_PIPE_PROFILE) && CCD_PIPE_PROFILE >= 3
        const unsigned long long ifce_grid_ticks = __builtin_amdgcn_s_memtime() - t_if;
#else
        const unsigned long long ifce_grid_ticks = 0;
        (void)ifce_grid_ticks;
#endif

        uint32_t seq_end;
        if (wave == 0) {
            __builtin_amdgcn_s_setprio(3);
#ifdef CCD_PIPE_PROFILE
            const unsigned long long k0 = S.prof_work;
            const unsigned long long g_t0 = __builtin_amdgcn_s_memtime(), sp0 = S.n_spins, se0 = S.stall_events;
#endif
            seq_end = decoder_grid<MF>(C, S);
            __builtin_amdgcn_s_setprio(0);
#ifdef CCD_PIPE_PROFILE
            if (lane == 0 && g == 0)
                for (int i = 0; i < 6; ++i) P.status[32 + i] = static_cast<int32_t>(S.wait_by_j[i] >> 10);
            if (lane == 0 && g < 4) {
                P.status[24 + 2 * g] = static_cast<int32_t>(ifce_grid_ticks >> 10);
                P.status[25 + 2 * g] = static_cast<int32_t>((S.prof_work - k0) >> 10);
                P.status[50 + 3 * g] = static_cast<int32_t>((__builtin_amdgcn_s_memtime() - g_t0) >> 10);
                P.status[51 + 3 * g] = static_cast<int32_t>(S.n_spins - sp0);
                P.status[52 + 3 * g] = static_cast<int32_t>(S.stall_events - se0);
            }
#endif
        } else {
            GridSeg segs[3];
            const int n_segs = grid_segments(static_cast<uint32_t>(C.H), static_cast<uint32_t>(C.W), C.task_pix, segs);
            const uint32_t grid_seq_base = C.seq_base;
            seq_end = grid_seq_base;
            for (int si = 0; si < n_segs; ++si) {
                const int tp = segs[si].task_pix;
                C.seq_base = seq_end;
                seq_end = tp == 8 ? producer_grid<NV, 8, MF, MF, DYN, SH>(C, prof, segs[si])
                                  : (tp == 4 ? producer_grid<NV, 16, false, MF, DYN, SH>(C, prof, segs[si]) : producer_grid<NV, 32, false, MF, DYN, SH>(C, prof, segs[si]));
                if (lds_load_acquire(C.s_abort) != 0) break;
            }
            C.seq_base = grid_seq_base;
        }
        const unsigned long long t_b = PROF_T();
        __syncthreads();
        PROF_ADD(prof_bar, t_b);
        if (lds_load_acquire(C.s_abort) != 0) break;
        C.seq_base = seq_end;
        C.px_base += static_cast<uint32_t>(C.H) * static_cast<uint32_t>(C.W);
    }
#if defined(CCD_PIPE_TRACE)
    {
                const unsigned int* t = reinterpret_cast<const unsigned int*>(ccd_pipe_smem + C.trace_off);
        for (int i = tid; i < kTraceTasks * 8; i += kPipeThreads) g_trace[i] = t[i];
    }
#endif
    if (tid == 0) {
        const uint32_t ab = *C.s_abort;
        P.status[0] = ab ? -static_cast<int32_t>(ab) : 0;
        P.status[1] = static_cast<int32_t>(S.word_pos);
#ifndef CCD_PIPE_PROFILE
        P.status[37] = static_cast<int32_t>(S.n_part_batches);
        {
            int n_streamed = 0;
            for (int g2 = 0; g2 < P.n_grids; ++g2) {
                const int gh = P.grid_h[g2], gw = P.grid_w[g2];
                const int n_max = wf_longest_step(gh, gw);
                StreamBody sb;
                sb.init(static_cast<uint32_t>(gh), static_cast<uint32_t>(gw), n_max >= CCD_T8 ? 8 : (n_max >= CCD_T4 ? 4 : 2));
                n_streamed += sb.on ? 1 : 0;
            }
            P.status[36] = n_streamed;
// ... 169 lines not shown
```

Before: 281.1 Mpixel/s.

## Pack per-pixel row metadata into 16-byte records read with one ds_read_b96

Changes RowMeta from separate top/cell/goff/mu_idx arrays into an array of 16-byte records, so the decoder's asm loads symbol base, ring cell and global offset with one ds_read_b96 instead of three ds_read_b32. The stored top is pre-incremented (sym0 = top+1), which removes a v_add from every symbol output. It also keeps seq/pixel counters live in v56/v57, replacing per-block scalar-to-vector moves with increments, and turns a branch in the ready-check into a select. This cuts LDS instruction count and waitcnt depth on the serial entropy-decode path, at the cost of more reserved VGPRs and riskier register juggling in hand-written asm.

```diff
diff --git a/cool_chic_amd/csrc/ccd_dec_parts4.inc b/cool_chic_amd/csrc/ccd_dec_parts4.inc
--- a/cool_chic_amd/csrc/ccd_dec_parts4.inc
+++ b/cool_chic_amd/csrc/ccd_dec_parts4.inc
@@ -76,15 +76,14 @@
                 "s_subb_u32 s51, s77, s79\n\t"
                 "444:\n\t"
                 "s_mov_b64 exec, 0xf\n\t"
-                "v_sub_u32 v52, %[top], %[raw]\n\t"
-                "v_add_u32 v52, 1, v52\n\t"
-                "ds_write_b8 %[ring], v52\n\t"
-                "global_store_byte %[goff], v52, %[lat]\n\t"
+                "v_sub_u32 v52, v62, %[raw]\n\t"
+                "ds_write_b8 v63, v52\n\t"
+                "global_store_byte v64, v52, %[lat]\n\t"
                 "s_mov_b64 exec, -1\n\t"
                 "s_add_u32 s58, %[pix0], %[i]\n\t"
                 "s_add_u32 s58, s58, 4\n\t"
-                "v_mov_b32 v56, s58\n\t"
-                "ds_write_b32 %[rdy], v56 offset:68\n\t"
+                "v_mov_b32 v57, s58\n\t"
+                "ds_write_b32 %[rdy], v57 offset:68\n\t"
                 "s_add_u32 s59, %[i], 8\n\t"
                 "s_waitcnt lgkmcnt(3)\n\t"
                 "v_readfirstlane_b32 s58, v54\n\t"
@@ -94,9 +93,7 @@
                 "s_cbranch_scc0 445f\n\t"
                 "s_mov_b64 s[52:53], s[48:49]\n\t"
                 "v_add_u32 v50, 0x800, v50\n\t"
-                "ds_read_b32 %[top], v53\n\t"
-                "ds_read_b32 %[ring], v53 offset:520\n\t"
-                "ds_read_b32 %[goff], v53 offset:1040\n\t"
+                "ds_read_b96 v[62:64], v53\n\t"
                 "s_add_u32 %[i], %[i], 4\n\t"
                 "s_mov_b32 s67, %[i]\n\t"
                 "s_add_u32 s54, %[i], 4\n\t"
@@ -289,15 +286,14 @@
                 "s_subb_u32 s51, s77, s79\n\t"
                 "454:\n\t"
                 "s_mov_b64 exec, 0xf0\n\t"
-                "v_sub_u32 v52, %[top], %[raw]\n\t"
-                "v_add_u32 v52, 1, v52\n\t"
-                "ds_write_b8 %[ring], v52\n\t"
-                "global_store_byte %[goff], v52, %[lat]\n\t"
+                "v_sub_u32 v52, v62, %[raw]\n\t"
+                "ds_write_b8 v63, v52\n\t"
+                "global_store_byte v64, v52, %[lat]\n\t"
                 "s_mov_b64 exec, -1\n\t"
                 "s_add_u32 s58, %[pix0], %[i]\n\t"
                 "s_add_u32 s58, s58, 4\n\t"
-                "v_mov_b32 v56, s58\n\t"
-                "ds_write_b32 %[rdy], v56 offset:68\n\t"
+                "v_mov_b32 v57, s58\n\t"
+                "ds_write_b32 %[rdy], v57 offset:68\n\t"
                 "s_add_u32 s59, %[i], 8\n\t"
                 "s_waitcnt lgkmcnt(3)\n\t"
                 "v_readfirstlane_b32 s58, v54\n\t"
@@ -307,9 +303,7 @@
                 "s_cbranch_scc0 455f\n\t"
                 "s_mov_b64 s[52:53], s[48:49]\n\t"
                 "v_add_u32 v50, 0x800, v50\n\t"
-                "ds_read_b32 %[top], v53\n\t"
-                "ds_read_b32 %[ring], v53 offset:520\n\t"
-                "ds_read_b32 %[goff], v53 offset:1040\n\t"
+                "ds_read_b96 v[62:64], v53\n\t"
                 "s_add_u32 %[i], %[i], 4\n\t"
                 "s_mov_b32 s67, %[i]\n\t"
                 "s_add_u32 s54, %[i], 4\n\t"
@@ -502,15 +496,14 @@
                 "s_subb_u32 s51, s77, s79\n\t"
                 "464:\n\t"
                 "s_mov_b64 exec, 0xf00\n\t"
-                "v_sub_u32 v52, %[top], %[raw]\n\t"
-                "v_add_u32 v52, 1, v52\n\t"
-                "ds_write_b8 %[ring], v52\n\t"
-                "global_store_byte %[goff], v52, %[lat]\n\t"
+                "v_sub_u32 v52, v62, %[raw]\n\t"
+                "ds_write_b8 v63, v52\n\t"
+                "global_store_byte v64, v52, %[lat]\n\t"
                 "s_mov_b64 exec, -1\n\t"
                 "s_add_u32 s58, %[pix0], %[i]\n\t"
                 "s_add_u32 s58, s58, 4\n\t"
-                "v_mov_b32 v56, s58\n\t"
-                "ds_write_b32 %[rdy], v56 offset:68\n\t"
+                "v_mov_b32 v57, s58\n\t"
+                "ds_write_b32 %[rdy], v57 offset:68\n\t"
                 "s_add_u32 s59, %[i], 8\n\t"
                 "s_waitcnt lgkmcnt(3)\n\t"
                 "v_readfirstlane_b32 s58, v54\n\t"
@@ -520,9 +513,7 @@
                 "s_cbranch_scc0 465f\n\t"
                 "s_mov_b64 s[52:53], s[48:49]\n\t"
                 "v_add_u32 v50, 0x800, v50\n\t"
-                "ds_read_b32 %[top], v53\n\t"
-                "ds_read_b32 %[ring], v53 offset:520\n\t"
-                "ds_read_b32 %[goff], v53 offset:1040\n\t"
+                "ds_read_b96 v[62:64], v53\n\t"
                 "s_add_u32 %[i], %[i], 4\n\t"
                 "s_mov_b32 s67, %[i]\n\t"
                 "s_add_u32 s54, %[i], 4\n\t"
diff --git a/cool_chic_amd/csrc/ccd_dec_parts8.inc b/cool_chic_amd/csrc/ccd_dec_parts8.inc
--- a/cool_chic_amd/csrc/ccd_dec_parts8.inc
+++ b/cool_chic_amd/csrc/ccd_dec_parts8.inc
@@ -150,15 +150,14 @@
                 "s_subb_u32 s51, s77, s79\n\t"
                 "408:\n\t"
                 "s_mov_b64 exec, 0xff\n\t"
-                "v_sub_u32 v52, %[top], %[raw]\n\t"
-                "v_add_u32 v52, 1, v52\n\t"
-                "ds_write_b8 %[ring], v52\n\t"
-                "global_store_byte %[goff], v52, %[lat]\n\t"
+                "v_sub_u32 v52, v62, %[raw]\n\t"
+                "ds_write_b8 v63, v52\n\t"
+                "global_store_byte v64, v52, %[lat]\n\t"
                 "s_mov_b64 exec, -1\n\t"
                 "s_add_u32 s58, %[pix0], %[i]\n\t"
                 "s_add_u32 s58, s58, 8\n\t"
-                "v_mov_b32 v56, s58\n\t"
-                "ds_write_b32 %[rdy], v56 offset:68\n\t"
+                "v_mov_b32 v52, s58\n\t"
+                "ds_write_b32 %[rdy], v52 offset:68\n\t"
                 "s_sub_u32 s59, s66, %[i]\n\t"
                 "s_waitcnt lgkmcnt(3)\n\t"
                 "v_readfirstlane_b32 s58, v54\n\t"
@@ -166,13 +165,12 @@
                 "s_cbranch_scc0 409f\n\t"
                 "s_bitcmp1_b32 s58, 1\n\t"
                 "s_cbranch_scc0 409f\n\t"
-                "ds_read_b32 %[top], v53\n\t"
-                "ds_read_b32 %[ring], v53 offset:520\n\t"
-                "ds_read_b32 %[goff], v53 offset:1040\n\t"
+                "ds_read_b96 v[62:64], v53\n\t"
                 "s_mov_b32 s65, 0\n\t"
                 "s_mov_b32 s54, s66\n\t"
                 "s_branch 308b\n\t"
                 "409:\n\t"
+                "v_mov_b32 v57, v52\n\t"
                 "s_mov_b64 s[52:53], s[74:75]\n\t"
                 "s_add_u32 %[i], %[i], 8\n\t"
                 "s_mov_b32 s67, %[i]\n\t"
diff --git a/cool_chic_amd/csrc/ccd_entropy_pipe.hip b/cool_chic_amd/csrc/ccd_entropy_pipe.hip
--- a/cool_chic_amd/csrc/ccd_entropy_pipe.hip
+++ b/cool_chic_amd/csrc/ccd_entropy_pipe.hip
@@ -56,13 +56,17 @@
 
 struct alignas(16) RowMeta {
     double rcp[kRows + 2];
-    int32_t mu_idx[kRows + 2];
-    int32_t top[kRows + 2];
-    uint32_t cell[kRows + 2];
-    uint32_t goff[kRows + 2];
+    struct Rec {
+        int32_t sym0;
+        uint32_t cell;
+        uint32_t goff;
+        int32_t mu_idx;
+    } rec[kRows + 2];
 };
-static_assert(offsetof(RowMeta, cell) - offsetof(RowMeta, top) == 520 && offsetof(RowMeta, goff) - offsetof(RowMeta, top) == 1040,
-              "the decoder's asm region reads cell / goff at these immediate offsets from a top symbol's address");
+static_assert(sizeof(RowMeta::Rec) == 16 && offsetof(RowMeta, rec) % 16 == 0 && offsetof(RowMeta::Rec, sym0) == 0 &&
+              offsetof(RowMeta::Rec, cell) == 4 && offsetof(RowMeta::Rec, goff) == 8 && offsetof(RowMeta::Rec, mu_idx) == 12,
+              "the decoder's asm region reads sym0 / cell / goff as one aligned ds_read_b96 into three consecutive VGPRs; the output tail\n"
+              "stores sym0 and mu_idx as words 0 and 3 of the record");
 
 extern __shared__ __attribute__((aligned(16))) unsigned char ccd_pipe_smem[];
 template <typename T>
@@ -213,13 +217,13 @@
     const int slot_mask = kRows / bpx - 1;
     int task_shift = task_pix == 8 ? 3 : (task_pix == 4 ? 2 : 1);
     const uint32_t ready_base = C.s_ready.off;
-    const uint32_t top_base = C.s_meta.off + static_cast<uint32_t>(offsetof(RowMeta, top));
+    const uint32_t rec_base = C.s_meta.off + static_cast<uint32_t>(offsetof(RowMeta, rec));
     const uint32_t tab_lane = C.s_tab.off + static_cast<uint32_t>(lane) * 8u;
-    const uint32_t lane_top_off = top_base + static_cast<uint32_t>(lane & (bpx - 1)) * 4u;
+    const uint32_t lane_rec_off = rec_base + static_cast<uint32_t>(lane & (bpx - 1)) * 16u;
     const uint64_t lat_addr = uni(reinterpret_cast<uint64_t>(C.lat));
     const RowMeta& meta = *C.s_meta;
     bool ok = true;
-    int raw = 0, top_l = 0;
+    int raw = 0;
     uint32_t n_spins = 0;
     uint32_t pix0 = uni(C.px_base);
     uint32_t n_part = 0;
@@ -238,7 +242,6 @@
         uint32_t n_step = seg_body ? seg_n_pix : static_cast<uint32_t>(it.n), step_x0 = static_cast<uint32_t>(it.x0), step_hy = static_cast<uint32_t>(it.H - it.y0);
         uint32_t steps_left = (it.raster || seg_body) ? 1u : static_cast<uint32_t>(seg_steps);
         uint32_t i = 0, mode = 0;
-        uint32_t v_ring = 0, v_goff = 0;
         while (true) {
             uint32_t status, k_rare;
             i = uni(i); seq = uni(seq); mode = uni(mode); n_spins = uni(n_spins);
@@ -260,6 +263,9 @@
                 "s_mul_i32 s72, %[n], s61\n\t"
                 "s_lshr_b32 s73, 16, %[tshift]\n\t"
                 "s_bfm_b32 s73, s73, 0\n\t"
+                "v_mov_b32 v56, %[seq]\n\t"
+                "s_add_u32 s58, %[pix0], %[i]\n\t"
+                "v_mov_b32 v57, s58\n\t"
                 "s_cmp_eq_u32 %[mode], 0\n\t"
                 "s_cbranch_scc0 6f\n\t"
                 "5:\n\t"
@@ -273,7 +279,7 @@
                 "s_lshr_b32 s57, s57, %[tshift]\n\t"
                 "s_bfm_b32 s57, s57, 0\n\t"
                 "v_lshl_add_u32 v50, s56, 9, %[tabl]\n\t"
-                "v_lshl_add_u32 v53, s56, 2, %[l4]\n\t"
+                "v_lshl_add_u32 v53, s56, 4, %[l4]\n\t"
                 "s_mov_b32 s68, 0\n\t"
                 "s_branch 18f\n\t"
                 "11:\n\t"
@@ -282,11 +288,9 @@
                 "s_cbranch_scc0 7f\n\t"
                 "18:\n\t"
                 "ds_read_b32 v52, v51\n\t"
-                "ds_read_b32 %[top], v53\n\t"
-                "ds_read_b32 %[ring], v53 offset:520\n\t"
-                "ds_read_b32 %[goff], v53 offset:1040\n\t"
+                "ds_read_b96 v[62:64], v53\n\t"
                 "ds_read2st64_b64 v[40:43], v50 offset1:1\n\t"
-                "s_waitcnt lgkmcnt(4)\n\t"
+                "s_waitcnt lgkmcnt(2)\n\t"
                 "v_readfirstlane_b32 s58, v52\n\t"
                 "s_cmp_eq_u32 s58, s57\n\t"
                 "s_cbranch_scc1 13f\n\t"
@@ -401,10 +405,9 @@
                 "s_and_b32 s58, s58, s62\n\t"
                 "s_add_u32 s58, s58, 1\n\t"
                 "s_bfm_b64 exec, s58, 0\n\t"
-                "v_sub_u32 v52, %[top], %[raw]\n\t"
-                "v_add_u32 v52, 1, v52\n\t"
-                "ds_write_b8 %[ring], v52\n\t"
-                "global_store_byte %[goff], v52, %[lat]\n\t"
+                "v_sub_u32 v52, v62, %[raw]\n\t"
+                "ds_write_b8 v63, v52\n\t"
+                "global_store_byte v64, v52, %[lat]\n\t"
                 "s_mov_b64 exec, -1\n\t"
                 "ds_write_b32 v51, %[zero]\n\t"
                 "s_add_u32 %[seq], %[seq], 1\n\t"
@@ -417,14 +420,13 @@
                 "s_and_b32 s58, s67, s62\n\t"
                 "s_sub_u32 s59, %[i], s67\n\t"
                 "s_bfm_b64 exec, s59, s58\n\t"
-                "v_sub_u32 v52, %[top], %[raw]\n\t"
-                "v_add_u32 v52, 1, v52\n\t"
-                "ds_write_b8 %[ring], v52\n\t"
-                "global_store_byte %[goff], v52, %[lat]\n\t"
+                "v_sub_u32 v52, v62, %[raw]\n\t"
+                "ds_write_b8 v63, v52\n\t"
+                "global_store_byte v64, v52, %[lat]\n\t"
                 "s_mov_b64 exec, -1\n\t"
                 "s_add_u32 s58, %[pix0], %[i]\n\t"
-                "v_mov_b32 v52, s58\n\t"
-                "ds_write_b32 %[rdy], v52 offset:68\n\t"
+                "v_mov_b32 v57, s58\n\t"
+                "ds_write_b32 %[rdy], v57 offset:68\n\t"
                 "126:\n\t"
                 "s_cmp_lt_u32 %[i], s66\n\t"
                 "s_cbranch_scc0 29f\n\t"
@@ -439,11 +441,9 @@
                 "s_mov_b32 s68, 0\n\t"
                 "28:\n\t"
                 "ds_read_b32 v52, v51\n\t"
-                "ds_read_b32 %[top], v53\n\t"
-                "ds_read_b32 %[ring], v53 offset:520\n\t"
-                "ds_read_b32 %[goff], v53 offset:1040\n\t"
+                "ds_read_b96 v[62:64], v53\n\t"
                 "ds_read2st64_b64 v[40:43], v50 offset1:1\n\t"
-                "s_waitcnt lgkmcnt(4)\n\t"
+                "s_waitcnt lgkmcnt(2)\n\t"
                 "v_readfirstlane_b32 s58, v52\n\t"
                 "s_bitcmp1_b32 s58, s59\n\t"
                 "s_cbranch_scc1 27f\n\t"
@@ -470,8 +470,8 @@
                 "s_mov_b32 s65, 0\n\t"
                 "ds_write_b32 v51, %[zero]\n\t"
                 "s_add_u32 %[seq], %[seq], 1\n\t"
-                "v_mov_b32 v52, %[seq]\n\t"
-                "ds_write_b32 %[rdy], v52 offset:64\n\t"
+                "v_mov_b32 v56, %[seq]\n\t"
+                "ds_write_b32 %[rdy], v56 offset:64\n\t"
                 "s_branch 22f\n\t"
                 "6:\n\t"
                 "s_sub_u32 s58, %[i], 1\n\t"
@@ -486,7 +486,8 @@
                 "s_add_u32 s57, s57, s56\n\t"
                 "s_lshl_b32 s57, s57, 9\n\t"
                 "v_add_u32 v50, s57, %[tabl]\n\t"
-                "v_lshl_add_u32 v53, s56, 2, %[l4]\n\t"
+                "v_lshl_add_u32 v53, s56, 4, %[l4]\n\t"
+                "ds_read_b96 v[62:64], v53\n\t"
                 "s_mov_b32 s65, 1\n\t"
                 "s_mov_b32 s66, s54\n\t"
                 "s_mov_b32 s67, s58\n\t"
@@ -495,6 +496,7 @@
                 "s_add_u32 s57, s57, 1\n\t"
                 "s_min_u32 s54, s57, s66\n\t"
                 "s_mov_b32 s68, 0\n\t"
+                "s_waitcnt lgkmcnt(0)\n\t"
                 "s_cmp_lt_u32 %[i], s54\n\t"
                 "s_cbranch_scc1 8b\n\t"
                 "s_branch 2b\n\t"
@@ -569,37 +571,33 @@
                 "80:\n\t"
 #include "ccd_dec_block16p.inc"
                 "s_mov_b64 exec, 0xffff\n\t"
-                "v_sub_u32 v52, %[top], %[raw]\n\t"
-                "v_add_u32 v52, 1, v52\n\t"
-                "ds_write_b8 %[ring], v52\n\t"
-                "global_store_byte %[goff], v52, %[lat]\n\t"
+                "v_sub_u32 v52, v62, %[raw]\n\t"
+                "ds_write_b8 v63, v52\n\t"
+                "global_store_byte v64, v52, %[lat]\n\t"
                 "s_mov_b64 exec, -1\n\t"
                 "ds_write_b32 v51, %[zero]\n\t"
                 "s_add_u32 %[seq], %[seq], 1\n\t"
-                "s_add_u32 s58, %[pix0], %[i]\n\t"
-                "v_mov_b32 v56, %[seq]\n\t"
-                "v_mov_b32 v57, s58\n\t"
+                "v_add_u32 v56, 1, v56\n\t"
+                "v_add_u32 v57, 16, v57\n\t"
                 "ds_write_b64 %[rdy], v[56:57] offset:64\n\t"
                 "22:\n\t"
                 "s_and_b32 s55, %[seq], %[smask]\n\t"
                 "v_lshl_add_u32 v51, s55, 2, %[rdy]\n\t"
                 "ds_read_b32 v54, v51\n\t"
                 "s_lshl_b32 s56, s55, %[bshift]\n\t"
-                "v_lshl_add_u32 v53, s56, 2, %[l4]\n\t"
-                "ds_read_b32 %[top], v53\n\t"
-                "ds_read_b32 %[ring], v53 offset:520\n\t"
-                "ds_read_b32 %[goff], v53 offset:1040\n\t"
+                "v_lshl_add_u32 v53, s56, 4, %[l4]\n\t"
+                "ds_read_b96 v[62:64], v53\n\t"
                 "v_lshl_add_u32 v50, s56, 9, %[tabl]\n\t"
                 "ds_read2st64_b64 v[40:43], v50 offset1:1\n\t"
                 "s_add_u32 s54, %[i], s69\n\t"
                 "s_cmp_le_u32 s54, s72\n\t"
-                "s_cbranch_scc0 25f\n\t"
-                "s_waitcnt lgkmcnt(4)\n\t"
+                "s_cselect_b32 s57, s73, -1\n\t"
+                "s_waitcnt lgkmcnt(2)\n\t"
                 "v_readfirstlane_b32 s59, v54\n\t"
-                "s_cmp_eq_u32 s59, s73\n\t"
+                "s_cmp_eq_u32 s59, s57\n\t"
                 "s_cbranch_scc1 80b\n\t"
-                "s_mov_b32 s57, s73\n\t"
-                "s_branch 23f\n\t"
+                "s_cmp_eq_u32 s57, s73\n\t"
+                "s_cbranch_scc1 23f\n\t"
                 "25:\n\t"
                 "s_cmp_lt_u32 %[i], %[n]\n\t"
                 "s_cbranch_scc0 30f\n\t"
@@ -610,7 +608,7 @@
                 "s_add_u32 s57, s58, s70\n\t"
                 "s_lshr_b32 s57, s57, %[tshift]\n\t"
                 "s_bfm_b32 s57, s57, 0\n\t"
-                "s_waitcnt lgkmcnt(4)\n\t"
+                "s_waitcnt lgkmcnt(2)\n\t"
                 "v_readfirstlane_b32 s59, v54\n\t"
                 "s_cmp_eq_u32 s59, s57\n\t"
                 "s_cbranch_scc0 23f\n\t"
@@ -654,17 +652,17 @@
                 "s_mov_b64 %[dst], s[50:51]\n\t"
                 "s_mov_b64 %[rng], s[52:53]\n\t"
                 "s_waitcnt lgkmcnt(0)\n\t"
-                : [dst] "+s"(rc_dist), [rng] "+s"(rc_range), [i] "+s"(i), [seq] "+s"(seq), [raw] "+v"(raw), [top] "+v"(top_l),
-                  [ring] "+v"(v_ring), [goff] "+v"(v_goff), [spins] "+s"(n_spins), [wpos] "+s"(word_pos), [st] "=s"(status), [kr] "=s"(k_rare),
+                : [dst] "+s"(rc_dist), [rng] "+s"(rc_range), [i] "+s"(i), [seq] "+s"(seq), [raw] "+v"(raw),
+                  [spins] "+s"(n_spins), [wpos] "+s"(word_pos), [st] "=s"(status), [kr] "=s"(k_rare),
                   [n] "+s"(n_step), [x0] "+s"(step_x0), [hy] "+s"(step_hy), [cleft] "+s"(steps_left),
                   [pix0] "+s"(pix0), [npart] "+s"(n_part)
                 : [mode] "s"(mode), [gw] "s"(static_cast<uint32_t>(grid_w)), [smask] "s"(static_cast<uint32_t>(slot_mask)),
                   [bshift] "s"(bpx_shift), [tshift] "s"(static_cast<uint32_t>(task_shift)),
                   [rdy] "v"(ready_base), [zero] "v"(0u),
                   [wbuf] "v"(wbuf), [wbase] "s"(wbase), [tabl] "v"(tab_lane), [lane] "v"(static_cast<uint32_t>(lane)),
-                  [l4] "v"(lane_top_off), [lat] "s"(lat_addr)
+                  [l4] "v"(lane_rec_off), [lat] "s"(lat_addr)
                 : "memory", "vcc", "scc", "m0", "s40", "s41", "s42", "s43", "s44", "s46", "s47", "s48", "s49", "s50", "s51", "s52", "s53", "s54", "s55",
-                  "s56", "s57", "s58", "s59", "s60", "s61", "s62", "s63", "s64", "s65", "s66", "s67", "s68", "s69", "s70", "s71", "s72", "s73", "s74", "s75", "s76", "s77", "s78", "s79", "s80", "v40", "v41", "v42", "v43", "v44", "v45", "v46", "v47", "v48", "v49", "v50", "v51", "v52", "v53", "v54", "v55", "v56", "v57", "v58", "v59", "v60", "v61");
+                  "s56", "s57", "s58", "s59", "s60", "s61", "s62", "s63", "s64", "s65", "s66", "s67", "s68", "s69", "s70", "s71", "s72", "s73", "s74", "s75", "s76", "s77", "s78", "s79", "s80", "v40", "v41", "v42", "v43", "v44", "v45", "v46", "v47", "v48", "v49", "v50", "v51", "v52", "v53", "v54", "v56", "v57", "v58", "v59", "v60", "v61", "v62", "v63", "v64");
 #pragma clang diagnostic pop
             if (status == 0) break;
             if (status == 3) {
@@ -716,7 +714,7 @@
                     ok = false;
                     break;
                 }
-                const double mu = -64.0 + static_cast<double>(meta.mu_idx[row0 + pi]) * (1.0 / 256.0);
+                const double mu = -64.0 + static_cast<double>(meta.rec[row0 + pi].mu_idx) * (1.0 / 256.0);
                 const double rcp = meta.rcp[row0 + pi];
                 const uint32_t f0 = window_left(mu, rcp, kAcLo + lane, C.s_exp);
                 const uint32_t f1 = window_left(mu, rcp, kAcLo + 64 + lane, C.s_exp);
@@ -727,7 +725,7 @@
                 if (sidx == kAlphabet - 1) right = 1u << kRcPrecision;
                 nd = rc_dist - scale * left;
                 nr = scale * static_cast<uint64_t>(right - left);
-                k = uni(1 - ((sidx + kAcLo) - meta.top[row0 + pi]));
+                k = uni(meta.rec[row0 + pi].sym0 - (sidx + kAcLo));
             }
             if (static_cast<uint32_t>(nr >> 32) == 0) {
                 nr <<= 32;
@@ -984,7 +982,6 @@
     return min(max(x + off, 0), hi);
 }
 static_assert(kMuOffset < (1 << 29) && kScaleOffset < (1 << 29) && kMuOffset >= 0 && kScaleOffset >= 0, "table_index: offsets");
-static_assert(offsetof(RowMeta, top) - offsetof(RowMeta, mu_idx) == (kRows + 2) * 4, "a pixel's top symbol is stored (kRows + 2) words behind its mu index");
 
 #if defined(CCD_PIPE_PROFILE)
 constexpr int kProfLevel = CCD_PIPE_PROFILE;
@@ -1022,8 +1019,8 @@
     __device__ __forceinline__ void count_task() { if constexpr (kProfLevel >= 3) prof[8] += 1; }
 };
 __device__ __forceinline__ void store_row_position(RowMeta& meta, int row, int y, int x, int W, int ring_mask) {
-    meta.cell[row] = static_cast<uint32_t>(ring_cell(y, x, ring_mask));
-    meta.goff[row] = static_cast<uint32_t>(y * W + x);
+    meta.rec[row].cell = static_cast<uint32_t>(ring_cell(y, x, ring_mask));
+    meta.rec[row].goff = static_cast<uint32_t>(y * W + x);
 }
 __device__ __forceinline__ void publish_ready(uint32_t rdy_addr, uint32_t rdy_val) {
     asm volatile("" ::: "memory");
@@ -1200,8 +1197,7 @@
                     const unsigned long long t_g = PROF_T();
                     {
                         const int mi = (g == 0 && live) ? slot * kBpx + half * kTaskPix + n : kRows;
-                        meta.cell[mi] = static_cast<uint32_t>(ring_cell(y, x, ring_mask));
-                        meta.goff[mi] = static_cast<uint32_t>(y * W + x);
+                        store_row_position(meta, mi, y, x, W, ring_mask);
                     }
                     uint32_t w0 = 0, w1 = 0;
 #pragma unroll
@@ -1338,7 +1334,7 @@
                     const int32_t idx_sc = static_cast<int32_t>(s8 < 0 ? 0 : (s8 > kNumScale - 1 ? kNumScale - 1 : s8));
                     const int mpx = slot * kBpx + half * kTaskPix + n;
                     if (g == 0 && live) {
-                        meta.mu_idx[mpx] = idx_mu;
+                        meta.rec[mpx].mu_idx = idx_mu;
                         meta.rcp[mpx] = C.s_rcp[idx_sc];
                     }
                     narrow_mask = static_cast<unsigned>(__ballot(g == 0 && live && idx_sc <= kNarrowMaxScale)) & 0xffffu;
@@ -1461,7 +1457,7 @@
                 int qo = q;
                 asm volatile("" : "+v"(qo));
                 const int mpx = slot * kBpx + half * kTaskPix + px;
-                mu_dst = lds_addr(&meta.mu_idx[px < cnt && qo == kQ0 ? mpx : kRows]);
+                mu_dst = lds_addr(&meta.rec[px < cnt && qo == kQ0 ? mpx : kRows]);
                 rcp_dst = lds_addr(&meta.rcp[px < cnt && qo == kQ0 + 1 ? mpx : kRows]);
                 int32_t wide_above = px < cnt && qo == kQ0 + 1 ? kNarrowMaxScale : 0x7fffffff;
                 asm volatile("" : "+v"(mu_dst), "+v"(rcp_dst), "+v"(wide_above));
@@ -1621,18 +1617,19 @@
                 uint2* tab = C.s_tab + static_cast<size_t>(base) * 64;
                 if constexpr (!MF) {
                     {
-                        int top = ((idx_mu + 128) >> 8) - 64 + 6;
-                        top = max(kAcLo + 13, min(kAcLo + kAlphabet - 1, top));
-                        lds_at<int32_t>(mu_dst)[0] = idx_mu;
-                        lds_at<int32_t>(mu_dst)[kRows + 2] = top;
+                        const int sym0 = max(kAcLo + 14, min(kAcLo + kAlphabet, ((idx_mu + 128) >> 8) - 64 + 7));
+                        int ssym_e = sym0 - e0;
+                        asm volatile("" : "+v"(ssym_e));
+                        lds_at<int32_t>(mu_dst)[0] = sym0;
+                        lds_at<int32_t>(mu_dst)[3] = idx_mu;
                         const double rcp256 = window_rcp256(own_rcp);
                         *lds_at<double>(rcp_dst) = own_rcp;
-                        const bool at_top = top == kAcLo + kAlphabet - 1;
+                        const bool at_top = sym0 == kAcLo + kAlphabet;
                         const uint32_t hi_f = at_top ? win_e0 : 0u, to_full = at_top ? win_e1 : 0u;
                         uint32_t left[kEpl];
 #pragma unroll
                         for (int j = 0; j < kEpl; ++j) {
-                            const int ssym = top - (e0 + j - 1);
+                            const int ssym = ssym_e - j;
                             uint32_t lo_m = static_cast<uint32_t>((kAcLo - ssym) >> 31);
                             if (j == kEpl - 1) lo_m &= win_left_m;
                             uint32_t l = window_cum_d256(window_d256(idx_mu, ssym), rcp256, C.s_exp) + static_cast<uint32_t>(ssym - kAcLo);
@@ -1665,7 +1662,7 @@
                     const int u = lane >> 4, e = lane & 15;
                     const int mine = u == 0 ? pix[0] : (u == 1 ? pix[1] : (u == 2 ? pix[2] : pix[3]));
                     const int mi = base + (mine < 0 ? pix[0] : mine);
-                    const int mu_idx = meta.mu_idx[mi];
+                    const int mu_idx = meta.rec[mi].mu_idx;
                     int top = ((mu_idx + 128) >> 8) - 64 + 6;
                     top = max(kAcLo + 13, min(kAcLo + kAlphabet - 1, top));
                     const double mu = -64.0 + static_cast<double>(mu_idx) * (1.0 / 256.0);
@@ -1678,7 +1675,7 @@
                     ent.y = (e == 0 || e == 15) ? 0u : ((e == 1 && ssym == kAcLo + kAlphabet - 1) ? (1u << kRcPrecision) - left : right - left);
                     if (mine >= 0) {
                         tab[mine * 64 + e] = ent;
-                        if (e == 0) meta.top[mi] = top;
+                        if (e == 0) meta.rec[mi].sym0 = top + 1;
                     }
                     if constexpr (MF) {
                         typedef unsigned int u32x4 __attribute__((ext_vector_type(4)));
@@ -1699,7 +1696,7 @@
                     wide &= wide - 1;
                     const int i = MF ? bit : bit / kLpp;
                     const int mi = base + i;
-                    const int mu_idx = meta.mu_idx[mi];
+                    const int mu_idx = meta.rec[mi].mu_idx;
                     int top = ((mu_idx + 128) >> 8) - 64 + 30;
                     top = max(kAcLo + 61, min(kAcLo + kAlphabet - 1, top));
                     const int ssym = top - (lane - 1);
@@ -1711,7 +1708,7 @@
                     ent.y = (lane == 0 || lane == 63) ? 0u
                             : ((lane == 1 && ssym == kAcLo + kAlphabet - 1) ? (1u << kRcPrecision) - left : right - left);
                     tab[i * 64 + lane] = ent;
-                    if (lane == 0) meta.top[mi] = top;
+                    if (lane == 0) meta.rec[mi].sym0 = top + 1;
                 }
                 if constexpr (!MF) publish_ready(rdy_addr, rdy_val);
                 else {
```

Measured after the change: 283.2 Mpixel/s (median of 6 runs). Within noise of the previous version (+0.8%).
